# jamshed/CaPS-SA

Measured on AMD Instinct MI355X. Metric: suffixes/sec (SA+LCP build), higher is better.
Workload: dtype u32

## Files before the change

caps-sa_amd/_binding.py:

```python
from __future__ import annotations

import ctypes
import weakref

import numpy as np

_u64, _vp, _ci = ctypes.c_uint64, ctypes.c_void_p, ctypes.c_int


class Stats(ctypes.Structure):
    _fields_ = [
        ("n", ctypes.c_uint64),
        ("idx_bytes", ctypes.c_uint32),
        ("p_eff", ctypes.c_uint32),
        ("ppp", ctypes.c_uint32),
        ("bits_per_char", ctypes.c_uint32),
        ("merge_passes_phase1", ctypes.c_uint32),
        ("merge_passes_phase2", ctypes.c_uint32),
        ("merge_passes_samples", ctypes.c_uint32),
        ("long_runs", ctypes.c_uint32),
        ("max_partition", ctypes.c_uint64),
        ("workspace_bytes", ctypes.c_uint64),
        ("ms_total", ctypes.c_double),
        ("ms_pack", ctypes.c_double),
        ("ms_sort_subarrays", ctypes.c_double),
        ("ms_select_pivots", ctypes.c_double),
        ("ms_locate_pivots", ctypes.c_double),
        ("ms_partition", ctypes.c_double),
        ("ms_merge_partitions", ctypes.c_double),
        ("ms_boundary_lcp", ctypes.c_double),
        ("ms_output", ctypes.c_double),
        ("ms_h2d", ctypes.c_double),
        ("ms_d2h", ctypes.c_double),
        ("merge_pass_ms", ctypes.c_double),
        ("merge_pass_launches", ctypes.c_uint64),
        ("merge_pass_elems", ctypes.c_uint64),
        ("tile_sort_ms", ctypes.c_double),
        ("tile_sort_launches", ctypes.c_uint64),
        ("tile_sort_elems", ctypes.c_uint64),
        ("bucket_scatter_ms", ctypes.c_double),
        ("bucket_scatter_launches", ctypes.c_uint64),
        ("bucket_scatter_elems", ctypes.c_uint64),
        ("bucket_count_ms", ctypes.c_double),
        ("collate_ms", ctypes.c_double),
        ("slot_splits", ctypes.c_uint32),
        ("slot_splits_redone", ctypes.c_uint32),
        ("path_direct", ctypes.c_uint32),
        ("path_fallback", ctypes.c_uint32),
        ("direct_groups", ctypes.c_uint32),
        ("direct_quantile", ctypes.c_uint32),
        ("direct_max_group", ctypes.c_uint64),
        ("level_a_ms", ctypes.c_double),
        ("direct_key_bits", ctypes.c_uint32),
        ("run_buckets", ctypes.c_uint32),
        ("result_waves", ctypes.c_uint32),
        ("n_devices", ctypes.c_uint32),
        ("ms_upload_max", ctypes.c_double),
        ("ms_upload_min", ctypes.c_double),
        ("ms_device_build_max", ctypes.c_double),
        ("ms_device_build_min", ctypes.c_double),
        ("ms_download_max", ctypes.c_double),
        ("ms_download_min", ctypes.c_double),
        ("tie_groups_deferred", ctypes.c_uint64),
        ("tie_elems_deferred", ctypes.c_uint64),
        ("tie_levels", ctypes.c_uint32),
        ("lcp_bytes_on_link", ctypes.c_uint32),
        ("finish_ms", ctypes.c_double),
        ("run_bucket_ms", ctypes.c_double),
        ("msd_ms", ctypes.c_double),
        ("knot_slot_splits", ctypes.c_uint32),
        ("knot_slot_splits_redone", ctypes.c_uint32),
        ("spill_entries", ctypes.c_uint64),
        ("direct_records", ctypes.c_uint32),
        ("tile_chain", ctypes.c_uint32),
        ("scatter_issue", ctypes.c_uint32),
    ]

    def as_dict(self) -> dict:
        return {k: getattr(self, k) for k, _ in self._fields_}


class ShardInfo(ctypes.Structure):
    _fields_ = [
        ("n", ctypes.c_uint64),
        ("p", ctypes.c_uint32), ("ppp", ctypes.c_uint32), ("rank", ctypes.c_uint32), ("world", ctypes.c_uint32),
        ("g0", ctypes.c_uint32), ("g1", ctypes.c_uint32),
        ("bits_per_char", ctypes.c_uint32), ("idx_bytes", ctypes.c_uint32),
        ("part_lo", ctypes.c_uint32), ("part_hi", ctypes.c_uint32),
        ("local_elems", ctypes.c_uint64),
        ("m_local", ctypes.c_uint64), ("m_total", ctypes.c_uint64),
        ("recv_total", ctypes.c_uint64),
        ("slice_off", ctypes.c_uint64),
        ("capacity", ctypes.c_uint64),
        ("ms_phase1", ctypes.c_double), ("ms_pivots", ctypes.c_double), ("ms_collate", ctypes.c_double),
        ("ms_phase2", ctypes.c_double),
        ("direct_fallback", ctypes.c_uint32), ("direct_groups", ctypes.c_uint32), ("direct_sub", ctypes.c_uint32),
        ("n_streams", ctypes.c_uint32),
        ("stream_cap", ctypes.c_uint64), ("send_capacity", ctypes.c_uint64),
        ("ms_scatter", ctypes.c_double), ("ms_sort", ctypes.c_double),
        ("ms_level_a", ctypes.c_double), ("ms_level_b", ctypes.c_double), ("ms_tile_sort", ctypes.c_double),
        ("ms_merge_passes", ctypes.c_double),
        ("level_a_elems", ctypes.c_uint64),
        ("slot_splits", ctypes.c_uint32), ("slot_splits_redone", ctypes.c_uint32),
        ("key_bytes", ctypes.c_uint32), ("exchange", ctypes.c_uint32),
        ("direct_quantile", ctypes.c_uint32), ("run_buckets", ctypes.c_uint32),
        ("tie_groups_deferred", ctypes.c_uint64), ("tie_levels", ctypes.c_uint32), ("reserved_", ctypes.c_uint32),
    ]

    def as_dict(self) -> dict:
        return {k: getattr(self, k) for k, _ in self._fields_}


SHARD_EXPORTS = ["shard_create", "shard_destroy", "shard_info", "shard_phase1", "shard_pivots", "shard_collate",
                 "shard_phase2", "shard_last_sa", "shard_fix_first_lcp", "shard_scatter", "shard_plan", "shard_sort",
                 "shard_phase1_arrays", "shard_set_key_bits"]

EXPORTS = ["device_count", "last_error", "version", "stats_bytes", "shard_info_bytes", "workspace_bytes", "workspace_bytes_ex", "release_cache", "host_alloc", "host_free", "gen_rand_seq",
           "inverse_bwt_workspace_bytes", "fm_index_bytes", "fm_from_bwt_workspace_bytes", "fm_count", "fm_locate", "fm_count_device", "fm_locate_device",
           "fm_index_bytes_ex", "fm_add_text_samples", "fm_add_text_samples_device", "fm_extract_workspace_bytes", "fm_extract", "fm_extract_device",
           "fm_match", "fm_match_device", "fm_mems_workspace_bytes", "fm_mems", "fm_mems_device", "fm_wide_index_bytes",
           "fm_wide_workspace_bytes", "kmer_workspace_bytes", "cross_workspace_bytes", "coll_workspace_bytes", "lpf_workspace_bytes", "lz77_workspace_bytes", "lce_index_bytes",
           "lce_range_min", "lce_range_min_device", "lce", "lce_device"] + SHARD_EXPORTS + [
    f"{name}_{sfx}"
    for sfx in ("u32", "u64")
    for name in ("build", "build_multi", "build_device", "verify_device", "verify_slice_device", "sort_suffixes", "sort_segments", "merge",
                 "upper_bound", "lcp", "build_bwt", "bwt_device", "inverse_bwt", "inverse_bwt_device", "fm_build", "fm_build_device",
                 "fm_build_from_bwt", "fm_build_from_bwt_device", "fm_build_wide", "fm_build_wide_device",
                 "kmers", "kmers_device", "kmer_spectrum", "kmer_spectrum_device", "kmer_census", "kmer_census_device",
                 "lpf", "lpf_device", "lz77", "lz77_device", "isa", "isa_device", "lce_build", "lce_build_device",
                 "cross_mums", "cross_mums_device", "cross_mems", "cross_mems_device",
                 "coll_kmers", "coll_kmers_device", "coll_sharing", "coll_sharing_device")
]


MEM_DTYPE = np.dtype([("pattern", "<u8"), ("start", "<u4"), ("length", "<u4"), ("first", "<u8"), ("count", "<u8")])

KMER_DTYPE = np.dtype([("first", "<u8"), ("count", "<u8"), ("pos", "<u8")])

CROSS_DTYPE = np.dtype([("a", "<u8"), ("b", "<u8"), ("len", "<u8")])
CROSS_MAX_OCC = 64

COLL_DTYPE = np.dtype([("first", "<u8"), ("count", "<u8"), ("occ", "<u8"), ("docs", "<u8")])
COLL_MAX_DOCS = 64

LZ_DTYPE = np.dtype([("pos", "<u8"), ("len", "<u8"), ("src", "<u8")])
LZ_LITERAL = 0xFFFFFFFFFFFFFFFF


class CapsSaError(RuntimeError):
    def __init__(self, code: int, msg: str):
        super().__init__(f"caps_sa error {code}: {msg}")
        self.code = code


def _sfx(idx_bits: int):
    return {32: ("u32", np.uint32), 64: ("u64", np.uint64)}[idx_bits]


# ... 965 lines not shown
```

caps-sa_amd/csrc/kernels.h:

```cpp
#pragma once
#include "kernel_lang.h"
#include "text.h"

namespace caps {

#ifndef CAPS_TILE_E
#define CAPS_TILE_E 4096
#endif
#ifndef CAPS_TILE_NT
#define CAPS_TILE_NT 1024
#endif
#ifndef CAPS_TILE_WAVES
#define CAPS_TILE_WAVES 8
#endif
#ifndef CAPS_LOCK_K
#define CAPS_LOCK_K 4
#endif
constexpr uint32_t TILE_E = CAPS_TILE_E;
constexpr uint32_t TILE_NT = CAPS_TILE_NT;
constexpr uint32_t TILE_EPT = TILE_E / TILE_NT;
constexpr uint32_t LOCK_K = CAPS_LOCK_K < TILE_EPT ? CAPS_LOCK_K : TILE_EPT;
#define TILE_WAVES_PER_SIMD CAPS_TILE_WAVES
#ifdef CAPS_NO_WAVES_BOUND
#undef LAUNCH_BOUNDS2
// ... 461 lines not shown
        }
    }
}


template <typename idx_t, int BITS, int K, bool RUNS = true>
DEV_INLINE void multi_lower_bound(const uint32_t* __restrict__ P, uint64_t n, const uint64_t* skey, const idx_t* ssa,
                                  const uint64_t (&key)[K], const idx_t (&sa)[K], uint32_t (&lo)[K], const uint32_t (&hi)[K],
                                  uint32_t top)
{
    for (uint32_t s = top >> 1; s >= 1; s >>= 1) {
        UNROLL
        for (int k = 0; k < K; ++k) {
            const uint32_t idx = lo[k] + s - 1;
            const uint64_t mk = skey[idx < TILE_E ? idx : TILE_E - 1];
            if (idx < hi[k] && mk < key[k]) lo[k] += s;
        }
    }
    UNROLL
    for (int k = 0; k < K; ++k) {
        if (lo[k] < hi[k] && skey[lo[k]] == key[k]) {
            uint32_t a = lo[k], b = hi[k];
            while (a < b) {
                const uint32_t mid = (a + b) >> 1;
                if (suffix_less<BITS, RUNS>(P, n, skey[mid], (uint64_t)ssa[mid], key[k], (uint64_t)sa[k])) a = mid + 1;
                else b = mid;
            }
            lo[k] = a;
        }
    }
}

template <int K>
DEV_INLINE void multi_key_bound(const uint64_t* skey, const uint64_t (&key)[K], const bool (&upper)[K], uint32_t (&lo)[K],
                                const uint32_t (&hi)[K], uint32_t top)
{
    for (uint32_t s = top >> 1; s >= 1; s >>= 1) {
        UNROLL
        for (int k = 0; k < K; ++k) {
            const uint32_t idx = lo[k] + s - 1;
            const uint64_t mk = skey[idx < TILE_E ? idx : TILE_E - 1];
            if (idx < hi[k] && (upper[k] ? mk <= key[k] : mk < key[k])) lo[k] += s;
        }
    }
}

HD uint32_t pow2_above(uint32_t x) { return 1u << (32 - (x ? __builtin_clz(x) : 32)); }

struct BucketParams {
    uint64_t kmin;
    uint64_t range;
    uint32_t shift;
    uint32_t B;
    uint32_t post;
    uint32_t m;
};

HD BucketParams make_bucket_params(uint64_t kmin, uint64_t kmax, uint32_t B)
{
    BucketParams q;
    q.kmin = kmin;
    q.B = B;
    q.range = kmax > kmin ? kmax - kmin : 0;
    q.shift = q.range ? (uint32_t)caps_clz64(q.range) : 0u;
    const uint64_t r32 = (q.range << q.shift) >> 32;
    uint32_t bits = 1;
    while ((2ull * B) >> bits) ++bits;
    q.post = bits < 32 ? 32 - bits : 0;
    const uint64_t num = (uint64_t)B << (32 + q.post);
    q.m = q.range ? (uint32_t)(num / (r32 + 1)) : 0u;
    return q;
}

DEV_INLINE uint32_t bucket_of(const BucketParams& bp, uint64_t key)
{
    if (bp.B <= 1) return 0;
    if (key <= bp.kmin) return 0;
    const uint64_t d = key - bp.kmin;
    if (d >= bp.range) return bp.B - 1;
    const uint32_t d32 = (uint32_t)((d << bp.shift) >> 32);
    const uint32_t b = caps_umul32hi(d32, bp.m) >> bp.post;
    return b < bp.B ? b : bp.B - 1;
}

template <uint32_t NBINS>
DEV_INLINE void block_exclusive_scan(KCTX uint32_t* h)
{
#ifdef CAPS_EMUL
    (void)kctx_;
    std::vector<uint32_t> c(NBINS);
    for (uint32_t i = 0; i < NBINS; ++i) c[i] = h[i];
    SYNC_LDS();
    uint32_t run = 0;
    for (uint32_t i = 0; i < NBINS; ++i) { h[i] = run; run += c[i]; }
    h[NBINS] = run;
    SYNC_LDS();
#else
    constexpr uint32_t BPT = NBINS / TILE_NT;
    static_assert(BPT >= 1 && BPT * TILE_NT == NBINS, "counters per thread");
    __shared__ uint32_t wave_tot[TILE_NT / 64];
    const uint32_t tid = threadIdx.x, lane = tid & 63, wv = tid >> 6;
    uint32_t v[BPT], sum = 0;
    UNROLL
    for (uint32_t i = 0; i < BPT; ++i) { v[i] = h[tid * BPT + i]; sum += v[i]; }
    uint32_t x = sum;
#define CAPS_DPP_ADD(ctrl, rows) x += (uint32_t)__builtin_amdgcn_update_dpp(0, (int)x, ctrl, rows, 0xF, false)
    CAPS_DPP_ADD(0x111, 0xF);
    CAPS_DPP_ADD(0x112, 0xF);
    CAPS_DPP_ADD(0x114, 0xF);
    CAPS_DPP_ADD(0x118, 0xF);
    CAPS_DPP_ADD(0x142, 0xA);
    CAPS_DPP_ADD(0x143, 0xC);
#undef CAPS_DPP_ADD
    if (lane == 63) wave_tot[wv] = x;
    SYNC_LDS();
    uint32_t run = x - sum;
    if (TILE_NT / 64 <= 16) {
        const uint32_t wt = lane < TILE_NT / 64 ? wave_tot[lane] : 0u;
        uint32_t ws = wt;
#define CAPS_DPP_ADD(ctrl) ws += (uint32_t)__builtin_amdgcn_update_dpp(0, (int)ws, ctrl, 0xF, 0xF, false)
        CAPS_DPP_ADD(0x111);
        CAPS_DPP_ADD(0x112);
        CAPS_DPP_ADD(0x114);
        CAPS_DPP_ADD(0x118);
#undef CAPS_DPP_ADD
        const int wvs = __builtin_amdgcn_readfirstlane((int)wv);
        run += (uint32_t)__builtin_amdgcn_readlane((int)ws, wvs) - (uint32_t)__builtin_amdgcn_readlane((int)wt, wvs);
    } else {
        for (uint32_t w = 0; w < wv; ++w) run += wave_tot[w];
    }
    UNROLL
    for (uint32_t i = 0; i < BPT; ++i) { h[tid * BPT + i] = run; run += v[i]; }
    if (tid == TILE_NT - 1) h[NBINS] = run;
    SYNC_LDS();
#endif
}
DEV_INLINE void block_exclusive_scan_bins(KCTX uint32_t* hist) { block_exclusive_scan<TILE_BINS_>(KCTX_PASS hist); }

template <typename idx_t> struct FinalOut {
    idx_t* sa = nullptr;
    idx_t* lcp = nullptr;
    uint64_t* first_key = nullptr;
    uint64_t* last_key = nullptr;
    idx_t* first_sa = nullptr;
    idx_t* last_sa = nullptr;
};

#ifdef CAPS_EMUL
extern "C" void caps_emul_count_tile(bool fast, bool known_range);
extern "C" void caps_emul_count_tile2(bool two_level_ok);
extern "C" void caps_emul_count_tile3(bool equalised_ok);
#endif
constexpr uint32_t TILE_BINS = TILE_BINS_;
#ifndef CAPS_TILE_BIN_LIMIT
#define CAPS_TILE_BIN_LIMIT 48
#endif
#ifndef CAPS_EQ_BIN_LIMIT
#define CAPS_EQ_BIN_LIMIT 128
#endif
constexpr uint32_t TILE_BIN_LIMIT = CAPS_TILE_BIN_LIMIT;
constexpr uint32_t EQ_BIN_LIMIT = CAPS_EQ_BIN_LIMIT;

template <typename idx_t>
DEV_INLINE uint64_t lcp_capped(uint32_t l, uint64_t n, idx_t a, idx_t b)
{
    if (sizeof(idx_t) == 4) {
        const uint32_t room = (uint32_t)n - (uint32_t)(a > b ? a : b);
        return l < room ? l : room;
    }
    const uint64_t room = n - (uint64_t)(a > b ? a : b);
    return l < room ? l : room;
}
template <int BITS, bool RUNS, typename idx_t>
DEV_INLINE uint64_t tile_pair_lcp(const uint32_t* __restrict__ P, uint64_t n, uint64_t ka, idx_t a, uint64_t kb, idx_t b, uint32_t)
{
    const uint64_t x = ka ^ kb;
    if (x) return lcp_capped<idx_t>((uint32_t)caps_clz64(x) / BITS, n, a, b);
    return pair_lcp<BITS, RUNS>(P, n, ka, (uint64_t)a, kb, (uint64_t)b);
}
template <int BITS, bool RUNS, typename idx_t>
DEV_INLINE uint64_t tile_pair_lcp(const uint32_t* __restrict__ P, uint64_t n, uint32_t ka, idx_t a, uint32_t kb, idx_t b, uint32_t cs)
{
    return pair_lcp32<BITS, RUNS>(P, n, ka, (uint64_t)a, kb, (uint64_t)b, cs);
}

template <typename idx_t> HD idx_t tie_sentinel() { return (idx_t)~(idx_t)0; }
template <int BITS, bool RUNS, typename idx_t>
DEV_INLINE uint64_t deferring_pair_lcp(const uint32_t* __restrict__ P, uint64_t n, uint64_t* __restrict__ bflag, uint32_t g, uint64_t ka, idx_t a,
                                       uint64_t kb, idx_t b)
{
    if (bflag && ka == kb) { bflag[g] = 1; return (uint64_t)tie_sentinel<idx_t>(); }
    return tile_pair_lcp<BITS, RUNS>(P, n, ka, a, kb, b, 0u);
}

#if defined(CAPS_PHASE_CLOCK) && !defined(CAPS_EMUL)
__device__ unsigned long long caps_phase_clock[32];
#define PHASE_T0() unsigned long long pc_t_ = clock64()
#define PHASE_MARK(i) do { const unsigned long long t_ = clock64(); if (threadIdx.x == 0) atomicAdd(&caps_phase_clock[i], t_ - pc_t_); pc_t_ = clock64(); } while (0)
#else
#define PHASE_T0() ((void)0)
#define PHASE_MARK(i) ((void)0)
#endif

#if defined(CAPS_EQ_CHECK) && !defined(CAPS_EMUL)
__device__ unsigned int caps_eq_check[64];
#define EQ_OK(ok, id) ((ok) ? true : (atomicAdd(&caps_eq_check[id], 1u), false))
#else
#define EQ_OK(ok, id) (true)
#endif
#define EQ_CHK(ok, id) ((void)EQ_OK((ok), (id)))

struct __attribute__((packed, aligned(4))) KeySaRec {
    uint32_t key_lo, key_hi;
    uint32_t sa;
};
static_assert(sizeof(KeySaRec) == 12 && alignof(KeySaRec) == 4, "12-byte records");
#ifdef CAPS_EMUL
DEV_INLINE KeySaRec rec_stream_load(const KeySaRec* p) { return *p; }
#elif !defined(CAPS_NO_STREAM_HINTS)
typedef uint32_t caps_u32x3 __attribute__((ext_vector_type(3)));
typedef caps_u32x3 caps_u32x3_a4 __attribute__((aligned(4)));
DEV_INLINE KeySaRec rec_stream_load(const KeySaRec* p)
{
    const caps_u32x3 v = __builtin_nontemporal_load(reinterpret_cast<const caps_u32x3_a4*>(p));
    KeySaRec r;
    r.key_lo = v.x; r.key_hi = v.y; r.sa = v.z;
    return r;
}
#else
DEV_INLINE KeySaRec rec_stream_load(const KeySaRec* p) { return *p; }
#endif
template <typename KP, typename idx_t> DEV_INLINE void store_rec(KP* out, uint64_t i, uint64_t key, idx_t sa)
{
    KeySaRec r;
    r.key_lo = (uint32_t)key; r.key_hi = (uint32_t)(key >> 32); r.sa = (uint32_t)sa;
    reinterpret_cast<KeySaRec*>(out)[i] = r;
}

DEV_INLINE const uint64_t* tile_src(const uint64_t* in, const uint64_t* out, bool from_out) { return from_out ? out : in; }
DEV_INLINE const uint32_t* tile_src(const uint32_t* in, const uint64_t*, bool) { return in; }

#define TILE_OUTGROWN (slot_cap != 0 && t.s1 - t.s0 > (uint64_t)slot_cap)

#define TILE_SRC_KEY in_key
#define TILE_SRC_SA in_sa
#define TILE_SORT_LOAD                                                                                          \
    PAR(tid) {                                                                                                  \
        if (tid == 0) { kmm[0] = ~0ull; kmm[1] = 0; flag[0] = 0; }                                              \
        for (uint32_t i = tid; i <= TILE_BINS; i += K_BLOCK_DIM) hist[i] = 0;                                   \
        UNROLL                                                                                                  \
        for (uint32_t k = 0; k < TILE_EPT; ++k) {                                                               \
            const uint32_t e = tid + k * TILE_NT;                                                               \
            if (e < cnt) {                                                                                      \
                uint64_t key;                                                                                   \
                idx_t sa;                                                                                       \
                if (FROM_TEXT) {                                                                                \
                    key = window64<BITS>(P, text_base + start + e);                                             \
                    sa = (idx_t)(text_base + start + e);                                                        \
                } else if (TILE_KEYS_FROM_TEXT) {    \
                    sa = STREAM_LOAD(&TILE_SRC_SA[in0 + e]);                                                    \
                    key = window64<BITS>(P, (uint64_t)sa);                                                      \
                } else {                                                                                        \
                    key = STREAM_LOAD(&TILE_SRC_KEY[in0 + e]);                                                  \
                    sa = STREAM_LOAD(&TILE_SRC_SA[in0 + e]);                                                    \
                }                                                                                               \
                TL(rk, tid, k) = (decltype(TL(rk, tid, k) + 0))key;                                             \
                TL(rs, tid, k) = sa;                                                                            \
            }                                                                                                   \
        }                                                                                                       \
    }

#define TILE_SYNC() SYNC()
#define TILE_SORT_RANGE TILE_SORT_RANGE_(seg_map[g])
#define TILE_SORT_RANGE_(MAP)                                                                                   \
    const bool known_range = seg_map != nullptr;                                                                \
    if (!known_range) {                                                                                         \
        TILE_SYNC();                                                                       \
        PAR(tid) {                                                                                              \
            uint64_t mn = ~0ull, mx = 0;                                                                        \
            UNROLL                                                                                              \
            for (uint32_t k = 0; k < TILE_EPT; ++k) {                                                           \
                const uint32_t e = tid + k * TILE_NT;                                                           \
                if (e < cnt) {                                                                                  \
                    const uint64_t key = (uint64_t)TL(rk, tid, k);                                              \
                    mn = key < mn ? key : mn;                                                                   \
                    mx = key > mx ? key : mx;                                                                   \
                }                                                                                               \
            }                                                                                                   \
            BLOCK_MINMAX_U64(&kmm[0], &kmm[1], mn, mx);                                                         \
        }                                                                                                       \
    }                                                                                                           \
    TILE_SYNC();                                                                                                \
    const BucketParams tb = known_range ? (MAP) : make_bucket_params(kmm[0], kmm[1], TILE_BINS);

#define TILE_SORT_PLACE_FINAL                                                                                   \
    PAR(tid) {                                                                                                  \
        UNROLL                                                                                                  \
        for (uint32_t k = 0; k < TILE_EPT; ++k) {                                                               \
            const uint32_t e = tid + k * TILE_NT;                                                               \
            if (e < cnt) {                                                                                      \
                const uint32_t d = TL(rd, tid, k);                                                              \
                skey[d] = TL(rk, tid, k);                                                                       \
                ssa[d] = TL(rs, tid, k);                                                                        \
            }                                                                                                   \
        }                                                                                                       \
    }                                                                                                           \
    TILE_SYNC();

#define TILE_SORT_EMIT TILE_SORT_EMIT_(0u)
#define TILE_EMIT_LCP_(ka, a, kb, b) tile_pair_lcp<BITS, TILE_RUNS>(P, n, ka, a, kb, b, TILE_KEY_SHIFT)
#define TILE_SORT_EMIT_(OV)                                                                                     \
    PAR(tid) {                                                                                                  \
        UNROLL                                                                                                  \
        for (uint32_t k = 0; k < TILE_EPT; ++k) {                                                               \
            const uint32_t e = tid + k * TILE_NT;                                                               \
            if (e < cnt) {                                                                                      \
                const uint64_t key = skey[e];                                                                   \
                const idx_t sa = ssa[e];                                                                        \
                uint64_t l = 0;                                                                                 \
                if (with_lcp && e) {                                                                            \
                    const uint32_t ov_ = (OV);                                                                  \
                    l = ov_ ? ov_ : TILE_EMIT_LCP_(skey[e - 1], ssa[e - 1], skey[e], sa);                          \
                }                                                                                               \
                if (direct) {                                                                                   \
                    STREAM_STORE(&fin.sa[start + e], sa);                                                       \
                    STREAM_STORE(&fin.lcp[start + e], (idx_t)l);                                                \
                    if (e == 0) { fin.first_key[g] = key; fin.first_sa[g] = sa; }                               \
                    if (e == cnt - 1) { fin.last_key[g] = key; fin.last_sa[g] = sa; }                           \
                } else {                                                                                        \
                    out_key[start + e] = key;                                                                   \
                    out_sa[start + e] = sa;                                                                     \
                    if (with_lcp) out_lcp[start + e] = (idx_t)l;                                                \
                }                                                                                               \
            }                                                                                                   \
        }                                                                                                       \
    }

template <typename idx_t, int BITS, bool FROM_TEXT, typename KT = uint64_t, int CHAIN = 0>
GLOBAL_FN LAUNCH_BOUNDS2(TILE_NT, TILE_WAVES_PER_SIMD) tile_sort_kernel(KCTX SegDesc sd, const uint32_t* __restrict__ P, uint64_t n,
                                                  uint64_t text_base, uint32_t lcp_mode, uint32_t slot_cap, const KT* in_key,
                                                  const idx_t* in_sa, uint64_t* out_key, idx_t* out_sa, idx_t* out_lcp,
                                                  FinalOut<idx_t> fin, const BucketParams* __restrict__ seg_map,
                                                  uint32_t* __restrict__ redo, const uint8_t* __restrict__ kshift)
{
    constexpr bool TILE_RUNS = false;
    constexpr bool K32 = sizeof(KT) == 4;
    constexpr bool TILE_KEYS_FROM_TEXT = false;
    constexpr bool BY_BUCKET = CHAIN != 0;
    constexpr uint32_t CHAIN_EARLY = BY_BUCKET ? TILE_EPT - 1 : 0u;
    static_assert(!K32 || !FROM_TEXT, "32-bit keys come from the slots of level B");
    static_assert(!BY_BUCKET || (!FROM_TEXT && !K32 && sizeof(idx_t) == 4), "bucket-indexed: 64-bit keys and 32-bit indices in slots");
    TL_DECL(KT, rk, TILE_EPT);
    TL_DECL(idx_t, rs, TILE_EPT);
    uint64_t bs0 = 0, bs1 = 0;
    BucketParams tb_early = BucketParams();
    if (BY_BUCKET) {
        bs0 = sd.seg_start[K_BLOCK_IDX];
        bs1 = sd.seg_start[K_BLOCK_IDX + 1];
        tb_early = seg_map[K_BLOCK_IDX];
        PAR(tid) {
            const uint64_t in0e = (uint64_t)K_BLOCK_IDX * slot_cap;
            UNROLL
            for (uint32_t k = 0; k < CHAIN_EARLY; ++k) {
                TL(rk, tid, k) = STREAM_LOAD(&in_key[in0e + tid + k * TILE_NT]);
                TL(rs, tid, k) = STREAM_LOAD(&in_sa[in0e + tid + k * TILE_NT]);
            }
        }
        ISSUE_FENCE();
    }
    const uint32_t b = K_BLOCK_IDX;
    if (!BY_BUCKET && b >= sd.tile_off[sd.G]) return;
    const uint32_t g = BY_BUCKET ? b : sd.tile_rec[b].g;
    const TileInfo t = BY_BUCKET ? TileInfo{bs0, bs1, 0u, g, {0u, 0u}} : tile_info(sd, b);
    if (BY_BUCKET && t.s1 == t.s0) return;
    const uint64_t start = t.s0 + (uint64_t)t.tl * TILE_E;
    const uint32_t cnt = (uint32_t)(t.s1 - start < TILE_E ? t.s1 - start : TILE_E);
    const bool with_lcp = lcp_mode != 0 && (t.s1 - t.s0) <= TILE_E;
    const bool direct = with_lcp && fin.sa != nullptr;
    const uint64_t in0 = slot_cap ? (uint64_t)g * slot_cap : start;
    const uint32_t TILE_KEY_SHIFT = K32 ? kshift[g] : 0u;
    const uint32_t tie_from = K32 ? (TILE_KEY_SHIFT + 32u) / BITS : TextTraits<BITS>::KCH;
    SHARED_ARRAY(KT, skey, TILE_E);
    SHARED_ARRAY(idx_t, ssa, TILE_E);
    SHARED_ARRAY(uint32_t, hist, TILE_BINS + 1);
    SHARED_ARRAY(uint64_t, kmm, 2);
    SHARED_ARRAY(uint32_t, flag, 1);
    constexpr bool SLOT_ORDER = sizeof(idx_t) == 4;
    SHARED_ARRAY(uint16_t, sbin, SLOT_ORDER ? TILE_E : 1);
    SHARED_ARRAY(uint16_t, perm, SLOT_ORDER ? TILE_E : 1);
    TL_DECL(uint32_t, rd, TILE_EPT);
    TL_DECL(uint32_t, rb, TILE_EPT);

    PHASE_T0();
    if (BY_BUCKET) {
        PAR(tid) {
            if (tid == 0) flag[0] = 0;
            for (uint32_t i = tid; i <= TILE_BINS; i += K_BLOCK_DIM) hist[i] = 0;
            UNROLL
            for (uint32_t k = CHAIN_EARLY; k < TILE_EPT; ++k) {
                const uint32_t e = tid + k * TILE_NT;
                if (e < cnt) {
                    TL(rk, tid, k) = STREAM_LOAD(&in_key[in0 + e]);
                    TL(rs, tid, k) = STREAM_LOAD(&in_sa[in0 + e]);
                }
            }
        }
    } else {
        TILE_SORT_LOAD
    }
    TILE_SORT_RANGE_(BY_BUCKET ? tb_early : seg_map[g])
    PHASE_MARK(0);
    bool fast = cnt > 1 && tb.range > 0;
    if (fast) {
        PAR(tid) {
            UNROLL
            for (uint32_t k = 0; k < TILE_EPT; ++k) {
                const uint32_t e = tid + k * TILE_NT;
                if (e < cnt) {
                    const uint32_t bin = bucket_of(tb, TL(rk, tid, k));
                    const uint32_t r = FETCH_ADD_U32(&hist[bin], 1u);
                    if (r >= TILE_BIN_LIMIT) flag[0] = 1;
                    TL(rb, tid, k) = bin;
                    TL(rd, tid, k) = r;
                }
            }
        }
        SYNC();
        fast = flag[0] == 0;
        PHASE_MARK(1);
    }
    if (cnt == 1) {
        PAR(tid) { if (tid == 0) { skey[0] = TL(rk, tid, 0); ssa[0] = TL(rs, tid, 0); } }
        SYNC();
        fast = true;
    } else if (fast) {
        block_exclusive_scan_bins(KCTX_PASS hist);
        PHASE_MARK(2);
        PAR(tid) {
            UNROLL
            for (uint32_t k = 0; k < TILE_EPT; ++k) {
                const uint32_t e = tid + k * TILE_NT;
                if (e < cnt) {
                    const uint32_t slot = hist[TL(rb, tid, k)] + TL(rd, tid, k);
                    skey[slot] = TL(rk, tid, k);
                    ssa[slot] = TL(rs, tid, k);
                    if (SLOT_ORDER) sbin[slot] = (uint16_t)TL(rb, tid, k);
                    else TL(rd, tid, k) = slot;
                }
            }
        }
        SYNC();
        PHASE_MARK(3);
        PAR(tid) {
            UNROLL
            for (uint32_t k = 0; k < TILE_EPT; ++k) {
                const uint32_t e = tid + k * TILE_NT;
                if (e < cnt) {
                    const uint32_t slot = SLOT_ORDER ? e : TL(rd, tid, k), bin = SLOT_ORDER ? (uint32_t)sbin[slot] : TL(rb, tid, k);
                    const uint32_t bs = hist[bin], be = hist[bin + 1];
                    const uint64_t key = SLOT_ORDER ? (uint64_t)skey[slot] : (uint64_t)TL(rk, tid, k);
                    uint32_t less = 0;
                    for (uint32_t j = bs; j < be; ++j) {
                        const uint64_t kj = skey[j];
                        less += kj < key ? 1u : 0u;
                        if (kj == key && j != slot) {
                            const uint64_t sa = SLOT_ORDER ? (uint64_t)ssa[slot] : (uint64_t)TL(rs, tid, k);
                            const uint32_t c = suffix_less_tie_bounded<BITS>(P, n, (uint64_t)ssa[j], sa, tie_from);
                            if (c == 2u) flag[0] = 1;
                            less += c & 1u;
                        }
                    }
                    if (SLOT_ORDER) RACY_STORE_U16(&perm[bs + less], (uint16_t)slot);
                    else TL(rd, tid, k) = bs + less;
                }
            }
        }
        SYNC();
        fast = flag[0] == 0;
        PHASE_MARK(4);
        if (fast && !SLOT_ORDER) {
            TILE_SORT_PLACE_FINAL
            PHASE_MARK(5);
        }
    }
#ifdef CAPS_EMUL
    caps_emul_count_tile(fast, known_range);
#endif
    if (!fast) {
        PAR(tid) { if (tid == 0) redo[1 + FETCH_ADD_U32(&redo[0], 1u)] = BY_BUCKET ? sd.tile_off[g] : b; }
        return;
    }
    if (SLOT_ORDER && cnt > 1) {
        PAR(tid) {
            UNROLL
            for (uint32_t k = 0; k < TILE_EPT; ++k) {
                const uint32_t e = tid + k * TILE_NT;
                if (e < cnt) {
                    const uint32_t sl = perm[e];
                    const KT key = skey[sl];
                    const idx_t sa = ssa[sl];
                    uint64_t l = 0;
                    if (with_lcp && e) { const uint32_t sp = perm[e - 1]; l = TILE_EMIT_LCP_(skey[sp], ssa[sp], key, sa); }
                    if (direct) {
                        STREAM_STORE(&fin.sa[start + e], sa);
                        STREAM_STORE(&fin.lcp[start + e], (idx_t)l);
                        if (e == 0) { fin.first_key[g] = key; fin.first_sa[g] = sa; }
                        if (e == cnt - 1) { fin.last_key[g] = key; fin.last_sa[g] = sa; }
                    } else {
                        out_key[start + e] = key;
                        out_sa[start + e] = sa;
                        if (with_lcp) out_lcp[start + e] = (idx_t)l;
                    }
                }
            }
        }
    } else {
        TILE_SORT_EMIT
    }
    PHASE_MARK(6);
}

GLOBAL_FN LAUNCH_BOUNDS(256) hot_tiles_kernel(KCTX SegDesc sd, uint32_t slot_cap, TileInfo* __restrict__ hot)
{
    PAR(tid) {
        const uint32_t nt = sd.tile_off[sd.G];
        const uint32_t i = K_BLOCK_IDX * K_BLOCK_DIM + tid;
        if (i < nt) {
            TileInfo t = sd.tile_rec[i];
            if (t.s1 - t.s0 > (uint64_t)slot_cap) { t.s1 = t.s0; t.tl = 0; }
            hot[i] = t;
        }
    }
}

GLOBAL_FN LAUNCH_BOUNDS(256) queue_all_tiles_kernel(KCTX SegDesc sd, uint32_t* __restrict__ redo)
{
    PAR(tid) {
        const uint32_t nt = sd.tile_off[sd.G];
        const uint32_t i = K_BLOCK_IDX * K_BLOCK_DIM + tid;
        if (i < nt) redo[1 + i] = i;
        if (i == 0) redo[0] = nt;
    }
}

#ifndef CAPS_EQ_ROUNDS
#define CAPS_EQ_ROUNDS 2
#endif
constexpr uint32_t EQ_ROUNDS = CAPS_EQ_ROUNDS;
#ifndef CAPS_TIE_G1
#define CAPS_TIE_G1 8
#endif
#ifndef CAPS_TIE_LIST_MAX
#define CAPS_TIE_LIST_MAX 2
#endif
constexpr uint32_t TIE_G1 = CAPS_TIE_G1;
constexpr uint32_t TIE_G2 = 64;
constexpr uint32_t TIE_LIST_CAP = TILE_E / 8;
constexpr uint32_t TIE_LIST_MAX = CAPS_TIE_LIST_MAX;
constexpr uint32_t TIE_DEEP_CAP = 64;
constexpr uint32_t TIE_VDEEP_CAP = 32;
constexpr uint32_t TIE_BIG_CAP = 1024;
constexpr uint32_t TIE_BIG_LANES = 64;
constexpr uint32_t EQ_FRAC_BITS = 13;
static_assert((uint64_t)TILE_BINS_ << EQ_FRAC_BITS <= (1u << 24), "positions fit 24 bits");

DEV_INLINE uint32_t eq_pos(const BucketParams& bp, uint64_t key)
{
    const uint32_t top = (bp.B << EQ_FRAC_BITS) - 1u;
    if (key <= bp.kmin) return 0;
    const uint64_t d = key - bp.kmin;
    if (d >= bp.range) return top;
    const uint32_t d32 = (uint32_t)((d << bp.shift) >> 32);
    const uint64_t prod = (uint64_t)d32 * bp.m;
    const uint32_t sh = 32u + bp.post;
    const uint32_t x = (uint32_t)(sh >= EQ_FRAC_BITS ? prod >> (sh - EQ_FRAC_BITS) : prod << (EQ_FRAC_BITS - sh));
    return x < top ? x : top;
}

DEV_INLINE uint32_t eq_big_lcp(const uint16_t* vslot, const uint32_t* vlcp, uint32_t cnt, uint32_t e)
{
    uint32_t l = 0;
    for (uint32_t q = 0; q < cnt && q < TIE_VDEEP_CAP; ++q)
        if (vslot[q] == e) l = vlcp[q];
    return l;
}

template <int BITS, bool TEXT, typename idx_t>
DEV_INLINE uint64_t eq_emit_lcp(const uint32_t* __restrict__ P, uint64_t n, uint64_t ka, idx_t a, uint64_t kb, idx_t b, uint32_t* lost, bool test_drop)
{
    if (TEXT) return pair_lcp<BITS, false>(P, n, ka, (uint64_t)a, kb, (uint64_t)b);
    const uint64_t x = ka ^ kb;
    if (x == 0) {
#ifdef CAPS_EMUL
        if (!test_drop) { std::fprintf(stderr, "eq_emit_lcp: neighbours %llu, %llu with equal keys and no lcp from the tie phases\n", (unsigned long long)a, (unsigned long long)b); std::abort(); }
#endif
        *lost = 1;
    }
    return lcp_capped<idx_t>(x ? (uint32_t)caps_clz64(x) / BITS : TextTraits<BITS>::KCH, n, a, b);
}

#ifndef CAPS_EQ_WAVES
#define CAPS_EQ_WAVES TILE_WAVES_PER_SIMD
#endif
#undef TILE_EMIT_LCP_
#define TILE_EMIT_LCP_(ka, a, kb, b) eq_emit_lcp<BITS, VDEEP>(P, n, ka, a, kb, b, &flag[1], TEST_DROP)
#undef TILE_SRC_KEY
#undef TILE_SRC_SA
#define TILE_SRC_KEY src_key
#define TILE_SRC_SA src_sa
#ifndef CAPS_EQ_FULL_SYNC
#undef TILE_SYNC
#define TILE_SYNC() SYNC_LDS()
#endif
#if !defined(CAPS_EMUL) && !defined(CAPS_PAR_PLAIN_ONLY)
#pragma push_macro("PAR")
#undef PAR
#define PAR(tid) PAR_FRESH(tid)
#define CAPS_PAR_SWITCHED
#endif
template <typename idx_t, int BITS, bool FROM_TEXT, bool VDEEP = false, bool PERSIST = true>
GLOBAL_FN LAUNCH_BOUNDS2(TILE_NT, CAPS_EQ_WAVES) tile_sort_eq_kernel(KCTX SegDesc sd, const uint32_t* __restrict__ P, uint64_t n,
                                                  uint64_t text_base, uint32_t lcp_mode, uint32_t slot_cap, const uint64_t* in_key,
                                                  const idx_t* in_sa, uint64_t* out_key, idx_t* out_sa, idx_t* out_lcp,
                                                  FinalOut<idx_t> fin, const BucketParams* __restrict__ seg_map,
// ... 1138 lines not shown
            uint64_t len = 0;
            for (uint32_t x = 0; x < sub && first + x < G; ++x) len += seg_end_of(seg_start, seg_end, first + x) - seg_start[first + x];
            uint64_t kmin = 0, kmax = ~0ull;
            if (range_mode >= 1) {
                const uint32_t j = part_off + parent;
                if (j > 0) kmin = pkey[j - 1];
                if (j + 1 < part_total) kmax = pkey[j];
                if (range_mode == 2) key32_range(kmin, kmax, j > 0, gshift[j]);
            }
            uint32_t B = 1;
            if (enable && len > TILE_E && kmax > kmin) B = (uint32_t)((len + BUCKET_TARGET - 1) / BUCKET_TARGET);
            if (sub > 1 && B < 2) B = 2;
            if (fine > 1 && B > 1 && B <= BUCKET_LDS) {
                const uint32_t k = BUCKET_LDS / B < fine ? BUCKET_LDS / B : fine;
                B *= k;
            }
            const BucketParams q = make_bucket_params(kmin, kmax, B);
            bp[g] = q;
            segB[g] = (g % sub == sub - 1 || g == G - 1) ? B : 0;
        }
    }
}

GLOBAL_FN LAUNCH_BOUNDS(256) bucket_group_kernel(KCTX uint32_t G, const uint64_t* __restrict__ segB, const uint64_t* __restrict__ bstart,
                                                 const uint64_t* __restrict__ fsegB, const uint64_t* __restrict__ fstart,
                                                 const uint64_t* __restrict__ fcount, uint64_t* __restrict__ count,
                                                 uint32_t* __restrict__ gfirst)
{
    SHARED_ARRAY(uint64_t, fc, BUCKET_LDS);
    for (uint32_t g = K_BLOCK_IDX; g < G; g += K_GRID_DIM) {
        const uint32_t B = (uint32_t)segB[g], F = (uint32_t)fsegB[g];
        const uint64_t b0 = bstart[g], f0 = fstart[g];
        if (B > BUCKET_LDS || F <= B || F > BUCKET_LDS) {
            PAR(tid) {
                for (uint32_t i = tid; i < B; i += K_BLOCK_DIM) { count[b0 + i] = i < F ? fcount[f0 + i] : 0; gfirst[b0 + i] = i; }
            }
            continue;
        }
        PAR(tid) { for (uint32_t f = tid; f < F; f += K_BLOCK_DIM) fc[f] = fcount[f0 + f]; }
        SYNC();
        PAR(tid) {
            if (tid == 0) {
                uint64_t cap = TILE_E, total = 0;
                for (uint32_t f = 0; f < F; ++f) total += fc[f];
                for (uint64_t lo = TILE_E, hi = total > TILE_E ? total : TILE_E;;) {
                    const uint64_t c_try = lo == TILE_E ? lo : (lo + hi) / 2;
                    uint32_t need = 1;
                    uint64_t run = 0;
                    for (uint32_t f = 0; f < F; ++f) {
                        const uint64_t c = fc[f];
                        if (run > 0 && run + c > c_try) { ++need; run = 0; }
                        run += c;
                    }
                    if (need <= B) { cap = c_try; hi = c_try; if (c_try == TILE_E) break; }
                    else lo = c_try + 1;
                    if (lo >= hi) { cap = hi; break; }
                }
                uint32_t gi = 0;
                uint64_t sum = 0;
                gfirst[b0] = 0;
                for (uint32_t f = 0; f < F; ++f) {
                    const uint64_t c = fc[f];
                    if (sum > 0 && sum + c > cap && gi + 1 < B) {
                        count[b0 + gi] = sum;
                        ++gi;
                        gfirst[b0 + gi] = f;
                        sum = 0;
                    }
                    sum += c;
                }
                count[b0 + gi] = sum;
                for (uint32_t i = gi + 1; i < B; ++i) { count[b0 + i] = 0; gfirst[b0 + i] = F; }
            }
        }
        SYNC();
    }
}

GLOBAL_FN LAUNCH_BOUNDS(256) bucket_ranges_kernel(KCTX const uint64_t* __restrict__ bstart, uint32_t G,
                                                  const BucketParams* __restrict__ bps, const uint64_t* __restrict__ pkey,
                                                  uint32_t range_mode, uint32_t part_off, uint32_t part_total, uint32_t sub,
                                                  BucketParams* __restrict__ tile_map,
                                                  const BucketParams* __restrict__ fbps, const uint32_t* __restrict__ gfirst,
                                                  const uint8_t* __restrict__ gshift, uint8_t* __restrict__ kshift)
{
    PAR(tid) {
        const uint64_t i = (uint64_t)K_BLOCK_IDX * K_BLOCK_DIM + tid;
        if (i < bstart[G]) {
            uint32_t a = 0, b = G;
            while (b - a > 1) {
                const uint32_t mid = (a + b) / 2;
                if (bstart[mid] <= i) a = mid; else b = mid;
            }
            const uint32_t g = a;
            const BucketParams bp = bps[g];
            uint64_t kmin = 0, kmax = ~0ull;
            if (range_mode >= 1) {
                const uint32_t j = part_off + g / sub;
                if (j > 0) kmin = pkey[j - 1];
                if (j + 1 < part_total) kmax = pkey[j];
                if (range_mode == 2) { key32_range(kmin, kmax, j > 0, gshift[j]); kshift[i] = gshift[j]; }
            }
            const uint32_t bk = (uint32_t)(i - bstart[g]);
            const double range1 = (double)(kmax - kmin) + 1.0;
            uint64_t l = kmin, h = kmax;
            if (bp.B > 1) {
                uint32_t lo = bk, hi = bk + 1, div = bp.B;
                if (gfirst) {
                    div = fbps[g].B;
                    lo = gfirst[i];
                    hi = bk + 1 < bp.B ? gfirst[i + 1] : div;
                    if (hi <= lo) hi = lo + 1;
                }
                const double dl = (double)lo / (double)div * range1, dh = (double)hi / (double)div * range1;
                if (lo > 0) l = kmin + (uint64_t)dl;
                if (hi < div) h = kmin + (uint64_t)dh;
                if (h < l) h = l;
            }
            tile_map[i] = make_bucket_params(l, h, TILE_BINS);
        }
    }
}

constexpr uint32_t TEXT_WIN = TILE_E / 4 + 24;
constexpr uint32_t SPLIT_LUT_BITS = TILE_E >= 4096 ? 12 : TILE_E >= 256 ? 8 : 4;
constexpr uint32_t SPLIT_LUT_CELLS = 1u << SPLIT_LUT_BITS;

template <int BITS> HD uint64_t text_win_base(uint64_t pos0) { return pos0 / TextTraits<BITS>::CPW; }

constexpr int MAP_LINEAR = 0, MAP_GROUPED = 1, MAP_SPLIT = 2;
HD uint32_t lds_swz(uint32_t i) { return i ^ ((i >> 4) & 15u) ^ ((i >> 8) & 15u); }
#ifdef CAPS_GA_NO_SWZ
#define GA_SWZ(i) (i)
#else
#define GA_SWZ(i) lds_swz(i)
#endif
constexpr uint32_t COUNT_CHUNK = 8;

template <bool REC, bool STREAM, typename KT, typename idx_t>
DEV_INLINE void load_elem(const KT* __restrict__ in_key, const idx_t* __restrict__ in_sa, uint64_t i, KT& key, idx_t& sa)
{
    if (REC) {
        const KeySaRec* p = reinterpret_cast<const KeySaRec*>(in_key) + i;
        const KeySaRec r = STREAM ? rec_stream_load(p) : *p;
        key = (KT)(((uint64_t)r.key_hi << 32) | r.key_lo);
        sa = (idx_t)r.sa;
    } else {
        key = STREAM ? STREAM_LOAD(&in_key[i]) : in_key[i];
        sa = STREAM ? STREAM_LOAD(&in_sa[i]) : in_sa[i];
    }
}
template <bool REC> DEV_INLINE uint64_t load_elem_key(const uint64_t* __restrict__ in_key, uint64_t i)
{
    if (REC) { const KeySaRec* p = reinterpret_cast<const KeySaRec*>(in_key) + i; return ((uint64_t)p->key_hi << 32) | p->key_lo; }
    return in_key[i];
}

template <typename idx_t, int BITS, int SRC, int MAP = MAP_LINEAR, bool REC_IN = false>
GLOBAL_FN LAUNCH_BOUNDS(TILE_NT) bucket_count_kernel(KCTX SegDesc sd, const uint32_t* __restrict__ P, uint64_t n_words,
                                                     uint64_t text_base, const uint64_t* __restrict__ in_key, RunSrc<idx_t> rsrc,
                                                     const BucketParams* __restrict__ bps, const uint64_t* __restrict__ bstart,
                                                     uint64_t* __restrict__ count, const uint64_t* __restrict__ split,
                                                     uint32_t split_stride, uint32_t in_sub, uint16_t* __restrict__ bid)
{
    constexpr bool FROM_TEXT = SRC == SRC_TEXT, FROM_RUNS = SRC == SRC_RUNS;
    SHARED_ARRAY(uint32_t, hist, BUCKET_LDS);
    SHARED_ARRAY(uint64_t, stab, MAP == MAP_SPLIT ? BUCKET_LDS : 1);
    SHARED_ARRAY(uint32_t, twin, FROM_TEXT ? TEXT_WIN : 1);
    SHARED_ARRAY(uint64_t, lsrc, FROM_RUNS ? TILE_E : 1);
    SHARED_ARRAY(idx_t, lrow, FROM_RUNS ? TILE_E : 1);
    const uint32_t n_tiles = sd.tile_off[sd.G];
    const uint32_t want = n_tiles / (4u * K_GRID_DIM);
    const uint32_t CH = want < 1u ? 1u : want > COUNT_CHUNK ? COUNT_CHUNK : want;
    const uint32_t n_chunks = (n_tiles + CH - 1) / CH;
    for (uint32_t v = K_BLOCK_IDX; v < n_chunks; v += K_GRID_DIM) {
    uint64_t cur_b0 = ~0ull;
    uint32_t cur_B = 0;
    const uint32_t b_end = (v + 1) * CH < n_tiles ? (v + 1) * CH : n_tiles;
    for (uint32_t b = v * CH; b < b_end; ++b) {
        const uint32_t g = sd.tile_rec[b].g;
        const TileInfo t = tile_info(sd, b);
        const uint64_t start = t.s0 + (uint64_t)t.tl * TILE_E;
        const uint32_t cnt = (uint32_t)(t.s1 - start < TILE_E ? t.s1 - start : TILE_E);
        const BucketParams bp = bps[g];
        const uint64_t b0 = bstart[g];
// ... 10 lines not shown
        PAR(tid) {
            if (fresh) {
                for (uint32_t i = tid; i < cur_B; i += K_BLOCK_DIM)
                    if (hist[i]) ATOMIC_ADD_U64(&count[cur_b0 + i], (uint64_t)hist[i]);
                if (lds) for (uint32_t i = tid; i < bp.B; i += K_BLOCK_DIM) hist[i] = 0;
                if (MAP == MAP_SPLIT && lds) for (uint32_t i = tid; i < n_split; i += K_BLOCK_DIM) stab[lds_swz(i)] = tab[i];
            }
            if (FROM_TEXT)
                for (uint32_t i = tid; i < TEXT_WIN; i += K_BLOCK_DIM) twin[i] = w0 + i < n_words ? P[w0 + i] : 0u;
            if (FROM_RUNS) { RUNS_STAGE(tid) }
        }
        if (fresh) { cur_b0 = lds ? b0 : ~0ull; cur_B = lds ? bp.B : 0u; }
        SYNC();
        const uint32_t top = pow2_above(n_split);
        PAR(tid) {
            uint64_t key[TILE_EPT];
            uint32_t bk[TILE_EPT];
            UNROLL
            for (uint32_t k = 0; k < TILE_EPT; ++k) {
                const uint32_t e = tid + k * TILE_NT;
                key[k] = 0;
                if (e < cnt)
                    key[k] = FROM_TEXT ? window64<BITS>(twin, text_base + start + e - w0 * TextTraits<BITS>::CPW)
                           : FROM_RUNS ? in_key[run_source<idx_t>(rsrc, runs_staged, lrow, lsrc, run_ns, run_rowR, run_rowA,
                                                                  run_a, run_b, run_x0 + e)]
                                       : load_elem_key<REC_IN>(in_key, start + e);
                bk[k] = MAP == MAP_SPLIT ? 0u : bucket_of(bp, key[k]);
            }
            if (MAP == MAP_SPLIT && lds) {
                for (uint32_t st = top >> 1; st >= 1; st >>= 1) {
                    UNROLL
                    for (uint32_t k = 0; k < TILE_EPT; ++k) {
                        const uint32_t idx = bk[k] + st - 1;
                        const uint64_t mk = stab[lds_swz(idx < n_split ? idx : n_split - 1)];
                        if (idx < n_split && mk < key[k]) bk[k] += st;
                    }
                }
            } else if (MAP == MAP_SPLIT) {
                for (uint32_t st = top >> 1; st >= 1; st >>= 1) {
                    UNROLL
                    for (uint32_t k = 0; k < TILE_EPT; ++k) {
                        const uint32_t idx = bk[k] + st - 1;
                        const uint64_t mk = tab[idx < n_split ? idx : n_split - 1];
                        if (idx < n_split && mk < key[k]) bk[k] += st;
                    }
                }
            }
            UNROLL
            for (uint32_t k = 0; k < TILE_EPT; ++k) {
                const uint32_t e = tid + k * TILE_NT;
                if (e < cnt) {
                    if (lds) FETCH_ADD_U32(&hist[bk[k]], 1u);
                    else ATOMIC_ADD_U64(&count[b0 + bk[k]], 1ull);
                    if (MAP == MAP_SPLIT && bid && lds) bid[start + e] = (uint16_t)bk[k];
                }
            }
        }
        SYNC();
    }
    if (cur_B) {
        PAR(tid) {
            for (uint32_t i = tid; i < cur_B; i += K_BLOCK_DIM)
                if (hist[i]) ATOMIC_ADD_U64(&count[cur_b0 + i], (uint64_t)hist[i]);
        }
        SYNC();
    }
    }
}

template <typename idx_t> struct Spill {
    uint64_t* count = nullptr;
    uint64_t cap = 0;
    uint32_t chunk = 0;
    uint64_t base = 0;
    uint64_t* key = nullptr;
    idx_t* sa = nullptr;
    uint32_t* bucket = nullptr;
    idx_t* rel = nullptr;
};
constexpr uint32_t SPILL_LONG = 64;
constexpr uint32_t SPILL_LONG_CAP = TILE_E / SPILL_LONG;
constexpr uint32_t SPILL_CHUNK = TILE_E / 128 ? TILE_E / 128 : 1;

template <typename idx_t, int BITS, int SRC, int MAP, typename KT = uint64_t, bool SPILL = false, bool REC_IN = false, bool ISSUE = false>
GLOBAL_FN LAUNCH_BOUNDS(TILE_NT) bucket_scatter_kernel(KCTX SegDesc sd, const uint32_t* __restrict__ P, uint64_t n_words,
                                                       uint64_t text_base, const KT* __restrict__ in_key,
                                                       const idx_t* __restrict__ in_sa, RunSrc<idx_t> rsrc,
                                                       const BucketParams* __restrict__ bps, const uint64_t* __restrict__ bstart,
                                                       const uint64_t* __restrict__ sub_start, uint64_t slot_cap,
                                                       idx_t* __restrict__ cursor,
                                                       KT* __restrict__ out_key, idx_t* __restrict__ out_sa,
                                                       const BucketParams* __restrict__ fbps, const uint32_t* __restrict__ gfirst,
                                                       const uint64_t* __restrict__ split, const uint16_t* __restrict__ split_lut,
                                                       const uint32_t* __restrict__ split_span, uint32_t sub, uint32_t split_stride,
                                                       uint32_t in_sub, const uint16_t* __restrict__ bid, Spill<idx_t> spill)
{
    constexpr bool GROUPED = MAP == MAP_GROUPED;
    const bool spec = slot_cap != 0;
    const idx_t NO_SLOT = (idx_t)~(idx_t)0;
#if CAPS_SCATTER_SWZ
    const uint32_t v = sub > 1 ? K_BLOCK_IDX
                               : (uint32_t)xcd_swizzle(K_BLOCK_IDX, K_GRID_DIM);
#else
    const uint32_t v = K_BLOCK_IDX;
#endif
    const uint32_t sx = sub > 1 ? K_BLOCK_IDX % sub : 0u;
    if (v >= sd.tile_off[sd.G]) return;
    const uint32_t b = v;
    const uint32_t g = sd.tile_rec[b].g;
    const TileInfo t = tile_info(sd, b);
    const uint64_t start = t.s0 + (uint64_t)t.tl * TILE_E;
    const uint32_t cnt = (uint32_t)(t.s1 - start < TILE_E ? t.s1 - start : TILE_E);
    static_assert(!ISSUE || (REC_IN && MAP == MAP_LINEAR && !SPILL), "loads first: the records of level A under the linear map");
    TL_DECL(KT, rk, TILE_EPT);
    TL_DECL(idx_t, rs, TILE_EPT);
    if (ISSUE) {
        if (cnt == 0) return;
        PAR(tid) {
            UNROLL
            for (uint32_t k = 0; k < TILE_EPT; ++k) {
                const uint32_t e = tid + k * TILE_NT;
                load_elem<REC_IN, true>(in_key, in_sa, start + (e < cnt ? e : cnt - 1), TL(rk, tid, k), TL(rs, tid, k));
            }
        }
        ISSUE_FENCE();
    }
    const BucketParams bp = bps[g];
    const uint64_t b0 = bstart[g];
    const bool grouped = GROUPED && bp.B > 1 && bp.B <= BUCKET_LDS;
    const BucketParams fbp = GROUPED ? fbps[g] : bp;
    SHARED_ARRAY(uint32_t, hist, TILE_BINS + 1);
    SHARED_ARRAY(idx_t, obase, TILE_BINS);
    static_assert(sizeof(KT) == 8 || (SRC == SRC_ARRAYS && MAP == MAP_LINEAR), "32-bit keys: arrays in, linear map");
    static_assert(!REC_IN || (SRC == SRC_ARRAYS && sizeof(KT) == 8 && sizeof(idx_t) == 4), "records: arrays in, 64-bit keys, 32-bit indices");
    SHARED_ARRAY(KT, skey, TILE_E);
    SHARED_ARRAY(idx_t, ssa, TILE_E);
    SHARED_ARRAY(uint16_t, sbk, TILE_E);
    SHARED_ARRAY(uint64_t, lr_at, SPILL ? SPILL_LONG_CAP : 1);
    SHARED_ARRAY(idx_t, lr_old, SPILL ? SPILL_LONG_CAP : 1);
    SHARED_ARRAY(uint32_t, lr_c, SPILL ? SPILL_LONG_CAP : 1);
    SHARED_ARRAY(uint32_t, lr_b, SPILL ? SPILL_LONG_CAP : 1);
    SHARED_ARRAY(uint32_t, nlong, 2);
    static_assert(!SPILL || (MAP == MAP_SPLIT && sizeof(KT) == 8), "the spill stream: splits by knots, 64-bit keys");
    TL_DECL(uint32_t, rb, TILE_EPT);
    TL_DECL(idx_t, rr, TILE_EPT);
    constexpr bool FROM_TEXT = SRC == SRC_TEXT, FROM_RUNS = SRC == SRC_RUNS;
    const bool lds = bp.B > 1 && bp.B <= BUCKET_LDS;
    uint32_t* twin = reinterpret_cast<uint32_t*>(skey);
    uint64_t* lsrc = reinterpret_cast<uint64_t*>(skey);
    idx_t* lrow = ssa;
    uint16_t* gtab = sbk;
    static_assert(TILE_E >= BUCKET_LDS && BUCKET_LDS <= 65536, "group table fits the bucket-id staging array");
    const uint64_t w0 = text_win_base<BITS>(text_base + start);
    uint64_t* stab = reinterpret_cast<uint64_t*>(skey) + TILE_E / 4;
    uint16_t* slut = reinterpret_cast<uint16_t*>(ssa);
    static_assert(TEXT_WIN * sizeof(uint32_t) <= (TILE_E / 4) * sizeof(uint64_t) && TILE_E / 4 + BUCKET_LDS <= TILE_E,
                  "text window + splitter table fit the key staging array");
    static_assert((SPLIT_LUT_CELLS + 1) * sizeof(uint16_t) <= TILE_E * sizeof(idx_t), "splitter LUT fits the index staging array");
    const uint32_t n_split = MAP == MAP_SPLIT && bp.B > 1 ? bp.B - 1 : 0u;
    const uint64_t* tab = MAP == MAP_SPLIT ? split + (uint64_t)(g / in_sub) * split_stride : nullptr;
    RUNS_TILE_SETUP
    if (ISSUE) {
        if (!lds) {
            PAR(tid) {
                UNROLL
                for (uint32_t k = 0; k < TILE_EPT; ++k) {
                    const uint32_t e = tid + k * TILE_NT;
                    if (e < cnt) {
                        const uint64_t bi = (b0 + (bp.B == 1 ? 0u : bucket_of(bp, (uint64_t)TL(rk, tid, k)))) * (spec ? sub : 1u) + sx;
                        const uint64_t off = bp.B == 1 ? (start - t.s0) + e : (uint64_t)caps_fetch_add(&cursor[bi], (idx_t)1);
                        if (!spec || off < slot_cap) {
                            const uint64_t dst = (spec ? bi * slot_cap : sub_start[bi]) + off;
                            out_key[dst] = TL(rk, tid, k);
                            out_sa[dst] = TL(rs, tid, k);
                        }
                    }
                }
                if (spec && bp.B == 1 && tid == 0) caps_fetch_add(&cursor[b0 * sub + sx], (idx_t)cnt);
            }
            DRAIN_GLOBAL();
            return;
        }
        PAR(tid) {
            for (uint32_t i = tid; i <= TILE_BINS; i += K_BLOCK_DIM) hist[i] = 0;
        }
        SYNC_LDS();
        PAR(tid) {
            UNROLL
            for (uint32_t k = 0; k < TILE_EPT; ++k) {
                const uint32_t e = tid + k * TILE_NT;
                if (e < cnt) {
                    const uint32_t bk = bucket_of(bp, (uint64_t)TL(rk, tid, k));
                    TL(rb, tid, k) = bk;
                    TL(rr, tid, k) = FETCH_ADD_U32(&hist[bk], 1u);
                }
            }
        }
        DRAIN_GLOBAL();
    } else {
    if (lds || FROM_TEXT || FROM_RUNS) {
        PAR(tid) {
            if (lds) for (uint32_t i = tid; i <= TILE_BINS; i += K_BLOCK_DIM) hist[i] = 0;
            if (SPILL && tid < 2) nlong[tid] = 0;
            if (MAP == MAP_SPLIT && lds && !bid) {
                for (uint32_t i = tid; i < n_split; i += K_BLOCK_DIM) stab[lds_swz(i)] = tab[i];
                if (split_lut) for (uint32_t i = tid; i <= SPLIT_LUT_CELLS; i += K_BLOCK_DIM) slut[i] = split_lut[i];
            }
            if (grouped)
                for (uint32_t i = tid; i < bp.B; i += K_BLOCK_DIM) {
                    const uint32_t f0 = gfirst[b0 + i], f1 = i + 1 < bp.B ? gfirst[b0 + i + 1] : fbp.B;
                    for (uint32_t f = f0; f < f1 && f < fbp.B; ++f) gtab[f] = (uint16_t)i;
                }
            if (FROM_TEXT)
                for (uint32_t i = tid; i < TEXT_WIN; i += K_BLOCK_DIM) twin[i] = w0 + i < n_words ? P[w0 + i] : 0u;
            if (FROM_RUNS) { RUNS_STAGE(tid) }
        }
        SYNC();
    }
    if (MAP == MAP_SPLIT && lds && bid) {
        PAR(tid) {
            UNROLL
            for (uint32_t k = 0; k < TILE_EPT; ++k) {
                const uint32_t e = tid + k * TILE_NT;
                if (e < cnt) {
                    const uint32_t bk = bid[start + e];
                    load_elem<REC_IN, false>(in_key, in_sa, start + e, TL(rk, tid, k), TL(rs, tid, k));
                    TL(rb, tid, k) = bk;
                    TL(rr, tid, k) = FETCH_ADD_U32(&hist[bk], 1u);
                }
            }
        }
    } else if (MAP == MAP_SPLIT && lds) {
        const uint32_t top = pow2_above(split_lut ? split_span[0] : n_split);
        TL_DECL(uint32_t, rh, TILE_EPT);
        PAR(tid) {
            UNROLL
            for (uint32_t k = 0; k < TILE_EPT; ++k) {
                const uint32_t e = tid + k * TILE_NT;
                const uint64_t src = start + e;
                uint64_t key = 0;
                idx_t sa = 0;
                if (e < cnt) {
                    if (FROM_TEXT) {
                        key = window64<BITS>(twin, text_base + start + e - w0 * TextTraits<BITS>::CPW);
                        sa = (idx_t)(text_base + start + e);
                    } else { KT key_in; load_elem<REC_IN, true>(in_key, in_sa, src, key_in, sa); key = (uint64_t)key_in; }
                }
                const uint32_t cell = (uint32_t)(key >> (64 - SPLIT_LUT_BITS));
                TL(rk, tid, k) = key;
                TL(rs, tid, k) = sa;
                TL(rb, tid, k) = split_lut ? slut[cell] : 0u;
                TL(rh, tid, k) = split_lut ? slut[cell + 1] : n_split;
            }
            for (uint32_t s = top >> 1; s >= 1; s >>= 1) {
                UNROLL
                for (uint32_t k = 0; k < TILE_EPT; ++k) {
                    const uint32_t idx = TL(rb, tid, k) + s - 1;
// ... 5 lines not shown
            for (uint32_t k = 0; k < TILE_EPT; ++k) {
                const uint32_t e = tid + k * TILE_NT;
                if (e < cnt) TL(rr, tid, k) = FETCH_ADD_U32(&hist[TL(rb, tid, k)], 1u);
            }
        }
    } else {
    PAR(tid) {
        UNROLL
        for (uint32_t k = 0; k < TILE_EPT; ++k) {
            const uint32_t e = tid + k * TILE_NT;
            if (e < cnt) {
                const uint64_t src = FROM_RUNS ? run_source<idx_t>(rsrc, runs_staged, lrow, lsrc, run_ns, run_rowR, run_rowA, run_a,
                                                                   run_b, run_x0 + e)
                                               : start + e;
                KT key_in = 0;
                idx_t sa = 0;
                if (FROM_TEXT) sa = (idx_t)(text_base + start + e);
                else load_elem<REC_IN, true>(in_key, in_sa, src, key_in, sa);
                const uint64_t key = FROM_TEXT ? window64<BITS>(twin, text_base + start + e - w0 * TextTraits<BITS>::CPW) : (uint64_t)key_in;
                uint32_t bk = 0;
                idx_t r;
                if (bp.B == 1) r = e;
                else {
                    if (MAP == MAP_SPLIT) {
                        uint32_t a = 0, z = bp.B - 1;
                        while (a < z) { const uint32_t mid = (a + z) >> 1; if (tab[mid] < key) a = mid + 1; else z = mid; }
                        bk = a;
                    } else {
                        bk = bucket_of(fbp, key);
                        if (grouped) bk = gtab[bk];
                    }
                    r = lds ? FETCH_ADD_U32(&hist[bk], 1u) : caps_fetch_add(&cursor[(b0 + bk) * (spec ? sub : 1u) + sx], (idx_t)1);
                }
                TL(rk, tid, k) = key;
                TL(rs, tid, k) = sa;
                TL(rb, tid, k) = bk;
                TL(rr, tid, k) = r;
            }
        }
    }
    }
    if (!lds) {
        PAR(tid) {
            UNROLL
            for (uint32_t k = 0; k < TILE_EPT; ++k) {
                const uint32_t e = tid + k * TILE_NT;
                if (e < cnt) {
                    const uint64_t off = (bp.B == 1 ? (start - t.s0) : 0) + TL(rr, tid, k);
                    const uint64_t bi = (b0 + TL(rb, tid, k)) * (spec ? sub : 1u) + sx;
                    if (!spec || off < slot_cap) {
                        const uint64_t dst = (spec ? bi * slot_cap : sub_start[bi]) + off;
                        out_key[dst] = TL(rk, tid, k);
                        out_sa[dst] = TL(rs, tid, k);
                    }
                }
            }
            if (spec && bp.B == 1 && tid == 0) caps_fetch_add(&cursor[b0 * sub + sx], (idx_t)cnt);
        }
        return;
    }
    }
    SYNC();
    constexpr uint32_t BPT = (TILE_BINS + TILE_NT - 1) / TILE_NT;
    TL_DECL(idx_t, co, BPT);
    TL_DECL(uint32_t, cc, BPT);
    PAR(tid) {
        UNROLL
        for (uint32_t j = 0; j < BPT; ++j) {
            const uint32_t i = tid + j * TILE_NT;
            const uint32_t c = i < bp.B ? hist[i] : 0u;
            TL(cc, tid, j) = c;
            TL(co, tid, j) = 0;
            if (c) TL(co, tid, j) = caps_fetch_add(&cursor[spec ? (b0 + i) * sub + sx : b0 + i], (idx_t)c);
        }
    }
    block_exclusive_scan_bins(KCTX_PASS hist);
    PAR(tid) {
        UNROLL
        for (uint32_t k = 0; k < TILE_EPT; ++k) {
            const uint32_t e = tid + k * TILE_NT;
            if (e < cnt) {
                const uint32_t bk = TL(rb, tid, k);
                const uint32_t q = hist[bk] + (uint32_t)TL(rr, tid, k);
                skey[q] = TL(rk, tid, k);
                ssa[q] = TL(rs, tid, k);
                sbk[q] = (uint16_t)bk;
            }
        }
        UNROLL
        for (uint32_t j = 0; j < BPT; ++j) {
            const uint32_t i = tid + j * TILE_NT;
            if (i < bp.B) {
                const uint32_t c = TL(cc, tid, j);
                const idx_t old = TL(co, tid, j);
                idx_t ob = 0;
                if (c) {
                    const uint64_t ci = spec ? (b0 + i) * sub + sx : b0 + i;
                    if (!spec) ob = (idx_t)(sub_start[b0 + i] + old);
                    else if ((uint64_t)old + c <= slot_cap) ob = (idx_t)(ci * slot_cap + old);
                    else if (SPILL && spill.count) {
                        uint64_t at = ~0ull;
                        if (spill.chunk) {
                            const uint32_t lo = FETCH_ADD_U32(&nlong[1], c);
                            if ((uint64_t)lo + c <= spill.chunk) at = (uint64_t)b * spill.chunk + lo;
                        }
                        if (at == ~0ull) at = FETCH_ADD_U64(spill.count, (uint64_t)c);
                        ob = NO_SLOT;
                        if (at + c <= spill.cap) {
                            ob = (idx_t)(spill.base + at);
                            if (c < SPILL_LONG) {
                                for (uint32_t j = 0; j < c; ++j) { spill.bucket[at + j] = (uint32_t)(b0 + i); spill.rel[at + j] = (idx_t)(old + j); }
                            } else {
                                const uint32_t q = FETCH_ADD_U32(&nlong[0], 1u);
                                lr_at[q] = at;
                                lr_old[q] = old;
                                lr_c[q] = c;
                                lr_b[q] = (uint32_t)(b0 + i);
                            }
                        }
                    } else ob = NO_SLOT;
                }
                obase[i] = ob;
            }
        }
    }
    if (ISSUE) DRAIN_GLOBAL();
    SYNC_LDS();
    PAR(tid) {
        UNROLL
        for (uint32_t k = 0; k < TILE_EPT; ++k) {
            const uint32_t q = tid + k * TILE_NT;
            if (q < cnt) {
                const uint32_t bk = sbk[q];
                const idx_t ob = obase[bk];
                if (SPILL && ob != NO_SLOT && (uint64_t)ob >= spill.base) {
                    const uint64_t dst = (uint64_t)ob - spill.base + (q - hist[bk]);
                    spill.key[dst] = skey[q];
                    spill.sa[dst] = ssa[q];
                } else if (ob != NO_SLOT) {
                    const uint64_t dst = (uint64_t)ob + (q - hist[bk]);
                    STREAM_STORE2(&out_key[dst], skey[q]);
                    STREAM_STORE2(&out_sa[dst], ssa[q]);
                }
            }
        }
        if (SPILL) {
            const uint32_t nl = nlong[0];
            for (uint32_t r = 0; r < nl && r < SPILL_LONG_CAP; ++r) {
                const uint64_t at = lr_at[r];
                const idx_t old = lr_old[r];
                const uint32_t c = lr_c[r], bb = lr_b[r];
                for (uint32_t j = tid; j < c; j += K_BLOCK_DIM) { spill.bucket[at + j] = bb; spill.rel[at + j] = (idx_t)(old + j); }
            }
        }
    }
}

template <typename idx_t>
GLOBAL_FN LAUNCH_BOUNDS(256) spill_gather_kernel(KCTX const uint64_t* __restrict__ seg_start, uint32_t NB, uint64_t slot_cap,
                                                 const uint8_t* __restrict__ skip, const uint64_t* __restrict__ slot_key,
                                                 const idx_t* __restrict__ slot_sa, uint64_t* __restrict__ dst_key,
                                                 idx_t* __restrict__ dst_sa)
{
    SHARED_ARRAY(uint32_t, lst, 256);
    SHARED_ARRAY(uint32_t, ln, 1);
    for (uint64_t base = (uint64_t)K_BLOCK_IDX * 256u; base < NB; base += (uint64_t)K_GRID_DIM * 256u) {
        PAR(tid) { if (tid == 0) ln[0] = 0; }
        SYNC();
        PAR(tid) {
            const uint64_t b = base + tid;
            if (b < NB) {
                const uint64_t len = seg_start[b + 1] - seg_start[b];
                if (len > slot_cap || (len && skip && skip[b])) lst[FETCH_ADD_U32(&ln[0], 1u)] = (uint32_t)b;
            }
        }
        SYNC();
        const uint32_t m = ln[0];
        for (uint32_t q = 0; q < m; ++q) {
            const uint32_t b = lst[q];
            const uint64_t s0 = seg_start[b], len = seg_start[b + 1] - s0;
            const uint64_t cnt = len < slot_cap ? len : slot_cap;
            PAR(tid) {
                for (uint64_t i = tid; i < cnt; i += K_BLOCK_DIM) {
                    dst_key[s0 + i] = slot_key[(uint64_t)b * slot_cap + i];
                    dst_sa[s0 + i] = slot_sa[(uint64_t)b * slot_cap + i];
                }
            }
        }
        SYNC();
    }
}

template <typename idx_t>
GLOBAL_FN LAUNCH_BOUNDS(256) spill_place_kernel(KCTX Spill<idx_t> sp, uint64_t cnt, const uint64_t* __restrict__ seg_start,
                                                uint64_t* __restrict__ dst_key, idx_t* __restrict__ dst_sa)
{
    PAR(tid) {
        for (uint64_t i = (uint64_t)K_BLOCK_IDX * K_BLOCK_DIM + tid; i < cnt; i += (uint64_t)K_GRID_DIM * K_BLOCK_DIM) {
            const uint32_t b = sp.bucket[i];
            if (b == ~0u) continue;
            const uint64_t d = seg_start[b] + (uint64_t)sp.rel[i];
            dst_key[d] = sp.key[i];
            dst_sa[d] = sp.sa[i];
        }
    }
}

#ifndef CAPS_GA_TILES
#define CAPS_GA_TILES 4
#endif
constexpr uint32_t GA_TILES = CAPS_GA_TILES;
constexpr uint32_t GA_E = GA_TILES * TILE_E;
constexpr uint32_t GA_EPT = GA_E / TILE_NT;
static_assert(GA_E <= (1u << 14) && BUCKET_LDS <= (1u << 11), "group << 14 | position fits a register");

template <typename idx_t, int BITS, typename KT = uint64_t, bool REC_OUT = false>
GLOBAL_FN LAUNCH_BOUNDS2(TILE_NT, TILE_WAVES_PER_SIMD) group_scatter_kernel(KCTX const uint32_t* __restrict__ P, uint64_t n_words,
                                                      uint64_t text_base, uint64_t len, const uint64_t* __restrict__ split, uint32_t K1,
                                                      const uint16_t* __restrict__ split_lut, const uint32_t* __restrict__ split_span,
                                                      uint32_t sub, uint64_t slot_cap, idx_t* __restrict__ cursor,
                                                      KT* __restrict__ out_key, idx_t* __restrict__ out_sa,
                                                      uint32_t tile_first, uint32_t tile_stride,
                                                      const uint64_t* __restrict__ region_start, const uint64_t* __restrict__ region_cap,
                                                      const uint8_t* __restrict__ gshift, uint32_t own_lo, uint32_t own_hi)
{
// ... 4442 lines not shown
```

caps-sa_amd/csrc/pipeline.h:

```cpp
#pragma once
#include <algorithm>
#include <cmath>
#include <cstdlib>
#include <cstdio>
#include <limits>
#include <stdexcept>
#include <string>
#include <vector>

#include "kernels.h"
#include "bounded.h"
#include "../../include/caps_sa_hip.h"

#ifndef CAPS_BACKEND_DEFINED
#include "hip_backend.h"
#endif

namespace caps {

template <typename idx_t> struct ElemBuf {
    uint64_t* key = nullptr;
    idx_t* sa = nullptr;
    idx_t* lcp = nullptr;
    size_t region_bytes = 0;
};

constexpr size_t WS_ALIGN = 256;
inline size_t align_up(size_t b) { return (b + (WS_ALIGN - 1)) & ~(WS_ALIGN - 1); }
inline char* align_up(char* p) { return reinterpret_cast<char*>(align_up(reinterpret_cast<uintptr_t>(p))); }

struct Arena {
    char* base = nullptr;
    size_t off = 0;
    template <typename T> T* take(size_t count)
    {
        off = align_up(off);
        T* p = base ? reinterpret_cast<T*>(base + off) : nullptr;
        off += count * sizeof(T);
        return p;
    }
};

struct SegBufs {
    uint64_t* seg_start = nullptr;
    uint64_t* seg_end = nullptr;
    uint32_t* tile_off = nullptr;
    TileInfo* tile_rec = nullptr;
    uint64_t* out2 = nullptr;
    uint32_t G = 0;
    SegDesc desc() const { return SegDesc{seg_start, tile_off, tile_rec, G}; }
};

constexpr uint32_t kMaxPasses = 96;

#ifndef CAPS_DIRECT_SUB
#define CAPS_DIRECT_SUB 8
#endif
constexpr uint32_t DIRECT_SUB = CAPS_DIRECT_SUB;
constexpr uint32_t DIRECT_RECORDS_DEFAULT = 1;
constexpr uint32_t DIRECT_TILE_CHAIN_DEFAULT = 1;
constexpr uint32_t DIRECT_SCATTER_ISSUE_DEFAULT = 1;
#ifndef CAPS_BUCKET_Q_32NDS
#define CAPS_BUCKET_Q_32NDS 24
#endif
#ifndef CAPS_QUANTILE_SPB
#define CAPS_QUANTILE_SPB 64
#endif
constexpr uint32_t BUCKET_Q = (TILE_E * CAPS_BUCKET_Q_32NDS) / 32;
constexpr uint32_t QUANTILE_SPB = CAPS_QUANTILE_SPB;

#ifndef CAPS_EQ_FINE
#define CAPS_EQ_FINE 16
#endif
constexpr uint32_t EQ_FINE = CAPS_EQ_FINE;

struct BucketBufs {
    BucketParams* params = nullptr;
    uint64_t* segB = nullptr;
    uint64_t* bstart = nullptr;
    uint64_t* count = nullptr;
    void* cursor = nullptr;
    uint64_t* scan_tmp = nullptr;
    uint64_t *first_key = nullptr, *last_key = nullptr;
    BucketParams* tile_map = nullptr;
    void *first_sa = nullptr, *last_sa = nullptr;
    SegBufs sub;
    BucketParams* fparams = nullptr;
    uint64_t* fsegB = nullptr;
    uint64_t* fstart = nullptr;
    uint64_t* fcount = nullptr;
    uint32_t* gfirst = nullptr;
    uint8_t* kshift = nullptr;
    uint8_t* skip = nullptr;
    uint64_t* run_list = nullptr;
    uint32_t nb_cap = 0;
    uint64_t tile_cap = 0;
    static uint32_t bucket_bound(uint64_t n_elems, uint32_t G) { return (uint32_t)(n_elems / BUCKET_Q + 2 * (uint64_t)G + 2); }
};

template <typename idx_t> struct Plan {
    uint64_t n = 0;
    int text_bits = 8;
    uint32_t p = 0;
    uint32_t ppp = 0;
    uint64_t m = 0;
    uint64_t tile_cap = 0;
    uint32_t* P = nullptr;
    ElemBuf<idx_t> A, B, SA_, SB_;
    uint64_t* pkey = nullptr;
    idx_t* psa = nullptr;
    idx_t* Pm = nullptr;
    idx_t* ruler = nullptr;
    idx_t* PmT = nullptr;
    idx_t* rulerT = nullptr;
    uint64_t* sizes = nullptr;
    uint64_t* gkey = nullptr;
    uint64_t* dstat = nullptr;
    idx_t* dcur = nullptr;
    uint16_t* glut = nullptr;
    uint8_t* gshift = nullptr;
    uint64_t* knots = nullptr;
    uint64_t* rcap = nullptr;
    uint64_t* rstart = nullptr;
    uint64_t* partial = nullptr;
    SegBufs seg1, seg2, segS;
    TileDesc* desc = nullptr;
    BucketBufs bk;
    uint64_t* pass_elems = nullptr;
    uint32_t* present = nullptr;
    uint8_t* lut = nullptr;
    size_t bytes = 0;
};

inline void effective_params(uint64_t n, uint64_t p_arg, uint32_t* p_eff, uint32_t* ppp)
{
    uint64_t p = p_arg > 0 ? p_arg : 8192;
    if (n / 16 < p) p = n / 16;
    if (p < 2) { *p_eff = (uint32_t)p; *ppp = 0; return; }
    const uint64_t a = (uint64_t)std::ceil(32.0 * std::log((double)n));
    const uint64_t b = n / p - 1;
    *p_eff = (uint32_t)p;
    *ppp = (uint32_t)(a < b ? a : b);
}

// ... 143 lines not shown
{
    auto alphabet = [&](uint64_t len, uint32_t present[8]) {
        be.memset(present_dev, 0, 16 * sizeof(uint32_t));
        const uint64_t want = (len + 16 * 256 - 1) / (16 * 256);
        const uint32_t grid = (uint32_t)(want < 4096 ? (want ? want : 1) : 4096);
        CAPS_LAUNCH(alphabet_kernel, grid, 256, be, dT, len, present_dev);
        be.d2h(present, present_dev, 8 * sizeof(uint32_t));
        be.sync();
    };
    auto pack = [&](int bits, const uint8_t lut[256], uint32_t* bad) {
        be.h2d(lut_dev, lut, 256);
        const uint64_t n_words = packed_words(n, bits);
        const uint64_t want = (n_words / (bits == 2 ? 1 : 4) + 255) / 256 + 1;
        const uint32_t grid = (uint32_t)(want < 65536 ? want : 65536);
        if (bits == 2) CAPS_LAUNCH(pack_kernel<2>, grid, 256, be, dT, n, (const uint8_t*)lut_dev, P, n_words, bad);
        else CAPS_LAUNCH(pack_kernel<8>, grid, 256, be, dT, n, (const uint8_t*)lut_dev, P, n_words, bad);
    };
    uint32_t present[8];
    uint8_t lut[256];
#ifdef CAPS_EMUL
    constexpr uint64_t SAMPLE = 1u << 12;
#else
    constexpr uint64_t SAMPLE = 1u << 20;
#endif
    if (n >= 16 * SAMPLE && !std::getenv("CAPS_SA_FULL_ALPHABET")) {
        alphabet(SAMPLE, present);
        if (build_lut(present, lut) == 2) {
            pack(2, lut, present_dev + 8);
            uint32_t bad = 0;
            be.d2h(&bad, present_dev + 8, sizeof bad);
            build_run_table(be, P, n, 2);
            if (!bad) return 2;
        }
    }
    alphabet(n, present);
    const int bits = build_lut(present, lut);
    if (bits > arena_bits) throw AlphabetError();
    pack(bits, lut, nullptr);
    build_run_table(be, P, n, bits);
    return bits;
}

template <typename OutT>
inline void device_exclusive_scan(Backend& be, const uint64_t* in, uint32_t G, OutT* out, uint64_t* tmp)
{
    const uint32_t chunks = (G + SCAN_CHUNK - 1) / SCAN_CHUNK;
    uint64_t* sums = tmp;
    uint64_t* offs = tmp + chunks + 1;
    CAPS_LAUNCH((block_scan_kernel<OutT>), chunks ? chunks : 1, 1024, be, in, (uint64_t)G, out, sums);
    CAPS_LAUNCH(scan_sizes_kernel, 1, 1024, be, (const uint64_t*)sums, chunks, offs);
    CAPS_LAUNCH((add_offsets_kernel<OutT>), chunks ? chunks : 1, 1024, be, out, (uint64_t)G, (const uint64_t*)offs, chunks);
}

#ifdef CAPS_EMUL
constexpr uint32_t kSmallScan = 48;
#else
constexpr uint32_t kSmallScan = 32768;
#endif

inline void prepare_segments(Backend& be, const SegBufs& s, uint64_t tile_bound, uint64_t* big_tmp = nullptr,
                             uint64_t* big_cnt = nullptr, bool use_end = false, const uint8_t* skip = nullptr)
{
    be.memset(s.out2, 0, 2 * sizeof(uint64_t));
    const uint64_t* send = use_end ? s.seg_end : nullptr;
    if (s.G <= kSmallScan || !big_tmp) {
        CAPS_LAUNCH(seg_prepare_kernel, 1, 1024, be, (const uint64_t*)s.seg_start, send, s.G, s.tile_off, s.out2, skip);
    } else {
        CAPS_LAUNCH(tile_count_kernel, (s.G + 255) / 256, 256, be, (const uint64_t*)s.seg_start, send, s.G, big_cnt, s.out2, skip);
        device_exclusive_scan<uint32_t>(be, big_cnt, s.G, s.tile_off, big_tmp);
        CAPS_LAUNCH(tile_total_kernel, 1, 64, be, (const uint32_t*)s.tile_off, s.G, s.out2);
    }
    const uint32_t grid = (uint32_t)((tile_bound + 255) / 256);
    CAPS_LAUNCH(tile_map_kernel, grid ? grid : 1, 256, be, (const uint64_t*)s.seg_start, send, (const uint32_t*)s.tile_off, s.G, s.tile_rec);
}

inline uint32_t tiles_of(uint64_t len) { return (uint32_t)((len + TILE_E - 1) / TILE_E); }

template <typename idx_t> struct SortResult {
    ElemBuf<idx_t> buf[2];
    uint32_t passes = 0;
    bool skip_finished = false;
    bool unified = false;
    bool k32 = false;
    bool failed = false;
    SegBufs segs;
    struct RunBucket { uint64_t s0, s1, key; };
    std::vector<RunBucket> run_buckets;
    SegBufs run_tables;
    const BucketBufs* run_bk = nullptr;
    TileDesc* run_desc = nullptr;
    uint64_t total = 0;
    uint64_t* defer_flags = nullptr;
    TileDesc* defer_desc = nullptr;
    uint64_t cap = 0;
    mutable bool msd_failed = false;
    KernelClock* finish_clock = nullptr;
    KernelClock* runb_clock = nullptr;
    KernelClock* msd_clock = nullptr;
    mutable uint64_t msd_groups = 0, msd_elems = 0;
    mutable uint32_t msd_levels = 0;
    uint32_t n_tiles = 0;
    FinalOut<idx_t> fin;
    ElemBuf<idx_t> uniform() const { return unified ? buf[0] : buf[passes & 1]; }
    PingPong<idx_t> pingpong() const
    {
        PingPong<idx_t> pp;
        for (int i = 0; i < 2; ++i) { pp.key[i] = buf[i].key; pp.sa[i] = buf[i].sa; pp.lcp[i] = buf[i].lcp; }
        return pp;
    }
};

struct SortOpts {
    bool from_text = false;
    uint64_t text_base = 0;
    bool need_lcp = false;
    bool skip_finished = false;
    bool no_equalise = false;
    const BucketBufs* bk = nullptr;
    uint32_t range_mode = 0;
    const uint64_t* pkey = nullptr;
    uint32_t part_off = 0, part_total = 0;
    bool speculate = false;
    uint32_t* slot_stats = nullptr;
    bool seg_ends = false;
    uint32_t sub = 1;
    const uint64_t* in_key = nullptr;
    const void* in_sa = nullptr;
    bool in_records = false;
    const uint8_t* gshift = nullptr;
    bool k32 = false;
    bool keys_only = false;
    bool comparison_only = false;
    bool skewed_keys = false;
    const uint64_t* knots = nullptr;
    uint32_t knots_per_parent = 0;
    bool knots_have_prev = false;
    bool spill_slots = false;
    TileInfo* hot_tile_rec = nullptr;
    uint64_t* spill_stats = nullptr;
    uint64_t in_extent = 0;
    const SegBufs* run_tables = nullptr;
    uint64_t* defer_flags = nullptr;
    const void* runs = nullptr;
    bool unify = false;
    void* final_sa = nullptr;
    void* final_lcp = nullptr;
    struct { uint64_t *first_key, *last_key; void *first_sa, *last_sa; } bnd = {nullptr, nullptr, nullptr, nullptr};
    uint32_t tile_chain = 0;
    uint32_t* tile_chain_used = nullptr;
    uint32_t scatter_issue = 0;
    uint32_t* scatter_issue_used = nullptr;
    KernelClock* tile_clock = nullptr;
    KernelClock* merge_clock = nullptr;
    KernelClock* scatter_clock = nullptr;
    KernelClock* count_clock = nullptr;
    uint64_t* pass_counters = nullptr;
};

template <typename idx_t, int BITS>
SortResult<idx_t> segmented_sort(Backend& be, const uint32_t* P, uint64_t n, TileDesc* desc, const SegBufs& s, uint32_t n_tiles,
                                 uint64_t max_len, ElemBuf<idx_t> cur, ElemBuf<idx_t> oth, uint64_t n_elems, const SortOpts& o)
{
    if (o.keys_only) {
        if (o.from_text || o.need_lcp || o.runs) throw std::invalid_argument("a keys-only sort takes (key, index) arrays and emits no LCPs");
        n = 0;
    }
    SortResult<idx_t> r;
    r.buf[0] = cur;
    r.buf[1] = oth;
    r.skip_finished = o.skip_finished;
    r.segs = s;
    r.n_tiles = n_tiles;
    if (n_tiles == 0) return r;
    const bool dbg = std::getenv("CAPS_SA_DEBUG") != nullptr;
    auto mark = [&](const char* what) { if (dbg) { be.sync(); std::fprintf(stderr, "[sort] %s\n", what); } };
    bool from_text = o.from_text;
    const BucketParams* seg_map = nullptr;
    SegBufs segs = s;
    bool skip = o.skip_finished;
    uint32_t slot_cap = 0;
    uint64_t* slot_key = nullptr;
    idx_t* slot_sa = nullptr;
    uint32_t slot_grid = 0;
    if (o.bk && (max_len > TILE_E || o.seg_ends)) {
        const BucketBufs& bk = *o.bk;
        const SegDesc psd = s.desc();
        const uint64_t* s_end = o.seg_ends ? (const uint64_t*)s.seg_end : (const uint64_t*)nullptr;
        const bool by_knots = o.knots != nullptr;
        if (by_knots) {
            const uint64_t NB = (uint64_t)(s.G / o.sub) * o.knots_per_parent;
            if (NB > bk.nb_cap) throw std::invalid_argument("more knot buckets than the bucket tables hold");
            CAPS_LAUNCH(knot_plan_kernel, (s.G + 255) / 256, 256, be, s.G, o.sub, o.knots_per_parent, bk.params, bk.segB);
            CAPS_LAUNCH(scan_sizes_kernel, 1, 1024, be, (const uint64_t*)bk.segB, s.G, bk.bstart);
            CAPS_LAUNCH(knot_ranges_kernel, (uint32_t)((NB + 255) / 256), 256, be, o.knots, NB, bk.tile_map, o.knots_have_prev ? 1u : 0u);
        } else {
        CAPS_LAUNCH(bucket_plan_kernel, (s.G + 255) / 256, 256, be, (const uint64_t*)s.seg_start, s_end, s.G, o.range_mode, o.pkey, o.part_off,
                    o.part_total ? o.part_total : s.G, 1u, 1u, o.sub,
                    bk.params, bk.segB, o.gshift);
        CAPS_LAUNCH(scan_sizes_kernel, 1, 1024, be, (const uint64_t*)bk.segB, s.G, bk.bstart);
        CAPS_LAUNCH(bucket_ranges_kernel, (bk.nb_cap + 255) / 256, 256, be, (const uint64_t*)bk.bstart, s.G,
                    (const BucketParams*)bk.params, o.pkey, o.range_mode, o.part_off, o.part_total ? o.part_total : s.G, o.sub,
                    bk.tile_map, (const BucketParams*)nullptr, (const uint32_t*)nullptr, o.gshift, bk.kshift);
        }
        seg_map = bk.tile_map;
        mark("bucket plan");
        const uint32_t pgrid = n_tiles < be.persistent_blocks() ? n_tiles : be.persistent_blocks();
        const bool runs = o.runs != nullptr;
        const RunSrc<idx_t> rsrc = runs ? *static_cast<const RunSrc<idx_t>*>(o.runs) : RunSrc<idx_t>();
        const uint64_t n_words = from_text ? packed_words(n, BITS) : 0;
        const uint64_t tbase = from_text ? o.text_base : 0;
        const uint64_t* src_key = o.in_key ? o.in_key : (const uint64_t*)cur.key;
        const idx_t* src_sa = o.in_key ? static_cast<const idx_t*>(o.in_sa) : (const idx_t*)cur.sa;
        const bool rec_in = o.in_records;
        if (rec_in && (sizeof(idx_t) != 4 || !o.in_key || from_text || o.runs || o.k32))
            throw std::invalid_argument("records: (64-bit key, 32-bit index) arrays given by the caller");
        uint16_t* bid = nullptr;
        if (by_knots && o.in_extent && !from_text && !o.runs && oth.region_bytes && !std::getenv("CAPS_SA_NO_BUCKET_IDS")) {
            const size_t room = (size_t)((reinterpret_cast<char*>(oth.key) + oth.region_bytes) - reinterpret_cast<char*>(oth.lcp));
            const uint64_t extent = o.in_key ? o.in_extent : n_elems;
            if (room >= extent * sizeof(uint16_t)) bid = reinterpret_cast<uint16_t*>(oth.lcp);
        }
        auto scatter = [&](const uint64_t* sub_start, uint32_t cap, uint64_t* okey, idx_t* osa, bool grouped = false) {
            const BucketParams* fbps = grouped ? bk.fparams : nullptr;
            const uint32_t* gfirst = grouped ? bk.gfirst : nullptr;
            BackendEvent s0 = be.record();
#define CAPS_SCATTER_LAUNCH(SRC_, MAP_, ikey, isa)                                                                          \
            CAPS_LAUNCH((bucket_scatter_kernel<idx_t, BITS, SRC_, MAP_>), n_tiles, TILE_NT, be, psd, P, n_words, tbase, ikey, isa, rsrc, \
                        (const BucketParams*)bk.params, (const uint64_t*)bk.bstart, sub_start, (uint64_t)cap, static_cast<idx_t*>(bk.cursor),       \
                        okey, osa, fbps, gfirst, o.knots, (const uint16_t*)nullptr, (const uint32_t*)nullptr, 1u, o.knots_per_parent, o.sub, \
                        (const uint16_t*)bid, Spill<idx_t>())
#define CAPS_SCATTER_LAUNCH_REC(MAP_)                                                                                        \
            CAPS_LAUNCH((bucket_scatter_kernel<idx_t, BITS, SRC_ARRAYS, MAP_, uint64_t, false, true>), n_tiles, TILE_NT, be, psd, P, n_words, tbase, \
                        src_key, src_sa, rsrc, (const BucketParams*)bk.params, (const uint64_t*)bk.bstart, sub_start, (uint64_t)cap,               \
                        static_cast<idx_t*>(bk.cursor), okey, osa, fbps, gfirst, o.knots, (const uint16_t*)nullptr, (const uint32_t*)nullptr, 1u,   \
                        o.knots_per_parent, o.sub, (const uint16_t*)bid, Spill<idx_t>())
            const uint64_t* nokey = nullptr;
            const idx_t* nosa = nullptr;
            if (rec_in) {
                if constexpr (sizeof(idx_t) == 4) {
                    if (by_knots) CAPS_SCATTER_LAUNCH_REC(MAP_SPLIT);
                    else if (grouped) CAPS_SCATTER_LAUNCH_REC(MAP_GROUPED);
                    else if (o.scatter_issue & 1u) {
                        CAPS_LAUNCH((bucket_scatter_kernel<idx_t, BITS, SRC_ARRAYS, MAP_LINEAR, uint64_t, false, true, true>), n_tiles, TILE_NT, be, psd,
                                    P, n_words, tbase, src_key, src_sa, rsrc, (const BucketParams*)bk.params, (const uint64_t*)bk.bstart, sub_start,
                                    (uint64_t)cap, static_cast<idx_t*>(bk.cursor), okey, osa, fbps, gfirst, o.knots, (const uint16_t*)nullptr,
                                    (const uint32_t*)nullptr, 1u, o.knots_per_parent, o.sub, (const uint16_t*)bid, Spill<idx_t>());
                        if (o.scatter_issue_used) *o.scatter_issue_used |= 1u;
                    } else CAPS_SCATTER_LAUNCH_REC(MAP_LINEAR);
                }
            } else
            if (from_text) { if (grouped) CAPS_SCATTER_LAUNCH(SRC_TEXT, MAP_GROUPED, nokey, nosa); else CAPS_SCATTER_LAUNCH(SRC_TEXT, MAP_LINEAR, nokey, nosa); }
            else if (runs) { if (grouped) CAPS_SCATTER_LAUNCH(SRC_RUNS, MAP_GROUPED, src_key, src_sa);
                             else CAPS_SCATTER_LAUNCH(SRC_RUNS, MAP_LINEAR, src_key, src_sa); }
            else if (by_knots) CAPS_SCATTER_LAUNCH(SRC_ARRAYS, MAP_SPLIT, src_key, src_sa);
            else { if (grouped) CAPS_SCATTER_LAUNCH(SRC_ARRAYS, MAP_GROUPED, src_key, src_sa);
                   else CAPS_SCATTER_LAUNCH(SRC_ARRAYS, MAP_LINEAR, src_key, src_sa); }
#undef CAPS_SCATTER_LAUNCH
#undef CAPS_SCATTER_LAUNCH_REC
            BackendEvent s1 = be.record();
            if (o.scatter_clock) { o.scatter_clock->spans.push_back({s0, s1}); o.scatter_clock->elems.push_back(n_elems); }
        };
        uint64_t out2[2] = {0, 0};
        auto adopt_buckets = [&]() {
            device_exclusive_scan<uint64_t>(be, bk.count, bk.nb_cap, bk.sub.seg_start, bk.scan_tmp);
        };
        const bool run_buckets = by_knots && o.need_lcp && o.final_sa && bk.skip && !std::getenv("CAPS_SA_NO_RUN_BUCKETS") &&
                                 n < (1ull << RunKey<(int)sizeof(idx_t)>::RB);
        auto bucket_tiles = [&]() {
            segs = bk.sub;
            segs.G = bk.nb_cap;
            uint64_t rl[1 + 4 * RUN_BUCKET_MAX];
            if (run_buckets) {
                const uint64_t NB = (uint64_t)(s.G / o.sub) * o.knots_per_parent;
                be.memset(bk.skip, 0, bk.nb_cap);
                be.memset(bk.run_list, 0, sizeof(uint64_t));
                CAPS_LAUNCH(run_bucket_mark_kernel, (uint32_t)((NB + 255) / 256), 256, be, o.knots, NB, o.knots_have_prev ? 1u : 0u, (uint32_t)BITS,
                            (const uint64_t*)bk.sub.seg_start, bk.skip, bk.run_list);
            }
            prepare_segments(be, segs, bk.tile_cap, bk.scan_tmp, bk.count, false, run_buckets ? bk.skip : nullptr);
            be.d2h(out2, segs.out2, sizeof out2);
            if (run_buckets) be.d2h(rl, bk.run_list, sizeof rl);
            be.sync();
            if (run_buckets) {
                const uint64_t cnt = rl[0] < RUN_BUCKET_MAX ? rl[0] : RUN_BUCKET_MAX;
                for (uint64_t j = 0; j < cnt; ++j) r.run_buckets.push_back({rl[2 + 4 * j], rl[3 + 4 * j], rl[4 + 4 * j]});
                std::sort(r.run_buckets.begin(), r.run_buckets.end(),
                          [](const typename SortResult<idx_t>::RunBucket& a, const typename SortResult<idx_t>::RunBucket& b) { return a.s0 < b.s0; });
                r.run_tables = o.run_tables ? *o.run_tables : bk.sub;
                r.run_bk = &bk;
                r.run_desc = desc;
                r.total = n_elems;
            }
        };
        const uint64_t nb_here = std::min<uint64_t>(bk.nb_cap, n_elems / BUCKET_TARGET + 2 * (uint64_t)(s.G / o.sub) + 2);
        const uint64_t slot_elems = nb_here * TILE_E;
        bool slots = false;
        if (by_knots && (from_text || runs)) throw std::invalid_argument("quantile buckets read (key, sa) arrays");
        if (o.k32 && (from_text || runs || by_knots || !o.speculate || !o.in_key || !o.final_sa))
            throw std::invalid_argument("32-bit keys: a slot split of (key32, sa) arrays with direct output");
        const bool can_slot = o.speculate && !by_knots &&
                              oth.region_bytes >= slot_elems * ((o.k32 ? sizeof(uint32_t) : sizeof(uint64_t)) + sizeof(idx_t)) &&
                              slot_elems + TILE_E < (uint64_t)std::numeric_limits<idx_t>::max();
        if (o.k32 && !can_slot) { r.failed = true; return r; }
        if (can_slot) {
            slot_key = oth.key;
            slot_sa = reinterpret_cast<idx_t*>(reinterpret_cast<char*>(oth.key) + slot_elems * sizeof(uint64_t));
            be.memset(bk.cursor, 0, (size_t)bk.nb_cap * sizeof(idx_t));
            if (o.k32) {
                slot_sa = reinterpret_cast<idx_t*>(reinterpret_cast<char*>(oth.key) + slot_elems * sizeof(uint32_t));
                BackendEvent s0 = be.record();
                CAPS_LAUNCH((bucket_scatter_kernel<idx_t, BITS, SRC_ARRAYS, MAP_LINEAR, uint32_t>), n_tiles, TILE_NT, be, psd, P, (uint64_t)0,
                            (uint64_t)0, reinterpret_cast<const uint32_t*>(o.in_key), src_sa, rsrc, (const BucketParams*)bk.params,
                            (const uint64_t*)bk.bstart, (const uint64_t*)nullptr, (uint64_t)TILE_E, static_cast<idx_t*>(bk.cursor),
                            reinterpret_cast<uint32_t*>(slot_key), slot_sa, (const BucketParams*)nullptr, (const uint32_t*)nullptr,
                            (const uint64_t*)nullptr, (const uint16_t*)nullptr, (const uint32_t*)nullptr, 1u, 0u, 1u, (const uint16_t*)nullptr,
                            Spill<idx_t>());
                BackendEvent s1 = be.record();
                if (o.scatter_clock) { o.scatter_clock->spans.push_back({s0, s1}); o.scatter_clock->elems.push_back(n_elems); }
            } else
            scatter(nullptr, TILE_E, slot_key, slot_sa);
            CAPS_LAUNCH((widen_kernel<idx_t>), (bk.nb_cap + 255) / 256, 256, be, (const idx_t*)static_cast<idx_t*>(bk.cursor),
                        (uint64_t)bk.nb_cap, bk.count);
            adopt_buckets();
            bucket_tiles();
            slots = out2[1] <= TILE_E;
            if (o.slot_stats) ++o.slot_stats[slots ? 0 : 1];
            if (o.k32 && !slots) { r.failed = true; return r; }
            if (dbg) std::fprintf(stderr, "[sort] slot split: largest bucket %llu -> %s\n", (unsigned long long)out2[1], slots ? "kept" : "redone");
        }
        if (by_knots && o.spill_slots && o.hot_tile_rec && !from_text && !runs && o.final_sa && o.final_lcp && o.need_lcp &&
            !std::getenv("CAPS_SA_NO_SPILL_SLOTS")) {
            const uint64_t NB = (uint64_t)(s.G / o.sub) * o.knots_per_parent;
            const uint64_t idx_max = (uint64_t)std::numeric_limits<idx_t>::max() - TILE_E - 1;
            char* lcp_lo = reinterpret_cast<char*>((reinterpret_cast<uintptr_t>(o.final_lcp) + 15) & ~uintptr_t(15));
            char* lcp_hi = reinterpret_cast<char*>(static_cast<idx_t*>(o.final_lcp) + n_elems);
            char* sa_lo = reinterpret_cast<char*>((reinterpret_cast<uintptr_t>(o.final_sa) + 15) & ~uintptr_t(15));
            char* sa_hi = reinterpret_cast<char*>(static_cast<idx_t*>(o.final_sa) + n_elems);
            uint64_t scap = 0;
            if (lcp_hi > lcp_lo + 64 && sa_hi > sa_lo + 64)
                scap = std::min<uint64_t>((uint64_t)(lcp_hi - lcp_lo) / sizeof(uint64_t), (uint64_t)(sa_hi - sa_lo - 32) / (2 * sizeof(idx_t) + sizeof(uint32_t)));
            const char* cap_env = std::getenv("CAPS_SA_TEST_SPILL_CAP");
            if (cap_env) scap = std::min<uint64_t>(scap, std::strtoull(cap_env, nullptr, 10));
            uint64_t cap_s = TILE_E;
            if (NB) cap_s = std::min<uint64_t>(cap_s, oth.region_bytes / (sizeof(uint64_t) + sizeof(idx_t)) / NB);
            const uint64_t want_stream = std::min<uint64_t>(scap, n_elems / 8 + 1024);
            if (NB && idx_max > want_stream) cap_s = std::min<uint64_t>(cap_s, (idx_max - want_stream) / NB);
            cap_s &= ~uint64_t(31);
            const char* slot_env = std::getenv("CAPS_SA_TEST_SPILL_SLOT");
            if (slot_env) cap_s = std::min<uint64_t>(cap_s, std::strtoull(slot_env, nullptr, 10));
            const uint64_t slot_total = NB * cap_s;
            if (slot_total < idx_max) scap = std::min<uint64_t>(scap, idx_max - slot_total);
            const bool fits = NB != 0 && NB <= bk.nb_cap && o.knots_per_parent <= BUCKET_LDS && (cap_env ? scap >= 1 : scap >= 1024) && slot_total < idx_max &&
                              (slot_env || cap_s >= (BUCKET_Q / 6) * 7) &&
                              oth.region_bytes >= slot_total * (sizeof(uint64_t) + sizeof(idx_t)) && bk.run_list;
            if (fits) {
                slot_key = oth.key;
                slot_sa = reinterpret_cast<idx_t*>(reinterpret_cast<char*>(oth.key) + slot_total * sizeof(uint64_t));
                Spill<idx_t> sp;
                sp.count = bk.run_list;
                sp.cap = scap;
                sp.base = slot_total;
                sp.key = reinterpret_cast<uint64_t*>(lcp_lo);
                sp.sa = reinterpret_cast<idx_t*>(sa_lo);
                sp.rel = sp.sa + scap;
                sp.bucket = reinterpret_cast<uint32_t*>(sp.rel + scap);
                const uint64_t fixed = (uint64_t)n_tiles * SPILL_CHUNK <= scap / 4 && !std::getenv("CAPS_SA_NO_SPILL_CHUNKS") ? (uint64_t)n_tiles * SPILL_CHUNK : 0;
                sp.chunk = fixed ? SPILL_CHUNK : 0u;
                be.memset(bk.cursor, 0, (size_t)bk.nb_cap * sizeof(idx_t));
                be.h2d(sp.count, &fixed, sizeof(uint64_t));
                if (fixed) be.memset(sp.bucket, 0xFF, (size_t)fixed * sizeof(uint32_t));
                BackendEvent s0 = be.record();
#define CAPS_SPILL_SCATTER_LAUNCH(REC_)                                                                                       \
                CAPS_LAUNCH((bucket_scatter_kernel<idx_t, BITS, SRC_ARRAYS, MAP_SPLIT, uint64_t, true, REC_>), n_tiles, TILE_NT, be, psd, P, (uint64_t)0, \
                            (uint64_t)0, src_key, src_sa, rsrc, (const BucketParams*)bk.params, (const uint64_t*)bk.bstart,         \
                            (const uint64_t*)nullptr, cap_s, static_cast<idx_t*>(bk.cursor), slot_key, slot_sa,                     \
                            (const BucketParams*)nullptr, (const uint32_t*)nullptr, o.knots, (const uint16_t*)nullptr,              \
                            (const uint32_t*)nullptr, 1u, o.knots_per_parent, o.sub, (const uint16_t*)nullptr, sp)
                if (rec_in) { if constexpr (sizeof(idx_t) == 4) CAPS_SPILL_SCATTER_LAUNCH(true); }
                else CAPS_SPILL_SCATTER_LAUNCH(false);
#undef CAPS_SPILL_SCATTER_LAUNCH
                uint64_t spilled = 0;
                be.d2h(&spilled, sp.count, sizeof spilled);
                CAPS_LAUNCH((widen_kernel<idx_t>), (bk.nb_cap + 255) / 256, 256, be, (const idx_t*)static_cast<idx_t*>(bk.cursor),
                            (uint64_t)bk.nb_cap, bk.count);
                adopt_buckets();
                bucket_tiles();
                slots = spilled <= scap;
                if (o.spill_stats) { ++o.spill_stats[slots ? 0 : 1]; o.spill_stats[2] += spilled; }
                if (dbg) std::fprintf(stderr, "[sort] split by knots with slots of %llu: %llu on the stream (room for %llu), largest bucket %llu -> %s\n",
                                      (unsigned long long)cap_s, (unsigned long long)spilled, (unsigned long long)scap, (unsigned long long)out2[1],
                                      slots ? "kept" : "redone");
                if (slots) {
                    const uint32_t ggrid_ = (uint32_t)std::min<uint64_t>((NB + 255) / 256, 16384);
                    CAPS_LAUNCH((spill_gather_kernel<idx_t>), ggrid_, 256, be, (const uint64_t*)bk.sub.seg_start, (uint32_t)NB, cap_s,
                                run_buckets ? (const uint8_t*)bk.skip : (const uint8_t*)nullptr, (const uint64_t*)slot_key, (const idx_t*)slot_sa,
                                cur.key, cur.sa);
                    if (spilled)
                        CAPS_LAUNCH((spill_place_kernel<idx_t>), (uint32_t)std::min<uint64_t>((spilled + 255) / 256, 16384), 256, be, sp, spilled,
                                    (const uint64_t*)bk.sub.seg_start, cur.key, cur.sa);
                    BackendEvent s1 = be.record();
                    if (o.scatter_clock) { o.scatter_clock->spans.push_back({s0, s1}); o.scatter_clock->elems.push_back(n_elems); }
                    slot_cap = (uint32_t)cap_s;
                } else {
                    BackendEvent s1 = be.record();
                    if (o.scatter_clock) { o.scatter_clock->spans.push_back({s0, s1}); o.scatter_clock->elems.push_back(n_elems); }
                }
            }
        }
        if (!slots) {
            const bool equalise = !by_knots && bk.fcount != nullptr && !o.no_equalise && !std::getenv("CAPS_SA_NO_EQUALISE");
            const BucketParams* cparams = bk.params;
            const uint64_t* cstart = bk.bstart;
            uint64_t* ccount = bk.count;
            if (equalise) {
                CAPS_LAUNCH(bucket_plan_kernel, (s.G + 255) / 256, 256, be, (const uint64_t*)s.seg_start, s_end, s.G, o.range_mode, o.pkey, o.part_off,
                            o.part_total ? o.part_total : s.G, 1u, EQ_FINE, o.sub, bk.fparams, bk.fsegB, o.gshift);
                CAPS_LAUNCH(scan_sizes_kernel, 1, 1024, be, (const uint64_t*)bk.fsegB, s.G, bk.fstart);
                be.memset(bk.fcount, 0, (size_t)EQ_FINE * bk.nb_cap * sizeof(uint64_t));
                cparams = bk.fparams;
                cstart = bk.fstart;
                ccount = bk.fcount;
            }
            be.memset(bk.count, 0, (size_t)bk.nb_cap * sizeof(uint64_t));
            be.memset(bk.cursor, 0, (size_t)bk.nb_cap * sizeof(idx_t));
            BackendEvent c0 = be.record();
            const uint64_t* no_tab = nullptr;
            if (from_text)
                CAPS_LAUNCH((bucket_count_kernel<idx_t, BITS, SRC_TEXT>), pgrid, TILE_NT, be, psd, P, n_words, tbase, (const uint64_t*)nullptr, rsrc,
                            cparams, cstart, ccount, no_tab, 0u, 1u, (uint16_t*)nullptr);
            else if (runs)
                CAPS_LAUNCH((bucket_count_kernel<idx_t, BITS, SRC_RUNS>), pgrid, TILE_NT, be, psd, P, n_words, tbase, src_key, rsrc,
                            cparams, cstart, ccount, no_tab, 0u, 1u, (uint16_t*)nullptr);
            else if (rec_in && by_knots) {
                if constexpr (sizeof(idx_t) == 4)
                    CAPS_LAUNCH((bucket_count_kernel<idx_t, BITS, SRC_ARRAYS, MAP_SPLIT, true>), pgrid, TILE_NT, be, psd, P, n_words, tbase, src_key,
                                rsrc, cparams, cstart, ccount, o.knots, o.knots_per_parent, o.sub, bid);
            } else if (rec_in) {
                if constexpr (sizeof(idx_t) == 4)
                    CAPS_LAUNCH((bucket_count_kernel<idx_t, BITS, SRC_ARRAYS, MAP_LINEAR, true>), pgrid, TILE_NT, be, psd, P, n_words, tbase, src_key,
                                rsrc, cparams, cstart, ccount, no_tab, 0u, 1u, (uint16_t*)nullptr);
            } else if (by_knots)
                CAPS_LAUNCH((bucket_count_kernel<idx_t, BITS, SRC_ARRAYS, MAP_SPLIT>), pgrid, TILE_NT, be, psd, P, n_words, tbase, src_key, rsrc,
                            cparams, cstart, ccount, o.knots, o.knots_per_parent, o.sub, bid);
            else
                CAPS_LAUNCH((bucket_count_kernel<idx_t, BITS, SRC_ARRAYS>), pgrid, TILE_NT, be, psd, P, n_words, tbase, src_key, rsrc,
                            cparams, cstart, ccount, no_tab, 0u, 1u, (uint16_t*)nullptr);
            if (equalise) {
                CAPS_LAUNCH(bucket_group_kernel, s.G < 16384 ? (s.G ? s.G : 1) : 16384, 256, be, s.G, (const uint64_t*)bk.segB, (const uint64_t*)bk.bstart,
                            (const uint64_t*)bk.fsegB, (const uint64_t*)bk.fstart, (const uint64_t*)bk.fcount, bk.count, bk.gfirst);
                CAPS_LAUNCH(bucket_ranges_kernel, (bk.nb_cap + 255) / 256, 256, be, (const uint64_t*)bk.bstart, s.G,
                            (const BucketParams*)bk.params, o.pkey, o.range_mode, o.part_off, o.part_total ? o.part_total : s.G, o.sub,
                            bk.tile_map, (const BucketParams*)bk.fparams, (const uint32_t*)bk.gfirst, o.gshift, bk.kshift);
            }
            BackendEvent c1 = be.record();
            if (o.count_clock) { o.count_clock->spans.push_back({c0, c1}); o.count_clock->elems.push_back(n_elems); }
            adopt_buckets();
            ElemBuf<idx_t> dst = from_text ? cur : oth;
            scatter((const uint64_t*)bk.sub.seg_start, 0u, dst.key, dst.sa, equalise);
            if (!from_text) {
                std::swap(cur, oth);
                r.buf[0] = cur;
                r.buf[1] = oth;
            }
            bucket_tiles();
        } else if (!slot_cap) {
            slot_cap = TILE_E;
            slot_grid = (uint32_t)nb_here;
        }

        mark("bucket scatter");
        n_tiles = (uint32_t)out2[0];
        max_len = out2[1];
        if (dbg) std::fprintf(stderr, "[sort] buckets: tiles %u max_len %llu\n", n_tiles, (unsigned long long)max_len);
        from_text = false;
        skip = true;
        r.skip_finished = true;
        r.segs = segs;
        r.n_tiles = n_tiles;
    }
    const SegDesc sd = segs.desc();
    SegDesc sd_hot = sd;
    if (slot_cap && max_len > slot_cap && o.hot_tile_rec) {
        CAPS_LAUNCH(hot_tiles_kernel, (n_tiles + 255) / 256, 256, be, sd, slot_cap, o.hot_tile_rec);
        sd_hot.tile_rec = o.hot_tile_rec;
    } else if (slot_cap && max_len > slot_cap) {
        throw std::invalid_argument("slots with outgrown buckets need room for the second tile table");
    }
    const uint32_t lcp_mode = o.need_lcp ? 1u : 0u;
    FinalOut<idx_t> fin;
    if (o.need_lcp && o.final_sa) {
        fin.sa = static_cast<idx_t*>(o.final_sa);
        fin.lcp = static_cast<idx_t*>(o.final_lcp);
        fin.first_key = o.bnd.first_key;
        fin.last_key = o.bnd.last_key;
        fin.first_sa = static_cast<idx_t*>(o.bnd.first_sa);
        fin.last_sa = static_cast<idx_t*>(o.bnd.last_sa);
    }
    r.fin = fin;
    uint32_t* redo = reinterpret_cast<uint32_t*>(desc);
    uint32_t* redo2 = redo + ((size_t)n_tiles + 2);
    uint32_t* redo3 = redo2 + ((size_t)n_tiles + 2);
    static_assert(sizeof(TileDesc) >= 3 * sizeof(uint32_t) + 1, "three queues fit the descriptor array");
    be.memset(redo, 0, sizeof(uint32_t));
    be.memset(redo2, 0, sizeof(uint32_t));
    be.memset(redo3, 0, sizeof(uint32_t));
    const uint32_t ggrid = n_tiles < 4 * be.persistent_blocks() ? n_tiles : 4 * be.persistent_blocks();
    const bool eq_tiles = !std::getenv("CAPS_SA_NO_EQ_TILES");
    const uint32_t drop = std::getenv("CAPS_SA_TEST_DROP_NOTE") ? 2u : 0u;
    if (!eq_tiles) redo3 = redo2 = redo;
    uint64_t* bflag = o.defer_flags && o.need_lcp && o.final_sa && !o.keys_only && !(o.k32 && slot_cap) ? o.defer_flags : nullptr;
    if (bflag) {
        be.memset(bflag, 0, (size_t)segs.G * sizeof(uint64_t));
        r.defer_flags = bflag;
        r.defer_desc = desc;
    }
    r.total = n_elems;
    r.cap = n_elems;
    auto defer_check = [&](uint32_t tiles_to_compare) {
        if (bflag && (uint64_t)tiles_to_compare * TILE_E > n_elems / 2) { bflag = nullptr; r.defer_flags = nullptr; }
    };
    BackendEvent t0 = be.record();
    if (o.seg_ends && segs.seg_start == s.seg_start)
        throw std::invalid_argument("segments in fixed-capacity regions must be bucketed (results are written compactly)");
    if (o.in_records && segs.seg_start == s.seg_start) throw std::invalid_argument("records are read by the bucket split only");
    const uint64_t* in_key = slot_cap ? slot_key : (o.in_key && segs.seg_start == s.seg_start) ? o.in_key : cur.key;
    const idx_t* in_sa = slot_cap ? slot_sa : (o.in_key && segs.seg_start == s.seg_start) ? static_cast<const idx_t*>(o.in_sa) : cur.sa;
    const uint8_t* no_shift = nullptr;
    r.k32 = o.k32 && slot_cap != 0;
    std::vector<uint64_t> dbg_ss;
    if (from_text) {
        CAPS_LAUNCH((tile_sort_kernel<idx_t, BITS, true>), n_tiles, TILE_NT, be, sd, P, n, o.text_base, lcp_mode, 0u,
                    (const uint64_t*)nullptr, (const idx_t*)nullptr, cur.key, cur.sa, cur.lcp, fin, seg_map, redo, no_shift);
        if (eq_tiles) CAPS_LAUNCH((tile_sort_eq_kernel<idx_t, BITS, true>), ggrid, TILE_NT, be, sd, P, n, o.text_base, lcp_mode, 0u,
                    (const uint64_t*)nullptr, (const idx_t*)nullptr, cur.key, cur.sa, cur.lcp, fin, seg_map, (const uint32_t*)redo, redo3, 0u | drop, redo2);
        if (eq_tiles) CAPS_LAUNCH((tile_sort_eq_kernel<idx_t, BITS, true, true>), ggrid, TILE_NT, be, sd, P, n, o.text_base, lcp_mode, 0u,
                    (const uint64_t*)nullptr, (const idx_t*)nullptr, cur.key, cur.sa, cur.lcp, fin, seg_map, (const uint32_t*)redo2, redo3, 0u, (uint32_t*)nullptr);
        CAPS_LAUNCH_RUNS(tile_sort_general_kernel, (idx_t, BITS, true), ggrid, TILE_NT, be, sd, P, n, o.text_base, lcp_mode, 0u,
                    (const uint64_t*)nullptr, (const idx_t*)nullptr, cur.key, cur.sa, cur.lcp, fin, (const uint32_t*)redo3, 0u, bflag);
    } else if (r.k32) {
        CAPS_LAUNCH((tile_sort_kernel<idx_t, BITS, false, uint32_t>), n_tiles, TILE_NT, be, sd, P, n, (uint64_t)0, lcp_mode, slot_cap,
                    reinterpret_cast<const uint32_t*>(in_key), in_sa, cur.key, cur.sa, cur.lcp, fin, seg_map, redo, (const uint8_t*)o.bk->kshift);
        if (eq_tiles) CAPS_LAUNCH((tile_sort_eq_kernel<idx_t, BITS, false>), ggrid, TILE_NT, be, sd, P, n, (uint64_t)0, lcp_mode, slot_cap,
                    (const uint64_t*)nullptr, in_sa, cur.key, cur.sa, cur.lcp, fin, (const BucketParams*)nullptr, (const uint32_t*)redo, redo3, 1u | drop, redo2);
        if (eq_tiles) CAPS_LAUNCH((tile_sort_eq_kernel<idx_t, BITS, false, true>), ggrid, TILE_NT, be, sd, P, n, (uint64_t)0, lcp_mode, slot_cap,
                    (const uint64_t*)nullptr, in_sa, cur.key, cur.sa, cur.lcp, fin, (const BucketParams*)nullptr, (const uint32_t*)redo2, redo3, 1u, (uint32_t*)nullptr);
        CAPS_LAUNCH_RUNS(tile_sort_general_kernel, (idx_t, BITS, false), ggrid, TILE_NT, be, sd, P, n, (uint64_t)0, lcp_mode, slot_cap,
                    (const uint64_t*)nullptr, in_sa, cur.key, cur.sa, cur.lcp, fin, (const uint32_t*)redo3, 1u, bflag);
    } else {
        const bool all_queued = o.skewed_keys && eq_tiles && !o.comparison_only;
        const bool per_tile = all_queued && (uint64_t)n_tiles * TILE_NT <= 0xFFFFFFFFull && !std::getenv("CAPS_SA_EQ_PERSISTENT");
        if (o.comparison_only) {
            CAPS_LAUNCH(queue_all_tiles_kernel, (n_tiles + 255) / 256, 256, be, sd, redo3);
            CAPS_LAUNCH_RUNS(tile_sort_general_kernel, (idx_t, BITS, false), ggrid, TILE_NT, be, sd, P, n, (uint64_t)0, lcp_mode, slot_cap,
                        in_key, in_sa, cur.key, cur.sa, cur.lcp, fin, (const uint32_t*)redo3, 0u, bflag);
        } else {
        bool by_bucket = false;
        if constexpr (sizeof(idx_t) == 4)
            by_bucket = (o.tile_chain & 1u) != 0 && !all_queued && slot_grid != 0 && slot_cap == TILE_E && max_len <= TILE_E &&
                        seg_map != nullptr && sd_hot.tile_rec == sd.tile_rec && slot_grid <= segs.G;
        if (o.tile_chain_used) *o.tile_chain_used = by_bucket ? 1u : 0u;
        if (dbg && !by_bucket && (o.tile_chain & 1u) != 0)
            std::fprintf(stderr, "[sort] table launch although the bucket-indexed one was asked for: idx bytes %u, all queued %d, slots %u of capacity %u "
                         "(a tile: %u), longest bucket %llu, bin maps %d, second tile table %d, segments %u\n", (unsigned)sizeof(idx_t), all_queued ? 1 : 0,
                         slot_grid, slot_cap, TILE_E, (unsigned long long)max_len, seg_map ? 1 : 0, sd_hot.tile_rec != sd.tile_rec ? 1 : 0, segs.G);
        if (dbg && by_bucket) {
            dbg_ss.resize((size_t)slot_grid + 1);
            be.d2h(dbg_ss.data(), segs.seg_start, dbg_ss.size() * sizeof(uint64_t));
            be.sync();
            const std::vector<uint64_t>& ss = dbg_ss;
            uint32_t last = 0, inner = 0, small = 0, cut = 0;
            uint64_t least = ~0ull;
            for (uint32_t g = 0; g < slot_grid; ++g) if (ss[g + 1] > ss[g]) last = g;
            for (uint32_t g = 0; g < last; ++g) inner += ss[g + 1] == ss[g] ? 1u : 0u;
            for (uint32_t g = 0; g <= last; ++g) {
                const uint64_t len = ss[g + 1] - ss[g];
                if (!len) continue;
                small += len < TILE_NT ? 1u : 0u;
                cut += len < (uint64_t)(TILE_EPT - 1) * TILE_NT ? 1u : 0u;
                least = len < least ? len : least;
            }
            std::fprintf(stderr, "[sort] bucket-indexed launch: %u slots for %u tiles, %u empty slots before the last full one (slot %u, %llu elements), "
                         "%u buckets below %u elements, %u below %u, smallest %llu\n", slot_grid, n_tiles, inner, last,
                         (unsigned long long)(ss[last + 1] - ss[last]), small, TILE_NT, cut, (TILE_EPT - 1) * TILE_NT, (unsigned long long)least);
        }
        if (all_queued && !per_tile) CAPS_LAUNCH(queue_all_tiles_kernel, (n_tiles + 255) / 256, 256, be, sd, redo);
        else if (by_bucket) {
            if constexpr (sizeof(idx_t) == 4)
                CAPS_LAUNCH((tile_sort_kernel<idx_t, BITS, false, uint64_t, 1>), slot_grid, TILE_NT, be, sd, P, n, (uint64_t)0, lcp_mode, slot_cap,
                            in_key, in_sa, cur.key, cur.sa, cur.lcp, fin, seg_map, redo, no_shift);
        } else if (!all_queued) CAPS_LAUNCH((tile_sort_kernel<idx_t, BITS, false>), n_tiles, TILE_NT, be, sd_hot, P, n, (uint64_t)0, lcp_mode, slot_cap,
                    in_key, in_sa, cur.key, cur.sa, cur.lcp, fin, seg_map, redo, no_shift);
        if (per_tile) {
            CAPS_LAUNCH((tile_sort_eq_kernel<idx_t, BITS, false, false, false>), n_tiles, TILE_NT, be, sd_hot, P, n, (uint64_t)0, lcp_mode, slot_cap,
                        in_key, in_sa, cur.key, cur.sa, cur.lcp, fin, seg_map, (const uint32_t*)nullptr, redo3, 0u | drop, redo2);
            uint32_t qn[2] = {0, 0};
            be.d2h(&qn[0], redo2, sizeof(uint32_t));
            be.d2h(&qn[1], redo3, sizeof(uint32_t));
            be.sync();
            if (qn[0]) CAPS_LAUNCH((tile_sort_eq_kernel<idx_t, BITS, false, true, false>), qn[0], TILE_NT, be, sd, P, n, (uint64_t)0, lcp_mode, slot_cap,
                        in_key, in_sa, cur.key, cur.sa, cur.lcp, fin, seg_map, (const uint32_t*)redo2, redo3, 0u, (uint32_t*)nullptr);
            const uint32_t ng = qn[0] + qn[1];
            if (bflag && qn[0]) {
                uint32_t q3 = 0;
                be.d2h(&q3, redo3, sizeof q3);
                be.sync();
                defer_check(q3);
            } else defer_check(qn[1]);
            if (ng && be.long_runs)
                CAPS_LAUNCH((tile_sort_general_kernel<idx_t, BITS, false, true, false>), ng, TILE_NT, be, sd, P, n, (uint64_t)0, lcp_mode, slot_cap,
                            in_key, in_sa, cur.key, cur.sa, cur.lcp, fin, (const uint32_t*)redo3, 0u, bflag);
            else if (ng)
                CAPS_LAUNCH((tile_sort_general_kernel<idx_t, BITS, false, false, false>), ng, TILE_NT, be, sd, P, n, (uint64_t)0, lcp_mode, slot_cap,
                            in_key, in_sa, cur.key, cur.sa, cur.lcp, fin, (const uint32_t*)redo3, 0u, bflag);
        } else {
            if (eq_tiles) CAPS_LAUNCH((tile_sort_eq_kernel<idx_t, BITS, false>), ggrid, TILE_NT, be, sd_hot, P, n, (uint64_t)0, lcp_mode, slot_cap,
                        in_key, in_sa, cur.key, cur.sa, cur.lcp, fin, seg_map, (const uint32_t*)redo, redo3, 0u | drop, redo2);
            if (eq_tiles) CAPS_LAUNCH((tile_sort_eq_kernel<idx_t, BITS, false, true>), ggrid, TILE_NT, be, sd, P, n, (uint64_t)0, lcp_mode, slot_cap,
                        in_key, in_sa, cur.key, cur.sa, cur.lcp, fin, seg_map, (const uint32_t*)redo2, redo3, 0u, (uint32_t*)nullptr);
            if (bflag) {
                uint32_t ng = 0;
                be.d2h(&ng, redo3, sizeof ng);
                be.sync();
                defer_check(ng);
            }
            CAPS_LAUNCH_RUNS(tile_sort_general_kernel, (idx_t, BITS, false), ggrid, TILE_NT, be, sd, P, n, (uint64_t)0, lcp_mode, slot_cap,
                        in_key, in_sa, cur.key, cur.sa, cur.lcp, fin, (const uint32_t*)redo3, 0u, bflag);
        }
        }
    }
    BackendEvent t1 = be.record();
    mark("tile sort");
    if (dbg) {
        uint32_t q[3] = {0, 0, 0};
        be.d2h(&q[0], redo, 4); be.d2h(&q[1], redo2, 4); be.d2h(&q[2], redo3, 4);
        be.sync();
        std::fprintf(stderr, "[sort] queues after the tile sorts: %u %u %u of %u tiles, deferring %d\n", q[0], q[1], q[2], n_tiles, bflag ? 1 : 0);
        if (!dbg_ss.empty()) {
            std::vector<uint32_t> qe(q[0]), slot_of_tile;
            if (q[0]) be.d2h(qe.data(), redo + 1, (size_t)q[0] * sizeof(uint32_t));
            be.sync();
            for (uint32_t g = 0; g + 1 < dbg_ss.size(); ++g) if (dbg_ss[g + 1] > dbg_ss[g]) slot_of_tile.push_back(g);
            uint32_t moved = 0, bad = 0;
            for (uint32_t t : qe) {
                if (t >= slot_of_tile.size()) ++bad;
                else if (slot_of_tile[t] != t) ++moved;
            }
            std::fprintf(stderr, "[sort] bucket-indexed launch: %u tiles queued, %u behind an empty slot, %u not tiles of the launch\n", q[0], moved, bad);
        }
    }
    if (o.tile_clock) { o.tile_clock->spans.push_back({t0, t1}); o.tile_clock->elems.push_back(n_elems); }
    const uint32_t grid = n_tiles < be.persistent_blocks() ? n_tiles : be.persistent_blocks();
    ElemBuf<idx_t> a = cur, b = oth;
    uint32_t* n_active = reinterpret_cast<uint32_t*>(desc + n_tiles);
    for (uint64_t R = TILE_E; R < max_len; R *= 2) {
        be.memset(n_active, 0, sizeof(uint32_t));
        CAPS_LAUNCH_RUNS(merge_partition_kernel, (idx_t, BITS), (n_tiles + 255) / 256, 256, be, sd, P, n, R, ~0ull, skip ? 1u : 0u,
                    lcp_mode, (const uint64_t*)a.key, (const idx_t*)a.sa, desc,
                    o.pass_counters ? o.pass_counters + r.passes : (uint64_t*)nullptr, bflag ? 1u : 0u, n_active);
        BackendEvent m0 = be.record();
        CAPS_LAUNCH_RUNS(merge_pass_kernel, (idx_t, BITS), grid, TILE_NT, be, (const TileDesc*)desc, (const uint32_t*)n_active, P, n,
                    (const uint64_t*)a.key, (const idx_t*)a.sa, b.key, b.sa, b.lcp, bflag);
        BackendEvent m1 = be.record();
        if (o.merge_clock) { o.merge_clock->spans.push_back({m0, m1}); o.merge_clock->elems.push_back(n_elems); }
        std::swap(a, b);
        ++r.passes;
        mark("merge pass");
    }
    if (o.unify && r.skip_finished && r.passes) {
        CAPS_LAUNCH((unify_kernel<idx_t>), n_tiles, 256, be, sd, (const uint64_t*)r.buf[1].key, (const idx_t*)r.buf[1].sa,
                    r.buf[0].key, r.buf[0].sa);
        r.unified = true;
    } else if (o.unify && r.skip_finished) {
        r.unified = true;
    }
    return r;
}

template <typename idx_t, int BITS>
void sort_run_buckets(Backend& be, const uint32_t* P, uint64_t n, const SortResult<idx_t>& r, idx_t* dSA, idx_t* dLCP)
{
    for (const auto& rb : r.run_buckets) {
        const uint64_t len = rb.s1 - rb.s0;
        const uint32_t grid = (uint32_t)std::min<uint64_t>((len + 255) / 256, 4096);
        SegBufs t = r.run_tables;
        t.G = 1;
        t.seg_end = nullptr;
        CAPS_LAUNCH(segment_range_kernel, 1, 64, be, t.seg_start, rb.s0, rb.s1);
        prepare_segments(be, t, tiles_of(len));
        CAPS_LAUNCH((run_rekey_kernel<idx_t, BITS>), grid, 256, be, P, n, rb.s0, rb.s1, rb.key, r.buf[0].key, (const idx_t*)r.buf[0].sa);
        SortOpts o;
        const SortResult<idx_t> rr = segmented_sort<idx_t, BITS>(be, P, n, r.run_desc, t, tiles_of(len), len, r.buf[0], r.buf[1], len, o);
        const ElemBuf<idx_t> res = rr.uniform();
        CAPS_LAUNCH((run_emit_kernel<idx_t, BITS>), grid, 256, be, P, n, rb.s0, rb.s1, r.total, (const uint64_t*)res.key, (const idx_t*)res.sa,
                    dSA, dLCP);
    }
}

constexpr uint32_t MSD_MAX_LEVELS = 128;
struct MsdArena {
    char* lo[2] = {nullptr, nullptr};
    char* hi[2] = {nullptr, nullptr};
    bool failed = false;
    template <typename T> T* head(size_t count, int pref = 0)
    {
        for (int k = 0; k < 2; ++k) {
            const int c = (pref + k) & 1;
            char* p = align_up(lo[c]);
            if (p && p + count * sizeof(T) <= hi[c]) { lo[c] = p + count * sizeof(T); return reinterpret_cast<T*>(p); }
        }
        failed = true;
        return nullptr;
    }
    template <typename T> T* tail(size_t count)
    {
        for (int c = 1; c >= 0; --c) {
            if (!hi[c]) continue;
            char* p = reinterpret_cast<char*>((reinterpret_cast<uintptr_t>(hi[c]) - count * sizeof(T)) & ~uintptr_t(255));
            if (p >= lo[c] && hi[c] - lo[c] >= (ptrdiff_t)(count * sizeof(T))) { hi[c] = p; return reinterpret_cast<T*>(p); }
        }
        failed = true;
        return nullptr;
    }
};

template <typename idx_t, int BITS>
bool msd_refine(Backend& be, const uint32_t* P, uint64_t n, const SortResult<idx_t>& r, idx_t* SA, idx_t* LCP)
{
    constexpr uint32_t KCH = TextTraits<BITS>::KCH;
    const SegDesc sd = r.segs.desc();
    const uint32_t n_tiles = r.n_tiles;
    const bool dbg = std::getenv("CAPS_SA_DEBUG") != nullptr;
// ... 134 lines not shown
    uint64_t *seg = segX, *gpos = gposX, *seg_n = segY, *gpos_n = gposY, *gdep = gdepX, *gdep_n = gdepY, *gpl = gplX, *gpl_n = gplY;
    uint32_t *gid = wgid, *gid_n = wgidY;
    const idx_t* in_sa = wsa0;
    uint64_t* kin = E1.key;
    uint64_t* flags = E1.key;
    uint64_t* offs = reinterpret_cast<uint64_t*>(E1.sa);
    uint32_t max_levels = MSD_MAX_LEVELS;
    if (const char* ml = std::getenv("CAPS_SA_TEST_MSD_MAX_LEVELS")) max_levels = (uint32_t)std::atoi(ml);
    while (nopen > 0) {
        if (r.msd_levels >= max_levels) return false;
        const uint32_t mg = (uint32_t)((m + 255) / 256);
        if (r.msd_levels) {
            const uint32_t gg = (uint32_t)std::min<uint64_t>((G + 255) / 256 + 1, 4ull * be.persistent_blocks());
            be.memset(gmin, 0, (size_t)G * sizeof(uint64_t));
            if (be.long_runs) CAPS_LAUNCH((msd_jump_kernel<idx_t, BITS, true>), mg, 256, be, P, n, m, (const uint64_t*)seg, (const uint32_t*)gid, (const uint8_t*)skip, in_sa, (const uint64_t*)gdep, (const uint64_t*)gpl, gmin);
            else CAPS_LAUNCH((msd_jump_kernel<idx_t, BITS, false>), mg, 256, be, P, n, m, (const uint64_t*)seg, (const uint32_t*)gid, (const uint8_t*)skip, in_sa, (const uint64_t*)gdep, (const uint64_t*)gpl, gmin);
            CAPS_LAUNCH(msd_jump_apply_kernel, gg, 256, be, (const uint64_t*)out3, (const uint8_t*)skip, (const uint64_t*)gmin, KCH, gdep);
        }
        CAPS_LAUNCH((msd_rekey_kernel<idx_t, BITS>), mg, 256, be, P, n, (const uint64_t*)gdep, m, (const uint32_t*)gid, (const uint8_t*)skip, in_sa, kin);
        {
            ls.seg_start = seg;
            ls.G = (uint32_t)G;
            const uint32_t lt = (uint32_t)std::min<uint64_t>(tiles_max, m / TILE_E + nopen + 1);
            prepare_segments(be, ls, lt, big_tmp, big_cnt, false, skip_tiles);
            SortOpts o;
            o.keys_only = true;
            o.comparison_only = true;
            o.skip_finished = true;
            o.unify = true;
            o.in_key = kin;
            o.in_sa = in_sa;
            const SortResult<idx_t> rr = segmented_sort<idx_t, BITS>(be, P, n, ldesc, ls, lt, gmax, E0, E1, m, o);
            if (rr.uniform().key != E0.key) return false;
        }
        CAPS_LAUNCH((msd_classify_kernel<idx_t, BITS>), mg, 256, be, n, (const uint64_t*)gdep, m, (const uint64_t*)seg, (const uint32_t*)gid, (const uint8_t*)skip,
                    (const uint64_t*)E0.key, (const idx_t*)E0.sa, (const uint64_t*)gpos, SA, LCP, flags);
        device_exclusive_scan<uint64_t>(be, flags, (uint32_t)m, offs, ltmp);
        CAPS_LAUNCH((msd_compact_kernel<idx_t>), mg, 256, be, m, (const uint64_t*)seg, (const uint32_t*)gid, (const idx_t*)E0.sa, (const uint64_t*)flags,
                    (const uint64_t*)offs, (const uint64_t*)gpos, E0.lcp, seg_n, gpos_n, gid_n, (const uint64_t*)gdep, gdep_n, KCH, gpl_n);
        CAPS_LAUNCH(msd_close_kernel, 1, 64, be, (const uint64_t*)(offs + m), seg_n, out3);
        D += KCH;
        ++r.msd_levels;
        std::swap(seg, seg_n);
        std::swap(gpos, gpos_n);
        std::swap(gid, gid_n);
        std::swap(gdep, gdep_n);
        std::swap(gpl, gpl_n);
        in_sa = E0.lcp;
        finish(seg, gpos, gdep, in_sa, gid, m);
        be.d2h(h3, out3, sizeof h3);
        be.sync();
        G = h3[0];
        m = h3[1];
        nopen = h3[2];
        gmax = h3[3];
        quick(seg, gpos, gdep, in_sa, h3 + 6);
        if (dbg) std::fprintf(stderr, "[msd] depth %llu: %llu groups of %llu members, %llu above %u finished in LDS, %llu above %u (largest %llu)\n", (unsigned long long)D,
                              (unsigned long long)G, (unsigned long long)m, (unsigned long long)(h3[6] + h3[7] + h3[8]), MSD_FIN_MAX, (unsigned long long)nopen,
                              MSD_QK_MAX, (unsigned long long)gmax);
        if (dbg && G <= Gm - 1) log_sizes(r.msd_levels, seg, gdep, G, h3 + 6);
        if (G > Gm - 1 || m > cap2 - 2) return false;
    }
    fix_edges();
    return true;
}

template <typename idx_t, int BITS>
void finalize(Backend& be, const uint32_t* P, uint64_t n, const SortResult<idx_t>& r, idx_t* dSA, idx_t* dLCP)
{
    if (r.n_tiles == 0) return;
    auto timed = [&](KernelClock* c, uint64_t elems, auto&& body) {
        if (!c) { body(); return; }
        const BackendEvent a = be.record();
        body();
        c->spans.push_back({a, be.record()});
        c->elems.push_back(elems);
    };
    timed(r.finish_clock, r.total, [&] {
        if (r.fin.sa == nullptr || r.passes > 0)
            CAPS_LAUNCH((finalize_kernel<idx_t, BITS>), r.n_tiles, 256, be, r.segs.desc(), P, n, r.pingpong(), r.skip_finished ? 1u : 0u,
                        r.passes & 1u, dSA, dLCP, r.fin);
        if (r.fin.sa != nullptr)
            CAPS_LAUNCH((head_lcp_kernel<idx_t, BITS>), (r.segs.G + 255) / 256, 256, be, P, n, (const uint64_t*)r.segs.seg_start, r.segs.G,
                        r.fin, r.k32 ? 1u : 0u);
    });
    if (!r.run_buckets.empty()) timed(r.runb_clock, 0, [&] { sort_run_buckets<idx_t, BITS>(be, P, n, r, dSA, dLCP); });
    if (r.defer_flags && !std::getenv("CAPS_SA_DEBUG_NO_MSD"))
        timed(r.msd_clock, 0, [&] { if (!msd_refine<idx_t, BITS>(be, P, n, r, dSA, dLCP)) r.msd_failed = true; });
}

inline int direct_shape(uint64_t n, uint32_t p, uint64_t m, uint32_t* PG, uint32_t* K1)
{
    *PG = *K1 = 0;
    if (p < 2 || n < 32ull * TILE_E || m < 64 || m > (1ull << 31)) return CAPS_SA_FB_SHAPE;
    const double group_max = 0.9 * (double)BUCKET_LDS * (double)BUCKET_TARGET;
    double want = std::sqrt((double)n / (double)BUCKET_TARGET);
    if (const char* k1 = std::getenv("CAPS_SA_DIRECT_K1")) { if (std::atof(k1) >= 2.0) want = std::atof(k1); }
    if (want > (double)BUCKET_LDS) want = (double)BUCKET_LDS;
    if ((double)n / group_max > want) want = (double)n / group_max;
    if (want < 2.0) want = 2.0;
    if (want > (double)BUCKET_LDS) return CAPS_SA_FB_SHAPE;
    uint32_t pg = (uint32_t)((double)p / want);
    if (pg < 1) pg = 1;
    const uint32_t k1 = (p + pg - 1) / pg;
    if (k1 < 2 || k1 > BUCKET_LDS || (double)n / k1 > group_max || m / k1 < 16) return CAPS_SA_FB_SHAPE;
    *PG = pg;
    *K1 = k1;
    return CAPS_SA_FB_NONE;
}


inline uint64_t test_stream_cap(uint64_t cap, uint64_t n_elems, uint64_t n_streams)
{
    const char* e = std::getenv("CAPS_SA_TEST_STREAM_CAP");
    if (!e || std::atof(e) <= 0.0 || n_streams == 0) return cap;
    const uint64_t c = (uint64_t)((double)n_elems / (double)n_streams * std::atof(e) / 100.0) + 2;
    return c < cap ? c & ~1ull : cap;
}

struct WaveSink {
    virtual void wave_done(Backend& be, uint64_t base, uint64_t cnt) = 0;
    virtual void reset(Backend& be) = 0;
    virtual void text(const uint32_t* P, const uint8_t* lut) {}
    virtual ~WaveSink() {}
};

template <typename idx_t> class Builder {
public:
    Builder(Backend& be, const Plan<idx_t>& pl) : be_(be), pl_(pl) {}
    void set_waves(uint32_t waves, WaveSink* sink, ElemBuf<idx_t> scratch = ElemBuf<idx_t>(), uint64_t scratch_elems = 0)
    {
        waves_ = waves ? waves : 1;
        sink_ = sink;
        wave_scratch_ = scratch;
        wave_scratch_elems_ = scratch_elems;
    }
    bool sink_served() const { return sink_served_; }

    void build(const uint8_t* dT, idx_t* dSA, idx_t* dLCP, caps_sa_stats* st, uint64_t max_context = 0)
    {
        const uint64_t n = pl_.n;
        if (st) { *st = caps_sa_stats(); st->n = n; st->idx_bytes = sizeof(idx_t); st->p_eff = pl_.p; }
        if (n == 0) return;
        BackendEvent e0 = be_.record();
        bits_ = prepare_text(be_, dT, n, pl_.P, pl_.present, pl_.lut, pl_.text_bits);
        BackendEvent e1 = be_.record();
        if (max_context != 0 && max_context < n) {
            if (pl_.p < 2 || pl_.ppp < 1) throw std::invalid_argument("bounded max_context needs n >= 32 and at least two subproblems (the reference is undefined below that)");
            if (bits_ == 2) run_bounded<2>(dSA, dLCP, max_context);
            else run_bounded<8>(dSA, dLCP, max_context);
            BackendEvent e2 = be_.record();
            be_.sync();
            if (st) {
                st->bits_per_char = (uint32_t)bits_;
                st->ppp = pl_.ppp;
                st->workspace_bytes = pl_.bytes;
                st->ms_pack = be_.elapsed_ms(e0, e1);
                st->ms_total = be_.elapsed_ms(e0, e2);
                st->ms_sort_subarrays = be_.elapsed_ms(e1, e2_);
                st->ms_select_pivots = be_.elapsed_ms(e2_, e3_);
                st->ms_locate_pivots = be_.elapsed_ms(e3_, e4_);
                st->ms_partition = be_.elapsed_ms(e4_, e5_);
                st->ms_merge_partitions = be_.elapsed_ms(e5_, e6_);
                st->ms_boundary_lcp = be_.elapsed_ms(e6_, e2);
                st->path_fallback = CAPS_SA_FB_BOUNDED;
            }
            be_.release_events();
            return;
        }
        if (bits_ == 2) run<2>(dSA, dLCP, st, e0, e1);
        else run<8>(dSA, dLCP, st, e0, e1);
    }

    int bits() const { return bits_; }

private:
    Backend& be_;
    const Plan<idx_t>& pl_;
    int bits_ = 0;
    uint32_t waves_ = 1;
    WaveSink* sink_ = nullptr;
    ElemBuf<idx_t> wave_scratch_;
    uint64_t wave_scratch_elems_ = 0;
    bool sink_served_ = false;
    uint32_t waves_used_ = 1;
    KernelClock merge_clock_;
    KernelClock tile_clock_;
    KernelClock scatter_clock_;
    KernelClock count_clock_;
    KernelClock collate_clock_;
    KernelClock finish_clock_, runb_clock_, msd_clock_;
    uint32_t pass_base_ = 0;
    uint32_t slot_stats_[2] = {0, 0};
    uint64_t spill_stats_[3] = {0, 0, 0};
    uint32_t passes1_ = 0, passes2_ = 0, passesS_ = 0;
    BackendEvent e2_, e3_, e4_, e5_, e6_, e7_, la0_, la1_;
    uint64_t max_part_ = 0;
    uint32_t path_direct_ = 0, path_fallback_ = 0, direct_groups_ = 0, direct_quantile_ = 0, direct_k32_ = 0, direct_records_ = 0, tile_chain_ = 0, scatter_issue_ = 0, run_buckets_ = 0;
    uint64_t direct_max_group_ = 0;
    uint64_t tie_groups_ = 0, tie_elems_ = 0;
    uint32_t tie_levels_ = 0;

    template <int BITS>
    SortResult<idx_t> seg_sort(const SegBufs& s, uint32_t n_tiles, uint64_t max_len, ElemBuf<idx_t> cur, ElemBuf<idx_t> oth,
                               uint64_t n_elems, SortOpts o, bool timed)
    {
        if (timed) {
            o.tile_clock = &tile_clock_;
            o.merge_clock = &merge_clock_;
            o.scatter_clock = &scatter_clock_;
            o.count_clock = &count_clock_;
            o.pass_counters = pl_.pass_elems + pass_base_;
            o.slot_stats = slot_stats_;
            o.speculate = std::getenv("CAPS_SA_NO_SLOTS") == nullptr && slot_stats_[1] == 0;
        }
        SortResult<idx_t> r = segmented_sort<idx_t, BITS>(be_, pl_.P, pl_.n, pl_.desc, s, n_tiles, max_len, cur, oth, n_elems, o);
        if (timed) {
            pass_base_ += r.passes;
            r.finish_clock = &finish_clock_;
            r.runb_clock = &runb_clock_;
            r.msd_clock = &msd_clock_;
        }
        return r;
    }
    void prepare_segments(const SegBufs& s, uint64_t tile_bound) { ::caps::prepare_segments(be_, s, tile_bound); }
    void set_final(SortOpts& o, idx_t* dSA, idx_t* dLCP)
    {
        o.final_sa = dSA;
        o.final_lcp = dLCP;
        o.bnd.first_key = pl_.bk.first_key;
        o.bnd.last_key = pl_.bk.last_key;
        o.bnd.first_sa = pl_.bk.first_sa;
        o.bnd.last_sa = pl_.bk.last_sa;
    }

    static uint32_t tree_depth(uint64_t cnt) { uint32_t d = 0; while ((1ull << d) < cnt) ++d; return d; }
    template <int BITS>
    void run_bounded(idx_t* dSA, idx_t* dLCP, uint64_t ctx)
    {
        const uint64_t n = pl_.n, s = n / pl_.p, last = s + n % pl_.p, m = pl_.ppp, nsamp = pl_.m;
        const uint32_t p = pl_.p;
        idx_t *SAw = pl_.A.sa, *LCPw = pl_.A.lcp;
        idx_t *pivot = pl_.SA_.sa, *pw = pl_.SB_.sa, *t1 = pl_.SA_.lcp, *t2 = pl_.SB_.lcp;
        idx_t *Pm = pl_.Pm, *ruler = pl_.PmT;
        uint64_t* scan = pl_.seg2.seg_start;
        const uint32_t* P = pl_.P;
        auto grid = [](uint64_t threads) { return capped_grid((threads + 255) / 256, 256); };
        CAPS_LAUNCH((bounded_init_kernel<idx_t>), grid(n), 256, be_, n, (const idx_t*)nullptr, dSA, SAw, dLCP, LCPw);
        for (uint32_t d = tree_depth(last); d-- > 0;)
            CAPS_LAUNCH((bounded_sort_level_kernel<idx_t, BITS>), grid((uint64_t)p << d), 256, be_, P, n, ctx, n, p, s, d, dSA, dLCP, SAw, LCPw);
        e2_ = be_.record();
        CAPS_LAUNCH((bounded_sample_kernel<idx_t>), grid((uint64_t)p * m), 256, be_, (const idx_t*)dSA, n, p, s, m, pivot);
        CAPS_LAUNCH((bounded_init_kernel<idx_t>), grid(nsamp), 256, be_, nsamp, (const idx_t*)pivot, pw, pivot, t1, t2);
        for (uint32_t d = tree_depth(nsamp); d-- > 0;)
            CAPS_LAUNCH((bounded_sort_level_kernel<idx_t, BITS>), grid(1ull << d), 256, be_, P, n, ctx, nsamp, 1u, nsamp, d, pw, t1, pivot, t2);
        CAPS_LAUNCH((bounded_sample_kernel<idx_t>), grid(p - 1), 256, be_, (const idx_t*)pw, nsamp, 1u, nsamp, (uint64_t)(p - 1), pivot);
        e3_ = be_.record();
        CAPS_LAUNCH((bounded_locate_kernel<idx_t, BITS>), grid((uint64_t)p * (p + 1)), 256, be_, P, n, ctx, p, s, (const idx_t*)dSA, (const idx_t*)pivot, Pm);
        e4_ = be_.record();
        CAPS_LAUNCH((bounded_ruler_kernel<idx_t>), (p + 255) / 256, 256, be_, p, (const idx_t*)Pm, ruler, pl_.sizes);
        CAPS_LAUNCH(scan_sizes_kernel, 1, 1024, be_, (const uint64_t*)pl_.sizes, p, scan);
        CAPS_LAUNCH((bounded_collate_kernel<idx_t>), grid(n), 256, be_, n, p, s, (const uint64_t*)scan, (const idx_t*)ruler, (const idx_t*)Pm,
                    (const idx_t*)dSA, (const idx_t*)dLCP, SAw, LCPw);
        be_.d2d(dSA, SAw, n * sizeof(idx_t));
        be_.d2d(dLCP, LCPw, n * sizeof(idx_t));
        e5_ = be_.record();
        for (uint32_t d = tree_depth(p); d-- > 0;)
            CAPS_LAUNCH((bounded_partition_level_kernel<idx_t, BITS>), grid((uint64_t)p << d), 256, be_, P, n, ctx, p, (const uint64_t*)scan,
                        (const idx_t*)ruler, d, dSA, dLCP, SAw, LCPw);
        e6_ = be_.record();
        CAPS_LAUNCH((bounded_boundary_kernel<idx_t, BITS>), (p + 255) / 256, 256, be_, P, n, p, (const uint64_t*)scan, (const idx_t*)dSA, dLCP);
    }

    template <int BITS>
    void run_classic(idx_t* dSA, idx_t* dLCP)
    {
        const uint64_t n = pl_.n;
        const uint32_t p = pl_.p;
        const uint64_t s = n / p, last = s + n % p;
        CAPS_LAUNCH(uniform_segments_kernel, (p + 256) / 256, 256, be_, pl_.seg1.seg_start, p, s, n);
        const uint32_t n_tiles1 = (p - 1) * tiles_of(s) + tiles_of(last);
// ... 110 lines not shown
        o2.skip_finished = true;
        o2.bk = &pl_.bk;
        o2.range_mode = 1;
        o2.pkey = pl_.pkey;
        if (fused) o2.runs = &rsrc;
        set_final(o2, dSA, dLCP);
        SortResult<idx_t> r2 = seg_sort<BITS>(pl_.seg2, n_tiles2, max_part_, in2, out2buf, n, o2, true);
        passes2_ = r2.passes;
        e6_ = be_.record();

        finalize<idx_t, BITS>(be_, pl_.P, n, r2, dSA, dLCP);
        e7_ = be_.record();
    }

    template <int BITS>
    bool run_direct(idx_t* dSA, idx_t* dLCP, uint32_t PG, uint32_t K1, BackendEvent e1, bool allow_k32 = true, bool defer = true)
    {
        const uint64_t n = pl_.n, m = pl_.m;
        const uint32_t p = pl_.p;
        CAPS_LAUNCH((sample_text_kernel<idx_t, BITS>), (uint32_t)((m + 255) / 256), 256, be_, (const uint32_t*)pl_.P, (uint64_t)0, n, m,
                    pl_.SA_.key, pl_.SA_.sa);
        CAPS_LAUNCH(uniform_segments_kernel, 1, 256, be_, pl_.segS.seg_start, 1u, m, m);
        prepare_segments(pl_.segS, tiles_of(m));
        SortOpts os;
        os.bk = &pl_.bk;
        os.unify = true;
        os.keys_only = true;
        SortResult<idx_t> rs = seg_sort<BITS>(pl_.segS, tiles_of(m), m, pl_.SA_, pl_.SB_, m, os, false);
        passesS_ = rs.passes;
        ElemBuf<idx_t> smp = rs.uniform();
        CAPS_LAUNCH((pick_pivots_kernel<idx_t>), (p + 255) / 256, 256, be_, (const uint64_t*)smp.key, (const idx_t*)smp.sa,
                    m, p, pl_.pkey, pl_.psa);
        be_.memset(pl_.dstat, 0, 4 * sizeof(uint64_t));
        uint32_t* dflag = reinterpret_cast<uint32_t*>(pl_.dstat + 2);
        CAPS_LAUNCH(group_keys_kernel, (p + 255) / 256, 256, be_, (const uint64_t*)pl_.pkey, p, PG, K1, pl_.gkey, dflag);
        CAPS_LAUNCH(skew_probe_kernel, (p + 255) / 256, 256, be_, (const uint64_t*)pl_.pkey, p, PG, K1, dflag + 2);
        uint32_t probe[4];
        be_.d2h(probe, dflag, sizeof probe);
        be_.sync();

        const ElemBuf<idx_t>& A = pl_.A;
        const uint32_t n_tilesA = tiles_of(n);
        const char* sub_env = std::getenv("CAPS_SA_DIRECT_SUB");
        uint32_t SUB = (n + GA_E - 1) / GA_E >= 32ull * DIRECT_SUB ? DIRECT_SUB : 1u;
        if (sub_env && std::atoi(sub_env) >= 1 && (uint32_t)std::atoi(sub_env) <= DIRECT_SUB) SUB = (uint32_t)std::atoi(sub_env);
        const uint32_t n_streams = K1 * SUB;
        uint64_t capA = A.region_bytes / ((sizeof(uint64_t) + sizeof(idx_t)) * (uint64_t)n_streams);
        const uint64_t idx_max = (uint64_t)std::numeric_limits<idx_t>::max() - TILE_E;
        if (capA > idx_max / n_streams) capA = idx_max / n_streams;
        capA = test_stream_cap(capA, n, n_streams);
        uint64_t* a_key = A.key;

        const char* mode_env = std::getenv("CAPS_SA_DIRECT_MODE");
        bool quantile = probe[0] != 0 || probe[2] != 0;
        if (mode_env && std::string(mode_env) == "linear") quantile = false;
        if (mode_env && std::string(mode_env) == "quantile") quantile = true;
        const uint64_t NBt = (n + BUCKET_Q - 1) / BUCKET_Q;
        const uint32_t KPG = (uint32_t)((NBt + K1 - 1) / K1);
        const uint64_t NB = (uint64_t)K1 * KPG;
        uint64_t m2 = NB * QUANTILE_SPB;
        if (m2 > n / 4) m2 = n / 4;
        if (quantile && (KPG < 2 || KPG > BUCKET_LDS || NB > pl_.bk.nb_cap || m2 < 8 * NB || m2 > (1ull << 31))) quantile = false;
        if (quantile && probe[3] > p / 4) { path_fallback_ = CAPS_SA_FB_PIVOT_TIES; return false; }
        if (!quantile && probe[0] != 0) { path_fallback_ = CAPS_SA_FB_PIVOT_TIES; return false; }
        uint64_t *rstart = nullptr, *rcap = nullptr;
        direct_quantile_ = quantile ? 1u : 0u;
        const char* keys_env = std::getenv("CAPS_SA_KEYS");
        const bool k32 = allow_k32 && !quantile && BITS == 2 && keys_env && std::string(keys_env) == "32";
        direct_k32_ = k32 ? 1u : 0u;
        idx_t* a_sa = reinterpret_cast<idx_t*>(reinterpret_cast<char*>(A.key) + (uint64_t)n_streams * capA * (k32 ? sizeof(uint32_t) : sizeof(uint64_t)));
        const char* la = std::getenv("CAPS_SA_LEVEL_A");
        const bool big_tiles = k32 || !(la && std::string(la) == "tile");
        const char* rec_env = std::getenv("CAPS_SA_RECORDS");
        const uint32_t rec_want = rec_env ? (uint32_t)std::atoi(rec_env) : DIRECT_RECORDS_DEFAULT;
        const bool rec_a = (rec_want & 1u) != 0 && sizeof(idx_t) == 4 && !k32 && big_tiles;
        direct_records_ = rec_a ? 1u : 0u;
        const char* chain_env = std::getenv("CAPS_SA_TILE_CHAIN");
        const uint32_t chain_want = chain_env ? (uint32_t)std::atoi(chain_env) : DIRECT_TILE_CHAIN_DEFAULT;
        tile_chain_ = 0;
        const char* issue_env = std::getenv("CAPS_SA_SCATTER_ISSUE");
        const bool may_wave = !(k32 || waves_ < 2 || !wave_scratch_.key);
        const uint32_t issue_want = rec_a && !quantile && !may_wave ? (issue_env ? (uint32_t)std::atoi(issue_env) : DIRECT_SCATTER_ISSUE_DEFAULT) & 1u : 0u;
        scatter_issue_ = 0;
        if (k32) CAPS_LAUNCH(group_shift_kernel, (K1 + 255) / 256, 256, be_, (const uint64_t*)pl_.gkey, K1, pl_.gshift);
        if (quantile) {
            CAPS_LAUNCH((sample_text_kernel<idx_t, BITS>), (uint32_t)((m2 + 255) / 256), 256, be_, (const uint32_t*)pl_.P, (uint64_t)0, n, m2,
                        pl_.A.key, pl_.A.sa);
            SegBufs sseg = pl_.seg1;
            sseg.G = 1;
            CAPS_LAUNCH(uniform_segments_kernel, 1, 256, be_, sseg.seg_start, 1u, m2, m2);
            prepare_segments(sseg, tiles_of(m2));
            SortOpts oq;
            oq.bk = &pl_.bk;
            oq.unify = true;
            oq.knots = pl_.gkey;
            oq.knots_per_parent = K1;
            oq.skewed_keys = probe[2] != 0;
            oq.keys_only = true;
            SortResult<idx_t> rq = seg_sort<BITS>(sseg, tiles_of(m2), m2, pl_.A, pl_.B, m2, oq, false);
            ElemBuf<idx_t> smp2 = rq.uniform();
            CAPS_LAUNCH(knots_kernel, (uint32_t)((NB + 255) / 256), 256, be_, (const uint64_t*)smp2.key, m2, NB, KPG, K1, pl_.knots, pl_.gkey);
            rstart = pl_.rstart;
            rcap = pl_.rcap;
            const uint64_t token = 2 * GA_E / K1 + 16;
            if (capA <= 2 * token) { path_fallback_ = CAPS_SA_FB_SHAPE; direct_quantile_ = 0; return false; }
            CAPS_LAUNCH(group_caps_kernel, (K1 + 255) / 256, 256, be_, (const uint64_t*)pl_.knots, NB, KPG, K1, SUB, capA - token, token, rcap);
            CAPS_LAUNCH(scan_sizes_kernel, 1, 1024, be_, (const uint64_t*)rcap, n_streams, rstart);
        }
        CAPS_LAUNCH(split_lut_kernel, (SPLIT_LUT_CELLS + 256) / 256, 256, be_, (const uint64_t*)pl_.gkey, K1 - 1, pl_.glut, dflag + 1);
        e3_ = be_.record();

        CAPS_LAUNCH(uniform_segments_kernel, 1, 256, be_, pl_.seg1.seg_start, 1u, n, n);
        SegBufs whole = pl_.seg1;
        whole.G = 1;
        prepare_segments(whole, n_tilesA);
        BucketParams one = make_bucket_params(0, ~0ull, K1);
        const uint64_t b01[2] = {0, K1};
        be_.h2d(pl_.bk.params, &one, sizeof one);
        be_.h2d(pl_.bk.bstart, b01, sizeof b01);
        be_.memset(pl_.dcur, 0, (size_t)n_streams * sizeof(idx_t));
        {
            BackendEvent s0 = be_.record();
            if (k32)
                CAPS_LAUNCH((group_scatter_kernel<idx_t, BITS, uint32_t>), (uint32_t)((n + GA_E - 1) / GA_E), TILE_NT, be_, (const uint32_t*)pl_.P,
                            packed_words(n, BITS), (uint64_t)0, n, (const uint64_t*)pl_.gkey, K1, (const uint16_t*)pl_.glut,
                            (const uint32_t*)(dflag + 1), SUB, capA, pl_.dcur, reinterpret_cast<uint32_t*>(a_key), a_sa, 0u, 1u,
                            (const uint64_t*)rstart, (const uint64_t*)rcap, (const uint8_t*)pl_.gshift, 0u, K1);
            else if (rec_a) {
                if constexpr (sizeof(idx_t) == 4)
                    CAPS_LAUNCH((group_scatter_kernel<idx_t, BITS, uint64_t, true>), (uint32_t)((n + GA_E - 1) / GA_E), TILE_NT, be_,
                                (const uint32_t*)pl_.P, packed_words(n, BITS), (uint64_t)0, n, (const uint64_t*)pl_.gkey, K1,
                                (const uint16_t*)pl_.glut, (const uint32_t*)(dflag + 1), SUB, capA, pl_.dcur, a_key, a_sa, 0u, 1u,
                                (const uint64_t*)rstart, (const uint64_t*)rcap, (const uint8_t*)nullptr, 0u, K1);
            } else if (big_tiles)
                CAPS_LAUNCH((group_scatter_kernel<idx_t, BITS>), (uint32_t)((n + GA_E - 1) / GA_E), TILE_NT, be_, (const uint32_t*)pl_.P,
                            packed_words(n, BITS), (uint64_t)0, n, (const uint64_t*)pl_.gkey, K1, (const uint16_t*)pl_.glut,
                            (const uint32_t*)(dflag + 1), SUB, capA, pl_.dcur, a_key, a_sa, 0u, 1u, (const uint64_t*)rstart, (const uint64_t*)rcap,
                            (const uint8_t*)nullptr, 0u, K1);
            else
                CAPS_LAUNCH((bucket_scatter_kernel<idx_t, BITS, SRC_TEXT, MAP_SPLIT>), n_tilesA, TILE_NT, be_, whole.desc(), (const uint32_t*)pl_.P,
                            packed_words(n, BITS), (uint64_t)0, (const uint64_t*)nullptr, (const idx_t*)nullptr, RunSrc<idx_t>(),
                            (const BucketParams*)pl_.bk.params, (const uint64_t*)pl_.bk.bstart, (const uint64_t*)nullptr, capA,
                            pl_.dcur, a_key, a_sa, (const BucketParams*)nullptr, (const uint32_t*)nullptr,
                            (const uint64_t*)pl_.gkey, (const uint16_t*)pl_.glut, (const uint32_t*)(dflag + 1), SUB, 0u, 1u, (const uint16_t*)nullptr,
                            Spill<idx_t>());
            BackendEvent s1 = be_.record();
            scatter_clock_.spans.push_back({s0, s1});
            scatter_clock_.elems.push_back(n);
            la0_ = s0;
            la1_ = s1;
        }
        SegBufs groups = pl_.seg2;
        groups.G = n_streams;
        CAPS_LAUNCH((slot_segments_kernel<idx_t>), (n_streams + 256) / 256, 256, be_, (const idx_t*)pl_.dcur, K1, SUB, big_tiles ? 1u : 0u, capA,
                    (const uint64_t*)rstart, (const uint64_t*)rcap, groups.seg_start, groups.seg_end, pl_.dstat);
        ::caps::prepare_segments(be_, groups, n / TILE_E + n_streams + 1, nullptr, nullptr, true);
        uint64_t out2[2], dstat[4];
        uint32_t W = (k32 || waves_ < 2 || !wave_scratch_.key) ? 1u : std::min<uint32_t>(waves_, K1);
        std::vector<idx_t> h_cur;
        if (W > 1) {
            h_cur.resize(n_streams);
            be_.d2h(h_cur.data(), pl_.dcur, (size_t)n_streams * sizeof(idx_t));
        }
        be_.d2h(out2, groups.out2, sizeof out2);
        be_.d2h(dstat, pl_.dstat, sizeof dstat);
        be_.sync();
// ... 15 lines not shown
            }
            std::fprintf(stderr, "[direct] level B input: %llu streams, %llu full tiles, last tiles that end in load", (unsigned long long)used,
                         (unsigned long long)full);
            for (uint32_t k = 0; k < TILE_EPT; ++k) std::fprintf(stderr, " %u: %llu", k + 1, (unsigned long long)tail[k]);
            std::fprintf(stderr, " (tiles of %u, %u threads)\n", TILE_E, TILE_NT);
        }
        e2_ = e1;
        e4_ = e3_;
        e5_ = be_.record();

        SortOpts o2;
        o2.need_lcp = true;
        o2.skip_finished = true;
        o2.bk = &pl_.bk;
        o2.range_mode = 1;
        o2.pkey = pl_.gkey;
        o2.part_total = K1;
        o2.sub = SUB;
        o2.seg_ends = true;
        if (quantile) {
            o2.knots = pl_.knots;
            o2.knots_per_parent = KPG;
            o2.in_extent = (uint64_t)n_streams * capA;
            o2.spill_slots = spill_stats_[1] == 0;
            o2.spill_stats = spill_stats_;
            o2.hot_tile_rec = pl_.seg1.tile_rec;
        }
        o2.skewed_keys = quantile && probe[2] != 0 && !std::getenv("CAPS_SA_TRY_LINEAR_TILES");
        if (k32) { o2.k32 = true; o2.range_mode = 2; o2.gshift = pl_.gshift; }
        o2.in_key = a_key;
        o2.in_sa = a_sa;
        o2.in_records = rec_a;
        if (defer && !k32 && !std::getenv("CAPS_SA_NO_DEFER")) o2.defer_flags = pl_.bk.fcount;
        o2.run_tables = &pl_.seg1;
        passes2_ = 0;
        run_buckets_ = 0;
        tie_groups_ = tie_elems_ = 0;
        tie_levels_ = 0;
        std::vector<uint32_t> wave_end;
        if (W > 1) {
            auto group_size = [&](uint32_t g) {
                uint64_t z = 0;
                for (uint32_t x = 0; x < SUB; ++x) { const uint32_t s = g * SUB + x; z += (uint64_t)h_cur[big_tiles ? (size_t)(s % SUB) * K1 + s / SUB : s]; }
                return z;
            };
            const uint64_t target = std::min<uint64_t>((n + W - 1) / W, wave_scratch_elems_);
            uint64_t acc = 0;
            for (uint32_t g = 0; g < K1; ++g) {
                const uint64_t z = group_size(g);
                if (z > wave_scratch_elems_) { wave_end.clear(); break; }
                if (acc && acc + z > target) { wave_end.push_back(g); acc = 0; }
                acc += z;
                if (g + 1 == K1) wave_end.push_back(K1);
            }
            W = wave_end.empty() ? 1u : (uint32_t)wave_end.size();
        }
        uint64_t base = 0;
        for (uint32_t w = 0; w < W; ++w) {
            const uint32_t g0 = W > 1 && w ? wave_end[w - 1] : 0u, g1 = W > 1 ? wave_end[w] : K1;
            SegBufs gw = groups;
            uint32_t n_tiles_w = (uint32_t)out2[0];
            uint64_t max_len_w = out2[1], elems_w = n;
            SortOpts ow = o2;
            if (W > 1) {
                gw.seg_start = groups.seg_start + (size_t)g0 * SUB;
                gw.seg_end = groups.seg_end + (size_t)g0 * SUB;
                gw.G = (g1 - g0) * SUB;
                elems_w = 0;
                max_len_w = 0;
                uint64_t tiles = 0;
                for (uint32_t s = g0 * SUB; s < g1 * SUB; ++s) {
                    const uint64_t z = (uint64_t)h_cur[big_tiles ? (size_t)(s % SUB) * K1 + s / SUB : s];
                    elems_w += z;
                    max_len_w = std::max(max_len_w, z);
                    tiles += (z + TILE_E - 1) / TILE_E;
                }
                n_tiles_w = (uint32_t)tiles;
                ::caps::prepare_segments(be_, gw, tiles + 1, nullptr, nullptr, true);
                ow.part_off = g0;
                if (quantile) { ow.knots = pl_.knots + (size_t)g0 * KPG; ow.knots_have_prev = g0 > 0; }
            }
            set_final(ow, dSA + base, dLCP + base);
            if (W == 1) { ow.tile_chain = chain_want; ow.tile_chain_used = &tile_chain_; }
            ow.scatter_issue = issue_want;
            ow.scatter_issue_used = &scatter_issue_;
            if (elems_w) {
                SortResult<idx_t> r2 = seg_sort<BITS>(gw, n_tiles_w, max_len_w, W > 1 ? wave_scratch_ : pl_.A, pl_.B, elems_w, ow, true);
                if (r2.failed) {
                    if (sink_) sink_->reset(be_);
                    return run_direct<BITS>(dSA, dLCP, PG, K1, e1, false, defer);
                }
                passes2_ = std::max(passes2_, r2.passes);
                run_buckets_ += (uint32_t)r2.run_buckets.size();
                finalize<idx_t, BITS>(be_, pl_.P, n, r2, dSA + base, dLCP + base);
                if (r2.msd_failed) {
                    if (sink_) sink_->reset(be_);
                    return run_direct<BITS>(dSA, dLCP, PG, K1, e1, allow_k32, false);
                }
                tie_groups_ += r2.msd_groups;
                tie_elems_ += r2.msd_elems;
                tie_levels_ = std::max(tie_levels_, r2.msd_levels);
                if (base) CAPS_LAUNCH((wave_head_lcp_kernel<idx_t, BITS>), 1, 64, be_, (const uint32_t*)pl_.P, n, (const idx_t*)dSA, dLCP, base);
            }
            if (sink_ && elems_w) sink_->wave_done(be_, base, elems_w);
            base += elems_w;
        }
        sink_served_ = sink_ != nullptr;
        waves_used_ = W;
        e6_ = be_.record();
        e7_ = be_.record();
        return true;
    }

    template <int BITS>
    void run(idx_t* dSA, idx_t* dLCP, caps_sa_stats* st, BackendEvent e0, BackendEvent e1)
    {
        const uint64_t n = pl_.n;
        const uint32_t p = pl_.p;
        be_.memset(pl_.pass_elems, 0, kMaxPasses * sizeof(uint64_t));

        if (p < 2) {
            CAPS_LAUNCH(uniform_segments_kernel, 1, 256, be_, pl_.seg1.seg_start, 1u, n, n);
            prepare_segments(pl_.seg1, tiles_of(n));
            SortOpts o;
            o.from_text = true;
            o.need_lcp = true;
            o.bk = &pl_.bk;
            set_final(o, dSA, dLCP);
            SortResult<idx_t> r = seg_sort<BITS>(pl_.seg1, tiles_of(n), n, pl_.A, pl_.B, n, o, true);
            passes1_ = r.passes;
            e2_ = e3_ = e4_ = e5_ = e6_ = be_.record();
            finalize<idx_t, BITS>(be_, pl_.P, n, r, dSA, dLCP);
            e7_ = be_.record();
        } else {
            uint32_t PG = 0, K1 = 0;
            const char* force = std::getenv("CAPS_SA_PATH");
            if (force && std::string(force) == "classic") path_fallback_ = CAPS_SA_FB_FORCED;
            else path_fallback_ = (uint32_t)direct_shape(n, p, pl_.m, &PG, &K1);
            if (path_fallback_ == CAPS_SA_FB_NONE && run_direct<BITS>(dSA, dLCP, PG, K1, e1)) path_direct_ = 1;
            else {
                run_classic<BITS>(dSA, dLCP);
            }
        }
        uint64_t pass_elems[kMaxPasses];
        be_.d2h(pass_elems, pl_.pass_elems, sizeof pass_elems);
        BackendEvent e8 = be_.record();
        be_.sync();

        if (st) {
            st->bits_per_char = BITS;
            st->long_runs = be_.long_runs ? 1u : 0u;
            st->ppp = pl_.ppp;
            st->max_partition = max_part_;
            st->merge_passes_phase1 = passes1_;
            st->merge_passes_phase2 = passes2_;
            st->merge_passes_samples = passesS_;
            st->workspace_bytes = pl_.bytes;
            st->ms_pack = be_.elapsed_ms(e0, e1);
            st->ms_sort_subarrays = be_.elapsed_ms(e1, e2_);
            st->ms_select_pivots = be_.elapsed_ms(e2_, e3_);
            st->ms_locate_pivots = be_.elapsed_ms(e3_, e4_);
            st->ms_partition = be_.elapsed_ms(e4_, e5_);
            st->ms_merge_partitions = be_.elapsed_ms(e5_, e6_);
            st->ms_boundary_lcp = be_.elapsed_ms(e6_, e7_);
            st->ms_output = be_.elapsed_ms(e7_, e8);
            st->ms_total = be_.elapsed_ms(e0, e8);
            auto sum = [&](KernelClock& c, double* ms, uint64_t* launches, uint64_t* elems) {
                for (size_t i = 0; i < c.spans.size(); ++i) {
                    *ms += be_.elapsed_ms(c.spans[i].first, c.spans[i].second);
                    *elems += c.elems[i];
                }
                *launches = c.spans.size();
            };
            sum(merge_clock_, &st->merge_pass_ms, &st->merge_pass_launches, &st->merge_pass_elems);
            sum(tile_clock_, &st->tile_sort_ms, &st->tile_sort_launches, &st->tile_sort_elems);
            uint64_t dummy_l = 0, dummy_e = 0;
            sum(scatter_clock_, &st->bucket_scatter_ms, &st->bucket_scatter_launches, &st->bucket_scatter_elems);
            sum(count_clock_, &st->bucket_count_ms, &dummy_l, &dummy_e);
            sum(collate_clock_, &st->collate_ms, &dummy_l, &dummy_e);
            sum(finish_clock_, &st->finish_ms, &dummy_l, &dummy_e);
            sum(runb_clock_, &st->run_bucket_ms, &dummy_l, &dummy_e);
            sum(msd_clock_, &st->msd_ms, &dummy_l, &dummy_e);
            st->path_direct = path_direct_;
            st->path_fallback = path_fallback_;
            st->direct_groups = direct_groups_;
            st->direct_quantile = direct_quantile_;
            st->run_buckets = run_buckets_;
            st->tie_groups_deferred = tie_groups_;
            st->tie_elems_deferred = tie_elems_;
            st->tie_levels = tie_levels_;
            st->result_waves = sink_served_ ? waves_used_ : 1u;
            st->n_devices = 1;
            st->direct_key_bits = path_direct_ && direct_k32_ ? 32u : 64u;
            st->direct_records = path_direct_ ? direct_records_ : 0u;
            st->tile_chain = path_direct_ ? tile_chain_ : 0u;
            st->scatter_issue = path_direct_ ? scatter_issue_ : 0u;
            st->direct_max_group = direct_max_group_;
            st->level_a_ms = direct_groups_ ? be_.elapsed_ms(la0_, la1_) : 0.0;
            st->slot_splits = slot_stats_[0];
            st->slot_splits_redone = slot_stats_[1];
            st->knot_slot_splits = (uint32_t)spill_stats_[0];
            st->knot_slot_splits_redone = (uint32_t)spill_stats_[1];
            st->spill_entries = spill_stats_[2];
            st->merge_pass_elems = 0;
            for (uint32_t i = 0; i < pass_base_ && i < kMaxPasses; ++i) st->merge_pass_elems += pass_elems[i];
        }
        be_.release_events();
    }
};

}
```

include/caps_sa_hip.h:

```cpp
#ifndef CAPS_SA_HIP_H
#define CAPS_SA_HIP_H

#include <stdint.h>
#include <stddef.h>

#ifdef __cplusplus
extern "C" {
#endif

#define CAPS_SA_OK 0
#define CAPS_SA_EINVAL (-1)
#define CAPS_SA_EUNSUPPORTED (-2)
#define CAPS_SA_EHIP (-3)
#define CAPS_SA_ENOMEM (-4)
#define CAPS_SA_ENODEVICE (-5)
#define CAPS_SA_EALPHABET (-6)

typedef struct caps_sa_stats {
    uint64_t n;
    uint32_t idx_bytes;
    uint32_t p_eff;
    uint32_t ppp;
    uint32_t bits_per_char;
    uint32_t merge_passes_phase1, merge_passes_phase2, merge_passes_samples;
    uint32_t long_runs;
    uint64_t max_partition;
    uint64_t workspace_bytes;
    double ms_total;
    double ms_pack;
    double ms_sort_subarrays;
    double ms_select_pivots;
    double ms_locate_pivots;
    double ms_partition;
    double ms_merge_partitions;
    double ms_boundary_lcp;
    double ms_output;
    double ms_h2d, ms_d2h;
    double merge_pass_ms;  uint64_t merge_pass_launches;  uint64_t merge_pass_elems;
    double tile_sort_ms;   uint64_t tile_sort_launches;   uint64_t tile_sort_elems;
    double bucket_scatter_ms; uint64_t bucket_scatter_launches; uint64_t bucket_scatter_elems;
    double bucket_count_ms;
    double collate_ms;
    uint32_t slot_splits, slot_splits_redone;
    uint32_t path_direct, path_fallback;
    uint32_t direct_groups;
    uint32_t direct_quantile;
    uint64_t direct_max_group;
    double level_a_ms;
    uint32_t direct_key_bits;
    uint32_t run_buckets;
    uint32_t result_waves;
    uint32_t n_devices;
    double ms_upload_max, ms_upload_min;
    double ms_device_build_max, ms_device_build_min;
    double ms_download_max, ms_download_min;
    uint64_t tie_groups_deferred, tie_elems_deferred;
    uint32_t tie_levels;
    uint32_t lcp_bytes_on_link;
    double finish_ms, run_bucket_ms, msd_ms;
    uint32_t knot_slot_splits, knot_slot_splits_redone;
    uint64_t spill_entries;
    uint32_t direct_records;
    uint32_t tile_chain;
    uint32_t scatter_issue;
} caps_sa_stats;

uint32_t caps_sa_hip_stats_bytes(void);
uint32_t caps_sa_hip_shard_info_bytes(void);

#define CAPS_SA_FB_NONE 0
#define CAPS_SA_FB_FORCED 1
#define CAPS_SA_FB_SHAPE 2
#define CAPS_SA_FB_LONG_RUNS 3
#define CAPS_SA_FB_PIVOT_TIES 4
#define CAPS_SA_FB_GROUP_OVERFLOW 5
#define CAPS_SA_FB_KEY32 6
#define CAPS_SA_FB_BOUNDED 7

int caps_sa_hip_device_count(void);
const char* caps_sa_hip_last_error(void);
const char* caps_sa_hip_version(void);

void caps_sa_hip_release_cache(void);

void* caps_sa_hip_host_alloc(uint64_t bytes);
void caps_sa_hip_host_free(void* p);

int caps_sa_hip_gen_rand_seq(uint32_t seed, uint64_t n, char* out);

int caps_sa_hip_workspace_bytes(uint64_t n, uint64_t subproblem_count, int idx_bytes, uint64_t* bytes);
int caps_sa_hip_workspace_bytes_ex(uint64_t n, uint64_t subproblem_count, int idx_bytes, int bits_per_char, uint64_t* bytes);

int caps_sa_hip_build_u32(const char* T, uint64_t n, uint64_t subproblem_count, uint64_t max_context,
                          uint32_t* SA, uint32_t* LCP, int device, caps_sa_stats* stats);
int caps_sa_hip_build_u64(const char* T, uint64_t n, uint64_t subproblem_count, uint64_t max_context,
                          uint64_t* SA, uint64_t* LCP, int device, caps_sa_stats* stats);

int caps_sa_hip_build_multi_u32(const char* T, uint64_t n, uint64_t subproblem_count, uint64_t max_context,
                                uint32_t* SA, uint32_t* LCP, const int* devices, int n_devices, caps_sa_stats* stats);
int caps_sa_hip_build_multi_u64(const char* T, uint64_t n, uint64_t subproblem_count, uint64_t max_context,
                                uint64_t* SA, uint64_t* LCP, const int* devices, int n_devices, caps_sa_stats* stats);

int caps_sa_hip_build_device_u32(const void* dT, uint64_t n, uint64_t subproblem_count, uint64_t max_context,
                                 void* dSA, void* dLCP, void* workspace, uint64_t workspace_bytes,
                                 void* hip_stream, caps_sa_stats* stats);
int caps_sa_hip_build_device_u64(const void* dT, uint64_t n, uint64_t subproblem_count, uint64_t max_context,
                                 void* dSA, void* dLCP, void* workspace, uint64_t workspace_bytes,
                                 void* hip_stream, caps_sa_stats* stats);

int caps_sa_hip_verify_device_u32(const void* dT, uint64_t n, const void* dSA, const void* dLCP,
                                  void* hip_stream, uint64_t* n_errors);
int caps_sa_hip_verify_device_u64(const void* dT, uint64_t n, const void* dSA, const void* dLCP,
                                  void* hip_stream, uint64_t* n_errors);

int caps_sa_hip_verify_slice_device_u32(const void* dT, uint64_t n, const void* dSA, const void* dLCP, uint64_t cnt,
                                        int is_head, void* hip_stream, uint64_t* n_errors);
int caps_sa_hip_verify_slice_device_u64(const void* dT, uint64_t n, const void* dSA, const void* dLCP, uint64_t cnt,
                                        int is_head, void* hip_stream, uint64_t* n_errors);


int caps_sa_hip_bwt_device_u32(const void* dT, uint64_t n, const void* dSA, uint64_t first, uint64_t cnt,
                               void* dBWT, void* hip_stream, uint64_t* primary);
int caps_sa_hip_bwt_device_u64(const void* dT, uint64_t n, const void* dSA, uint64_t first, uint64_t cnt,
                               void* dBWT, void* hip_stream, uint64_t* primary);
int caps_sa_hip_build_bwt_u32(const char* T, uint64_t n, uint64_t subproblem_count, uint64_t max_context,
                              uint32_t* SA, uint32_t* LCP, uint8_t* BWT, uint64_t* primary, int device, caps_sa_stats* stats);
int caps_sa_hip_build_bwt_u64(const char* T, uint64_t n, uint64_t subproblem_count, uint64_t max_context,
                              uint64_t* SA, uint64_t* LCP, uint8_t* BWT, uint64_t* primary, int device, caps_sa_stats* stats);


int caps_sa_hip_inverse_bwt_workspace_bytes(uint64_t n, int idx_bytes, uint64_t* bytes);
int caps_sa_hip_inverse_bwt_device_u32(const void* dBWT, uint64_t n, uint64_t primary, void* dT,
                                       void* workspace, uint64_t workspace_bytes, void* hip_stream);
int caps_sa_hip_inverse_bwt_device_u64(const void* dBWT, uint64_t n, uint64_t primary, void* dT,
                                       void* workspace, uint64_t workspace_bytes, void* hip_stream);
int caps_sa_hip_inverse_bwt_u32(const uint8_t* BWT, uint64_t n, uint64_t primary, char* T, int device);
int caps_sa_hip_inverse_bwt_u64(const uint8_t* BWT, uint64_t n, uint64_t primary, char* T, int device);


int caps_sa_hip_fm_index_bytes(uint64_t n, uint32_t sa_sample, int idx_bytes, uint64_t* bytes);
int caps_sa_hip_fm_build_device_u32(const void* dBWT, uint64_t n, uint64_t primary, const void* dSA, uint32_t sa_sample,
                                    void* dIndex, uint64_t index_bytes, void* hip_stream);
int caps_sa_hip_fm_build_device_u64(const void* dBWT, uint64_t n, uint64_t primary, const void* dSA, uint32_t sa_sample,
                                    void* dIndex, uint64_t index_bytes, void* hip_stream);
int caps_sa_hip_fm_build_u32(const uint8_t* BWT, uint64_t n, uint64_t primary, const uint32_t* SA, uint32_t sa_sample,
                             void* index, uint64_t index_bytes, int device);
int caps_sa_hip_fm_build_u64(const uint8_t* BWT, uint64_t n, uint64_t primary, const uint64_t* SA, uint32_t sa_sample,
// ... 245 lines not shown
```

Measured before the change: 76.43 billion.

## Pack slot keys and suffix indices into 64-bit records for bucket-indexed sort

The bucket scatter now writes one 64-bit record per element, holding a 32-bit shifted key relative to the bucket base plus the suffix index, instead of separate key and index arrays. The tile sort rebuilds the full key from the bucket's kmin and per-bucket shift, and starts tie LCPs from the reduced key width. A separate unpack kernel writes indices back for tiles that need the slot arrays. This cuts slot-array traffic and LDS use in the scatter, at the cost of extra unpack work, deeper LCP scans on truncated-key ties, and a debug tie-count pass.

New measurement: 81.01 billion, median of 6. 1.06x the previous value.

```diff
diff --git a/caps-sa_amd/_binding.py b/caps-sa_amd/_binding.py
--- a/caps-sa_amd/_binding.py
+++ b/caps-sa_amd/_binding.py
@@ -74,6 +74,7 @@
         ("direct_records", ctypes.c_uint32),
         ("tile_chain", ctypes.c_uint32),
         ("scatter_issue", ctypes.c_uint32),
+        ("slot_keys", ctypes.c_uint32),
     ]
 
     def as_dict(self) -> dict:
diff --git a/caps-sa_amd/csrc/kernels.h b/caps-sa_amd/csrc/kernels.h
--- a/caps-sa_amd/csrc/kernels.h
+++ b/caps-sa_amd/csrc/kernels.h
@@ -567,6 +567,29 @@
     const uint32_t b = caps_umul32hi(d32, bp.m) >> bp.post;
     return b < bp.B ? b : bp.B - 1;
 }
+
+HD uint32_t slot_key_shift(uint64_t range, uint32_t B)
+{
+    const uint64_t w = range / (B ? B : 1u);
+    const uint32_t bl = w == ~0ull ? 65u : 64u - (uint32_t)caps_clz64(w + 1);
+    return bl > 30u ? bl - 30u : 0u;
+}
+HD uint64_t slot_key_base(uint64_t l, uint32_t s)
+{
+    if (30u + s >= 64u) return 0;
+    const uint64_t m = 1ull << (30u + s);
+    return l > m ? l - m : 0;
+}
+HD uint64_t slot_key_restore(uint64_t base, uint32_t s, uint32_t r)
+{
+    const uint64_t bs = base >> s;
+    return (bs + (uint32_t)(r - (uint32_t)bs)) << s;
+}
+DEV_INLINE uint32_t slot_kshift_of(const uint8_t* __restrict__ kshift, uint32_t g)
+{
+    return (reinterpret_cast<const uint32_t*>(kshift)[g >> 2] >> (8u * (g & 3u))) & 0xFFu;
+}
+HD uint64_t slot_rec(uint64_t key, uint32_t s, uint32_t sa) { return ((uint64_t)sa << 32) | (uint32_t)(key >> s); }
 
 template <uint32_t NBINS>
 DEV_INLINE void block_exclusive_scan(KCTX uint32_t* h)
@@ -669,6 +692,14 @@
     return pair_lcp32<BITS, RUNS>(P, n, ka, (uint64_t)a, kb, (uint64_t)b, cs);
 }
 
+template <int BITS, typename idx_t>
+DEV_INLINE uint64_t slot_pair_lcp(const uint32_t* __restrict__ P, uint64_t n, uint64_t ka, idx_t a, uint64_t kb, idx_t b, uint32_t from)
+{
+    const uint64_t x = ka ^ kb;
+    if (x) return lcp_capped<idx_t>((uint32_t)caps_clz64(x) / BITS, n, a, b);
+    return deep_lcp<BITS, false>(P, n, (uint64_t)a, (uint64_t)b, from);
+}
+
 template <typename idx_t> HD idx_t tie_sentinel() { return (idx_t)~(idx_t)0; }
 template <int BITS, bool RUNS, typename idx_t>
 DEV_INLINE uint64_t deferring_pair_lcp(const uint32_t* __restrict__ P, uint64_t n, uint64_t* __restrict__ bflag, uint32_t g, uint64_t ka, idx_t a,
@@ -821,7 +852,7 @@
         }                                                                                                       \
     }
 
-template <typename idx_t, int BITS, bool FROM_TEXT, typename KT = uint64_t, int CHAIN = 0>
+template <typename idx_t, int BITS, bool FROM_TEXT, typename KT = uint64_t, int CHAIN = 0, bool SLOTREC = false>
 GLOBAL_FN LAUNCH_BOUNDS2(TILE_NT, TILE_WAVES_PER_SIMD) tile_sort_kernel(KCTX SegDesc sd, const uint32_t* __restrict__ P, uint64_t n,
                                                   uint64_t text_base, uint32_t lcp_mode, uint32_t slot_cap, const KT* in_key,
                                                   const idx_t* in_sa, uint64_t* out_key, idx_t* out_sa, idx_t* out_lcp,
@@ -835,20 +866,23 @@
     constexpr uint32_t CHAIN_EARLY = BY_BUCKET ? TILE_EPT - 1 : 0u;
     static_assert(!K32 || !FROM_TEXT, "32-bit keys come from the slots of level B");
     static_assert(!BY_BUCKET || (!FROM_TEXT && !K32 && sizeof(idx_t) == 4), "bucket-indexed: 64-bit keys and 32-bit indices in slots");
+    static_assert(!SLOTREC || (BY_BUCKET && BITS == 2), "records of slot keys: the bucket-indexed build on 2-bit texts");
     TL_DECL(KT, rk, TILE_EPT);
     TL_DECL(idx_t, rs, TILE_EPT);
     uint64_t bs0 = 0, bs1 = 0;
     BucketParams tb_early = BucketParams();
+    uint32_t ks_early = 0;
     if (BY_BUCKET) {
         bs0 = sd.seg_start[K_BLOCK_IDX];
         bs1 = sd.seg_start[K_BLOCK_IDX + 1];
         tb_early = seg_map[K_BLOCK_IDX];
+        if (SLOTREC) ks_early = slot_kshift_of(kshift, K_BLOCK_IDX);
         PAR(tid) {
             const uint64_t in0e = (uint64_t)K_BLOCK_IDX * slot_cap;
             UNROLL
             for (uint32_t k = 0; k < CHAIN_EARLY; ++k) {
                 TL(rk, tid, k) = STREAM_LOAD(&in_key[in0e + tid + k * TILE_NT]);
-                TL(rs, tid, k) = STREAM_LOAD(&in_sa[in0e + tid + k * TILE_NT]);
+                if (!SLOTREC) TL(rs, tid, k) = STREAM_LOAD(&in_sa[in0e + tid + k * TILE_NT]);
             }
         }
         ISSUE_FENCE();
@@ -864,7 +898,9 @@
     const bool direct = with_lcp && fin.sa != nullptr;
     const uint64_t in0 = slot_cap ? (uint64_t)g * slot_cap : start;
     const uint32_t TILE_KEY_SHIFT = K32 ? kshift[g] : 0u;
-    const uint32_t tie_from = K32 ? (TILE_KEY_SHIFT + 32u) / BITS : TextTraits<BITS>::KCH;
+    const uint32_t tie_from = K32       ? (TILE_KEY_SHIFT + 32u) / BITS
+                              : SLOTREC ? (64u - ks_early) / BITS
+                                        : TextTraits<BITS>::KCH;
     SHARED_ARRAY(KT, skey, TILE_E);
     SHARED_ARRAY(idx_t, ssa, TILE_E);
     SHARED_ARRAY(uint32_t, hist, TILE_BINS + 1);
@@ -886,7 +922,7 @@
                 const uint32_t e = tid + k * TILE_NT;
                 if (e < cnt) {
                     TL(rk, tid, k) = STREAM_LOAD(&in_key[in0 + e]);
-                    TL(rs, tid, k) = STREAM_LOAD(&in_sa[in0 + e]);
+                    if (!SLOTREC) TL(rs, tid, k) = STREAM_LOAD(&in_sa[in0 + e]);
                 }
             }
         }
@@ -894,6 +930,18 @@
         TILE_SORT_LOAD
     }
     TILE_SORT_RANGE_(BY_BUCKET ? tb_early : seg_map[g])
+    if (SLOTREC) {
+        const uint64_t kbase = slot_key_base(tb.kmin, ks_early);
+        PAR(tid) {
+            UNROLL
+            for (uint32_t k = 0; k < TILE_EPT; ++k) {
+                if (k >= CHAIN_EARLY && tid + k * TILE_NT >= cnt) continue;
+                const uint64_t rec = (uint64_t)TL(rk, tid, k);
+                TL(rs, tid, k) = (idx_t)(rec >> 32);
+                TL(rk, tid, k) = (KT)slot_key_restore(kbase, ks_early, (uint32_t)rec);
+            }
+        }
+    }
     PHASE_MARK(0);
     bool fast = cnt > 1 && tb.range > 0;
     if (fast) {
@@ -985,7 +1033,11 @@
                     const KT key = skey[sl];
                     const idx_t sa = ssa[sl];
                     uint64_t l = 0;
-                    if (with_lcp && e) { const uint32_t sp = perm[e - 1]; l = TILE_EMIT_LCP_(skey[sp], ssa[sp], key, sa); }
+                    if (with_lcp && e) {
+                        const uint32_t sp = perm[e - 1];
+                        if (SLOTREC) l = slot_pair_lcp<BITS, idx_t>(P, n, (uint64_t)skey[sp], ssa[sp], (uint64_t)key, sa, tie_from);
+                        else l = TILE_EMIT_LCP_(skey[sp], ssa[sp], key, sa);
+                    }
                     if (direct) {
                         STREAM_STORE(&fin.sa[start + e], sa);
                         STREAM_STORE(&fin.lcp[start + e], (idx_t)l);
@@ -1025,6 +1077,39 @@
         const uint32_t i = K_BLOCK_IDX * K_BLOCK_DIM + tid;
         if (i < nt) redo[1 + i] = i;
         if (i == 0) redo[0] = nt;
+    }
+}
+
+GLOBAL_FN LAUNCH_BOUNDS(256) slot_unpack_kernel(KCTX SegDesc sd, const uint32_t* __restrict__ redo, uint32_t slot_cap,
+                                                const uint64_t* __restrict__ rec, uint32_t* __restrict__ out_sa)
+{
+    const uint32_t n_redo = redo[0];
+    for (uint32_t qi = K_BLOCK_IDX; qi < n_redo; qi += K_GRID_DIM) {
+        const TileInfo t = tile_info(sd, redo[1 + qi]);
+        const uint64_t len = t.s1 - t.s0, in0 = (uint64_t)t.g * slot_cap;
+        const uint32_t cnt = (uint32_t)(len < slot_cap ? len : slot_cap);
+        PAR(tid) {
+            for (uint32_t i = tid; i < cnt; i += K_BLOCK_DIM) out_sa[in0 + i] = (uint32_t)(rec[in0 + i] >> 32);
+        }
+    }
+}
+
+template <typename idx_t, int BITS>
+GLOBAL_FN LAUNCH_BOUNDS(256) slot_tie_count_kernel(KCTX const uint32_t* __restrict__ P, const uint64_t* __restrict__ seg_start, uint32_t G,
+                                                   const uint8_t* __restrict__ kshift, const idx_t* __restrict__ sa,
+                                                   uint64_t* __restrict__ count)
+{
+    for (uint32_t g = K_BLOCK_IDX; g < G; g += K_GRID_DIM) {
+        const uint64_t s0 = seg_start[g], s1 = seg_start[g + 1];
+        const uint32_t s = kshift[g];
+        PAR(tid) {
+            uint64_t c = 0;
+            for (uint64_t i = s0 + 1 + tid; i < s1; i += K_BLOCK_DIM)
+                c += (window64<BITS>(P, (uint64_t)sa[i - 1]) >> s) == (window64<BITS>(P, (uint64_t)sa[i]) >> s) ? 1u : 0u;
+            if (c) ATOMIC_ADD_U64(count, c);
+            if (tid == 0 && s1 > s0 && s0 > 0 && (window64<BITS>(P, (uint64_t)sa[s0 - 1]) >> s) == (window64<BITS>(P, (uint64_t)sa[s0]) >> s))
+                ATOMIC_ADD_U64(count + 1, 1ull);
+        }
     }
 }
 
@@ -2329,7 +2414,7 @@
                                                   uint32_t range_mode, uint32_t part_off, uint32_t part_total, uint32_t sub,
                                                   BucketParams* __restrict__ tile_map,
                                                   const BucketParams* __restrict__ fbps, const uint32_t* __restrict__ gfirst,
-                                                  const uint8_t* __restrict__ gshift, uint8_t* __restrict__ kshift)
+                                                  const uint8_t* __restrict__ gshift, uint8_t* __restrict__ kshift, uint32_t slot_keys)
 {
     PAR(tid) {
         const uint64_t i = (uint64_t)K_BLOCK_IDX * K_BLOCK_DIM + tid;
@@ -2348,6 +2433,7 @@
                 if (j + 1 < part_total) kmax = pkey[j];
                 if (range_mode == 2) { key32_range(kmin, kmax, j > 0, gshift[j]); kshift[i] = gshift[j]; }
             }
+            if (slot_keys && range_mode != 2) kshift[i] = (uint8_t)slot_key_shift(bp.range, bp.B);
             const uint32_t bk = (uint32_t)(i - bstart[g]);
             const double range1 = (double)(kmax - kmin) + 1.0;
             uint64_t l = kmin, h = kmax;
@@ -2524,7 +2610,8 @@
 constexpr uint32_t SPILL_LONG_CAP = TILE_E / SPILL_LONG;
 constexpr uint32_t SPILL_CHUNK = TILE_E / 128 ? TILE_E / 128 : 1;
 
-template <typename idx_t, int BITS, int SRC, int MAP, typename KT = uint64_t, bool SPILL = false, bool REC_IN = false, bool ISSUE = false>
+template <typename idx_t, int BITS, int SRC, int MAP, typename KT = uint64_t, bool SPILL = false, bool REC_IN = false, bool ISSUE = false,
+          bool SLOT32 = false>
 GLOBAL_FN LAUNCH_BOUNDS(TILE_NT) bucket_scatter_kernel(KCTX SegDesc sd, const uint32_t* __restrict__ P, uint64_t n_words,
                                                        uint64_t text_base, const KT* __restrict__ in_key,
                                                        const idx_t* __restrict__ in_sa, RunSrc<idx_t> rsrc,
@@ -2554,6 +2641,7 @@
     const uint64_t start = t.s0 + (uint64_t)t.tl * TILE_E;
     const uint32_t cnt = (uint32_t)(t.s1 - start < TILE_E ? t.s1 - start : TILE_E);
     static_assert(!ISSUE || (REC_IN && MAP == MAP_LINEAR && !SPILL), "loads first: the records of level A under the linear map");
+    static_assert(!SLOT32 || (ISSUE && sizeof(KT) == 8 && sizeof(idx_t) == 4), "slot keys: the build that issues its loads first, 32-bit indices");
     TL_DECL(KT, rk, TILE_EPT);
     TL_DECL(idx_t, rs, TILE_EPT);
     if (ISSUE) {
@@ -2569,6 +2657,7 @@
     }
     const BucketParams bp = bps[g];
     const uint64_t b0 = bstart[g];
+    const uint32_t ks = SLOT32 ? slot_key_shift(bp.range, bp.B) : 0u;
     const bool grouped = GROUPED && bp.B > 1 && bp.B <= BUCKET_LDS;
     const BucketParams fbp = GROUPED ? fbps[g] : bp;
     SHARED_ARRAY(uint32_t, hist, TILE_BINS + 1);
@@ -2576,7 +2665,7 @@
     static_assert(sizeof(KT) == 8 || (SRC == SRC_ARRAYS && MAP == MAP_LINEAR), "32-bit keys: arrays in, linear map");
     static_assert(!REC_IN || (SRC == SRC_ARRAYS && sizeof(KT) == 8 && sizeof(idx_t) == 4), "records: arrays in, 64-bit keys, 32-bit indices");
     SHARED_ARRAY(KT, skey, TILE_E);
-    SHARED_ARRAY(idx_t, ssa, TILE_E);
+    SHARED_ARRAY(idx_t, ssa, SLOT32 ? 1 : TILE_E);
     SHARED_ARRAY(uint16_t, sbk, TILE_E);
     SHARED_ARRAY(uint64_t, lr_at, SPILL ? SPILL_LONG_CAP : 1);
     SHARED_ARRAY(idx_t, lr_old, SPILL ? SPILL_LONG_CAP : 1);
@@ -2613,8 +2702,11 @@
                         const uint64_t off = bp.B == 1 ? (start - t.s0) + e : (uint64_t)caps_fetch_add(&cursor[bi], (idx_t)1);
                         if (!spec || off < slot_cap) {
                             const uint64_t dst = (spec ? bi * slot_cap : sub_start[bi]) + off;
-                            out_key[dst] = TL(rk, tid, k);
-                            out_sa[dst] = TL(rs, tid, k);
+                            if (SLOT32) out_key[dst] = (KT)slot_rec((uint64_t)TL(rk, tid, k), ks, (uint32_t)TL(rs, tid, k));
+                            else {
+                                out_key[dst] = TL(rk, tid, k);
+                                out_sa[dst] = TL(rs, tid, k);
+                            }
                         }
                     }
                 }
@@ -2786,8 +2878,11 @@
             if (e < cnt) {
                 const uint32_t bk = TL(rb, tid, k);
                 const uint32_t q = hist[bk] + (uint32_t)TL(rr, tid, k);
-                skey[q] = TL(rk, tid, k);
-                ssa[q] = TL(rs, tid, k);
+                if (SLOT32) skey[q] = (KT)slot_rec((uint64_t)TL(rk, tid, k), ks, (uint32_t)TL(rs, tid, k));
+                else {
+                    skey[q] = TL(rk, tid, k);
+                    ssa[q] = TL(rs, tid, k);
+                }
                 sbk[q] = (uint16_t)bk;
             }
         }
@@ -2844,7 +2939,7 @@
                 } else if (ob != NO_SLOT) {
                     const uint64_t dst = (uint64_t)ob + (q - hist[bk]);
                     STREAM_STORE2(&out_key[dst], skey[q]);
-                    STREAM_STORE2(&out_sa[dst], ssa[q]);
+                    if (!SLOT32) STREAM_STORE2(&out_sa[dst], ssa[q]);
                 }
             }
         }
diff --git a/caps-sa_amd/csrc/pipeline.h b/caps-sa_amd/csrc/pipeline.h
--- a/caps-sa_amd/csrc/pipeline.h
+++ b/caps-sa_amd/csrc/pipeline.h
@@ -60,6 +60,7 @@
 constexpr uint32_t DIRECT_RECORDS_DEFAULT = 1;
 constexpr uint32_t DIRECT_TILE_CHAIN_DEFAULT = 1;
 constexpr uint32_t DIRECT_SCATTER_ISSUE_DEFAULT = 1;
+constexpr uint32_t DIRECT_SLOT_KEYS_DEFAULT = 1;
 #ifndef CAPS_BUCKET_Q_32NDS
 #define CAPS_BUCKET_Q_32NDS 24
 #endif
@@ -369,6 +370,7 @@
     bool skip_finished = false;
     bool unified = false;
     bool k32 = false;
+    bool slot_keys = false;
     bool failed = false;
     SegBufs segs;
     struct RunBucket { uint64_t s0, s1, key; };
@@ -437,12 +439,53 @@
     uint32_t* tile_chain_used = nullptr;
     uint32_t scatter_issue = 0;
     uint32_t* scatter_issue_used = nullptr;
+    uint32_t slot_keys = 0;
+    uint32_t* slot_keys_used = nullptr;
     KernelClock* tile_clock = nullptr;
     KernelClock* merge_clock = nullptr;
     KernelClock* scatter_clock = nullptr;
     KernelClock* count_clock = nullptr;
     uint64_t* pass_counters = nullptr;
 };
+
+template <typename idx_t, int BITS>
+void describe_slot_keys(Backend& be, const uint32_t* P, const BucketBufs& bk, const uint64_t* seg_start, const std::vector<uint64_t>& ss,
+                        uint32_t slot_grid, uint32_t G, const idx_t* sa)
+{
+    std::vector<uint8_t> ks(slot_grid);
+    std::vector<BucketParams> tm(slot_grid);
+    uint64_t ties[2] = {0, 0};
+    uint64_t* dbg_ties = bk.count;
+    be.memset(dbg_ties, 0, sizeof ties);
+    CAPS_LAUNCH((slot_tie_count_kernel<idx_t, BITS>), slot_grid < 4096 ? slot_grid : 4096u, 256, be, P, seg_start, slot_grid,
+                (const uint8_t*)bk.kshift, sa, dbg_ties);
+    be.d2h(ks.data(), bk.kshift, ks.size());
+    be.d2h(tm.data(), bk.tile_map, tm.size() * sizeof(BucketParams));
+    be.d2h(ties, dbg_ties, sizeof ties);
+    be.sync();
+    uint32_t smin = 64, smax = 0, wraps = 0, full = 0;
+    for (uint32_t g = 0; g < slot_grid; ++g) {
+        if (ss[g + 1] == ss[g]) continue;
+        ++full;
+        smin = std::min<uint32_t>(smin, ks[g]);
+        smax = std::max<uint32_t>(smax, ks[g]);
+        const uint32_t w = 32u + ks[g];
+        if (w < 64 && (tm[g].kmin >> w) != ((tm[g].kmin + tm[g].range) >> w)) ++wraps;
+    }
+    std::fprintf(stderr, "[sort] slot keys: shifts %u .. %u, %u of %u buckets whose window wraps, %llu neighbour pairs with equal slot keys, "
+                 "%llu bucket heads tied with the element before them\n", full ? smin : 0u, smax, wraps, full,
+                 (unsigned long long)ties[0], (unsigned long long)ties[1]);
+    if (G > 256) return;
+    std::vector<BucketParams> gp(G);
+    std::vector<uint64_t> gb((size_t)G + 1);
+    be.d2h(gp.data(), bk.params, gp.size() * sizeof(BucketParams));
+    be.d2h(gb.data(), bk.bstart, gb.size() * sizeof(uint64_t));
+    be.sync();
+    for (uint32_t g = 0; g < G; ++g)
+        if (gb[g + 1] > gb[g])
+            std::fprintf(stderr, "[sort] slot keys: group map kmin %llu kmax %llu B %u first bucket %llu\n",
+                         (unsigned long long)gp[g].kmin, (unsigned long long)(gp[g].kmin + gp[g].range), gp[g].B, (unsigned long long)gb[g]);
+}
 
 template <typename idx_t, int BITS>
 SortResult<idx_t> segmented_sort(Backend& be, const uint32_t* P, uint64_t n, TileDesc* desc, const SegBufs& s, uint32_t n_tiles,
@@ -469,6 +512,12 @@
     uint64_t* slot_key = nullptr;
     idx_t* slot_sa = nullptr;
     uint32_t slot_grid = 0;
+    bool slot32 = false;
+    if constexpr (sizeof(idx_t) == 4 && BITS == 2)
+        slot32 = (o.slot_keys & 1u) != 0 && (o.scatter_issue & 1u) != 0 && (o.tile_chain & 1u) != 0 && o.in_records && o.in_key && o.bk && !o.knots &&
+                 !o.k32 && o.speculate && !o.skewed_keys && !o.comparison_only && !o.keys_only && !o.runs && !o.from_text && o.need_lcp &&
+                 o.final_sa && o.final_lcp;
+    if (o.slot_keys_used) *o.slot_keys_used = 0;
     if (o.bk && (max_len > TILE_E || o.seg_ends)) {
         const BucketBufs& bk = *o.bk;
         const SegDesc psd = s.desc();
@@ -487,7 +536,7 @@
         CAPS_LAUNCH(scan_sizes_kernel, 1, 1024, be, (const uint64_t*)bk.segB, s.G, bk.bstart);
         CAPS_LAUNCH(bucket_ranges_kernel, (bk.nb_cap + 255) / 256, 256, be, (const uint64_t*)bk.bstart, s.G,
                     (const BucketParams*)bk.params, o.pkey, o.range_mode, o.part_off, o.part_total ? o.part_total : s.G, o.sub,
-                    bk.tile_map, (const BucketParams*)nullptr, (const uint32_t*)nullptr, o.gshift, bk.kshift);
+                    bk.tile_map, (const BucketParams*)nullptr, (const uint32_t*)nullptr, o.gshift, bk.kshift, slot32 ? 1u : 0u);
         }
         seg_map = bk.tile_map;
         mark("bucket plan");
@@ -507,7 +556,7 @@
             const uint64_t extent = o.in_key ? o.in_extent : n_elems;
             if (room >= extent * sizeof(uint16_t)) bid = reinterpret_cast<uint16_t*>(oth.lcp);
         }
-        auto scatter = [&](const uint64_t* sub_start, uint32_t cap, uint64_t* okey, idx_t* osa, bool grouped = false) {
+        auto scatter = [&](const uint64_t* sub_start, uint32_t cap, uint64_t* okey, idx_t* osa, bool grouped = false, bool rec_out = false) {
             const BucketParams* fbps = grouped ? bk.fparams : nullptr;
             const uint32_t* gfirst = grouped ? bk.gfirst : nullptr;
             BackendEvent s0 = be.record();
@@ -527,7 +576,14 @@
                 if constexpr (sizeof(idx_t) == 4) {
                     if (by_knots) CAPS_SCATTER_LAUNCH_REC(MAP_SPLIT);
                     else if (grouped) CAPS_SCATTER_LAUNCH_REC(MAP_GROUPED);
-                    else if (o.scatter_issue & 1u) {
+                    else if (rec_out) {
+                        if constexpr (BITS == 2)
+                            CAPS_LAUNCH((bucket_scatter_kernel<idx_t, BITS, SRC_ARRAYS, MAP_LINEAR, uint64_t, false, true, true, true>), n_tiles, TILE_NT, be,
+                                        psd, P, n_words, tbase, src_key, src_sa, rsrc, (const BucketParams*)bk.params, (const uint64_t*)bk.bstart, sub_start,
+                                        (uint64_t)cap, static_cast<idx_t*>(bk.cursor), okey, osa, fbps, gfirst, o.knots, (const uint16_t*)nullptr,
+                                        (const uint32_t*)nullptr, 1u, o.knots_per_parent, o.sub, (const uint16_t*)bid, Spill<idx_t>());
+                        if (o.scatter_issue_used) *o.scatter_issue_used |= 1u;
+                    } else if (o.scatter_issue & 1u) {
                         CAPS_LAUNCH((bucket_scatter_kernel<idx_t, BITS, SRC_ARRAYS, MAP_LINEAR, uint64_t, false, true, true>), n_tiles, TILE_NT, be, psd,
                                     P, n_words, tbase, src_key, src_sa, rsrc, (const BucketParams*)bk.params, (const uint64_t*)bk.bstart, sub_start,
                                     (uint64_t)cap, static_cast<idx_t*>(bk.cursor), okey, osa, fbps, gfirst, o.knots, (const uint16_t*)nullptr,
@@ -589,6 +645,7 @@
                               oth.region_bytes >= slot_elems * ((o.k32 ? sizeof(uint32_t) : sizeof(uint64_t)) + sizeof(idx_t)) &&
                               slot_elems + TILE_E < (uint64_t)std::numeric_limits<idx_t>::max();
         if (o.k32 && !can_slot) { r.failed = true; return r; }
+        slot32 = slot32 && can_slot;
         if (can_slot) {
             slot_key = oth.key;
             slot_sa = reinterpret_cast<idx_t*>(reinterpret_cast<char*>(oth.key) + slot_elems * sizeof(uint64_t));
@@ -605,12 +662,13 @@
                 BackendEvent s1 = be.record();
                 if (o.scatter_clock) { o.scatter_clock->spans.push_back({s0, s1}); o.scatter_clock->elems.push_back(n_elems); }
             } else
-            scatter(nullptr, TILE_E, slot_key, slot_sa);
+            scatter(nullptr, TILE_E, slot_key, slot_sa, false, slot32);
             CAPS_LAUNCH((widen_kernel<idx_t>), (bk.nb_cap + 255) / 256, 256, be, (const idx_t*)static_cast<idx_t*>(bk.cursor),
                         (uint64_t)bk.nb_cap, bk.count);
             adopt_buckets();
             bucket_tiles();
             slots = out2[1] <= TILE_E;
+            slot32 = slot32 && slots;
             if (o.slot_stats) ++o.slot_stats[slots ? 0 : 1];
             if (o.k32 && !slots) { r.failed = true; return r; }
             if (dbg) std::fprintf(stderr, "[sort] slot split: largest bucket %llu -> %s\n", (unsigned long long)out2[1], slots ? "kept" : "redone");
@@ -737,7 +795,7 @@
                             (const uint64_t*)bk.fsegB, (const uint64_t*)bk.fstart, (const uint64_t*)bk.fcount, bk.count, bk.gfirst);
                 CAPS_LAUNCH(bucket_ranges_kernel, (bk.nb_cap + 255) / 256, 256, be, (const uint64_t*)bk.bstart, s.G,
                             (const BucketParams*)bk.params, o.pkey, o.range_mode, o.part_off, o.part_total ? o.part_total : s.G, o.sub,
-                            bk.tile_map, (const BucketParams*)bk.fparams, (const uint32_t*)bk.gfirst, o.gshift, bk.kshift);
+                            bk.tile_map, (const BucketParams*)bk.fparams, (const uint32_t*)bk.gfirst, o.gshift, bk.kshift, 0u);
             }
             BackendEvent c1 = be.record();
             if (o.count_clock) { o.count_clock->spans.push_back({c0, c1}); o.count_clock->elems.push_back(n_elems); }
@@ -764,7 +822,7 @@
         r.skip_finished = true;
         r.segs = segs;
         r.n_tiles = n_tiles;
-    }
+    } else slot32 = false;
     const SegDesc sd = segs.desc();
     SegDesc sd_hot = sd;
     if (slot_cap && max_len > slot_cap && o.hot_tile_rec) {
@@ -814,6 +872,8 @@
     const idx_t* in_sa = slot_cap ? slot_sa : (o.in_key && segs.seg_start == s.seg_start) ? static_cast<const idx_t*>(o.in_sa) : cur.sa;
     const uint8_t* no_shift = nullptr;
     r.k32 = o.k32 && slot_cap != 0;
+    r.slot_keys = slot32;
+    if (o.slot_keys_used) *o.slot_keys_used = slot32 ? 1u : 0u;
     std::vector<uint64_t> dbg_ss;
     if (from_text) {
         CAPS_LAUNCH((tile_sort_kernel<idx_t, BITS, true>), n_tiles, TILE_NT, be, sd, P, n, o.text_base, lcp_mode, 0u,
@@ -846,6 +906,7 @@
             by_bucket = (o.tile_chain & 1u) != 0 && !all_queued && slot_grid != 0 && slot_cap == TILE_E && max_len <= TILE_E &&
                         seg_map != nullptr && sd_hot.tile_rec == sd.tile_rec && slot_grid <= segs.G;
         if (o.tile_chain_used) *o.tile_chain_used = by_bucket ? 1u : 0u;
+        if (slot32 && !by_bucket) throw std::logic_error("slots of slot-key records are read by the bucket-indexed launch only");
         if (dbg && !by_bucket && (o.tile_chain & 1u) != 0)
             std::fprintf(stderr, "[sort] table launch although the bucket-indexed one was asked for: idx bytes %u, all queued %d, slots %u of capacity %u "
                          "(a tile: %u), longest bucket %llu, bin maps %d, second tile table %d, segments %u\n", (unsigned)sizeof(idx_t), all_queued ? 1 : 0,
@@ -870,8 +931,15 @@
                          "%u buckets below %u elements, %u below %u, smallest %llu\n", slot_grid, n_tiles, inner, last,
                          (unsigned long long)(ss[last + 1] - ss[last]), small, TILE_NT, cut, (TILE_EPT - 1) * TILE_NT, (unsigned long long)least);
         }
+        const uint32_t kft = slot32 ? 1u : 0u;
         if (all_queued && !per_tile) CAPS_LAUNCH(queue_all_tiles_kernel, (n_tiles + 255) / 256, 256, be, sd, redo);
-        else if (by_bucket) {
+        else if (by_bucket && slot32) {
+            if constexpr (sizeof(idx_t) == 4 && BITS == 2) {
+                CAPS_LAUNCH((tile_sort_kernel<idx_t, BITS, false, uint64_t, 1, true>), slot_grid, TILE_NT, be, sd, P, n, (uint64_t)0, lcp_mode, slot_cap,
+                            in_key, in_sa, cur.key, cur.sa, cur.lcp, fin, seg_map, redo, (const uint8_t*)o.bk->kshift);
+                CAPS_LAUNCH(slot_unpack_kernel, ggrid, 256, be, sd, (const uint32_t*)redo, slot_cap, in_key, slot_sa);
+            }
+        } else if (by_bucket) {
             if constexpr (sizeof(idx_t) == 4)
                 CAPS_LAUNCH((tile_sort_kernel<idx_t, BITS, false, uint64_t, 1>), slot_grid, TILE_NT, be, sd, P, n, (uint64_t)0, lcp_mode, slot_cap,
                             in_key, in_sa, cur.key, cur.sa, cur.lcp, fin, seg_map, redo, no_shift);
@@ -901,9 +969,9 @@
                             in_key, in_sa, cur.key, cur.sa, cur.lcp, fin, (const uint32_t*)redo3, 0u, bflag);
         } else {
             if (eq_tiles) CAPS_LAUNCH((tile_sort_eq_kernel<idx_t, BITS, false>), ggrid, TILE_NT, be, sd_hot, P, n, (uint64_t)0, lcp_mode, slot_cap,
-                        in_key, in_sa, cur.key, cur.sa, cur.lcp, fin, seg_map, (const uint32_t*)redo, redo3, 0u | drop, redo2);
+                        in_key, in_sa, cur.key, cur.sa, cur.lcp, fin, seg_map, (const uint32_t*)redo, redo3, kft | drop, redo2);
             if (eq_tiles) CAPS_LAUNCH((tile_sort_eq_kernel<idx_t, BITS, false, true>), ggrid, TILE_NT, be, sd, P, n, (uint64_t)0, lcp_mode, slot_cap,
-                        in_key, in_sa, cur.key, cur.sa, cur.lcp, fin, seg_map, (const uint32_t*)redo2, redo3, 0u, (uint32_t*)nullptr);
+                        in_key, in_sa, cur.key, cur.sa, cur.lcp, fin, seg_map, (const uint32_t*)redo2, redo3, kft, (uint32_t*)nullptr);
             if (bflag) {
                 uint32_t ng = 0;
                 be.d2h(&ng, redo3, sizeof ng);
@@ -911,7 +979,7 @@
                 defer_check(ng);
             }
             CAPS_LAUNCH_RUNS(tile_sort_general_kernel, (idx_t, BITS, false), ggrid, TILE_NT, be, sd, P, n, (uint64_t)0, lcp_mode, slot_cap,
-                        in_key, in_sa, cur.key, cur.sa, cur.lcp, fin, (const uint32_t*)redo3, 0u, bflag);
+                        in_key, in_sa, cur.key, cur.sa, cur.lcp, fin, (const uint32_t*)redo3, kft, bflag);
         }
         }
     }
@@ -934,6 +1002,8 @@
             }
             std::fprintf(stderr, "[sort] bucket-indexed launch: %u tiles queued, %u behind an empty slot, %u not tiles of the launch\n", q[0], moved, bad);
         }
+        if constexpr (sizeof(idx_t) == 4 && BITS == 2)
+            if (slot32 && !dbg_ss.empty()) describe_slot_keys<idx_t, BITS>(be, P, *o.bk, segs.seg_start, dbg_ss, slot_grid, s.G, fin.sa);
     }
     if (o.tile_clock) { o.tile_clock->spans.push_back({t0, t1}); o.tile_clock->elems.push_back(n_elems); }
     const uint32_t grid = n_tiles < be.persistent_blocks() ? n_tiles : be.persistent_blocks();
@@ -1234,7 +1304,7 @@
                         r.passes & 1u, dSA, dLCP, r.fin);
         if (r.fin.sa != nullptr)
             CAPS_LAUNCH((head_lcp_kernel<idx_t, BITS>), (r.segs.G + 255) / 256, 256, be, P, n, (const uint64_t*)r.segs.seg_start, r.segs.G,
-                        r.fin, r.k32 ? 1u : 0u);
+                        r.fin, r.k32 || r.slot_keys ? 1u : 0u);
     });
     if (!r.run_buckets.empty()) timed(r.runb_clock, 0, [&] { sort_run_buckets<idx_t, BITS>(be, P, n, r, dSA, dLCP); });
     if (r.defer_flags && !std::getenv("CAPS_SA_DEBUG_NO_MSD"))
@@ -1348,7 +1418,7 @@
     uint32_t passes1_ = 0, passes2_ = 0, passesS_ = 0;
     BackendEvent e2_, e3_, e4_, e5_, e6_, e7_, la0_, la1_;
     uint64_t max_part_ = 0;
-    uint32_t path_direct_ = 0, path_fallback_ = 0, direct_groups_ = 0, direct_quantile_ = 0, direct_k32_ = 0, direct_records_ = 0, tile_chain_ = 0, scatter_issue_ = 0, run_buckets_ = 0;
+    uint32_t path_direct_ = 0, path_fallback_ = 0, direct_groups_ = 0, direct_quantile_ = 0, direct_k32_ = 0, direct_records_ = 0, tile_chain_ = 0, scatter_issue_ = 0, slot_keys_ = 0, run_buckets_ = 0;
     uint64_t direct_max_group_ = 0;
     uint64_t tie_groups_ = 0, tie_elems_ = 0;
     uint32_t tie_levels_ = 0;
@@ -1625,6 +1695,9 @@
         const bool may_wave = !(k32 || waves_ < 2 || !wave_scratch_.key);
         const uint32_t issue_want = rec_a && !quantile && !may_wave ? (issue_env ? (uint32_t)std::atoi(issue_env) : DIRECT_SCATTER_ISSUE_DEFAULT) & 1u : 0u;
         scatter_issue_ = 0;
+        const char* slot_env = std::getenv("CAPS_SA_SLOT_KEYS");
+        const uint32_t slot_want = BITS == 2 && issue_want && (chain_want & 1u) ? (slot_env ? (uint32_t)std::atoi(slot_env) : DIRECT_SLOT_KEYS_DEFAULT) & 1u : 0u;
+        slot_keys_ = 0;
         if (k32) CAPS_LAUNCH(group_shift_kernel, (K1 + 255) / 256, 256, be_, (const uint64_t*)pl_.gkey, K1, pl_.gshift);
         if (quantile) {
             CAPS_LAUNCH((sample_text_kernel<idx_t, BITS>), (uint32_t)((m2 + 255) / 256), 256, be_, (const uint32_t*)pl_.P, (uint64_t)0, n, m2,
@@ -1806,6 +1879,7 @@
             }
             set_final(ow, dSA + base, dLCP + base);
             if (W == 1) { ow.tile_chain = chain_want; ow.tile_chain_used = &tile_chain_; }
+            if (W == 1) { ow.slot_keys = slot_want; ow.slot_keys_used = &slot_keys_; }
             ow.scatter_issue = issue_want;
             ow.scatter_issue_used = &scatter_issue_;
             if (elems_w) {
@@ -1919,6 +1993,7 @@
             st->direct_records = path_direct_ ? direct_records_ : 0u;
             st->tile_chain = path_direct_ ? tile_chain_ : 0u;
             st->scatter_issue = path_direct_ ? scatter_issue_ : 0u;
+            st->slot_keys = path_direct_ ? slot_keys_ : 0u;
             st->direct_max_group = direct_max_group_;
             st->level_a_ms = direct_groups_ ? be_.elapsed_ms(la0_, la1_) : 0.0;
             st->slot_splits = slot_stats_[0];
diff --git a/include/caps_sa_hip.h b/include/caps_sa_hip.h
--- a/include/caps_sa_hip.h
+++ b/include/caps_sa_hip.h
@@ -63,6 +63,7 @@
     uint32_t direct_records;
     uint32_t tile_chain;
     uint32_t scatter_issue;
+    uint32_t slot_keys;
 } caps_sa_stats;
 
 uint32_t caps_sa_hip_stats_bytes(void);
```
